# zaiisao/ConTEXTure-NeRF

Measured on AMD Instinct MI355X. Metric: UNet denoise steps/sec (CFG-batched SD2-depth UNet eval + PLMS update), higher is better.
Workload: dtype f16; 1 GPU; BASELINE configs[1]: 1 view @768^2 (latent 96^2), 50 PLMS steps (51 UNet evals), SD2-depth UNet fp16, CFG batch 2, guidance 10, random-init weights; mesh substitution napoleon.obj -> n/a for this stage (denoise loop only); latent=96, cfg_batch=2, ctx_len=77, views_per_rank=1, parallelism=view-shard x1

## Files before the change

contexture-nerf_amd/csrc/gemm.hip:

```cpp
#include "common.h"
#include "kernels.h"
#include <hip/hip_ext.h>
#include <stdlib.h>

__device__ __forceinline__ int xcd_remap(int bid, int nwg)
{
    int q = nwg >> 3, r = nwg & 7, x = bid & 7;
    return (x < r ? x * (q + 1) : r * (q + 1) + (x - r) * q) + (bid >> 3);
}

__device__ __forceinline__ float fast_erf(float x)
{
    float ax = __builtin_fabsf(x);
    float t = __builtin_amdgcn_rcpf(1.0f + 0.3275911f * ax);
    float p = t * (0.254829592f + t * (-0.284496736f + t * (1.421413741f + t * (-1.453152027f + t * 1.061405429f))));
    float e = 1.0f - p * __builtin_amdgcn_exp2f(-1.4426950408889634f * ax * ax);
    return __builtin_copysignf(e, x);
}
__device__ __forceinline__ float gelu_erf(float x) { return 0.5f * x * (1.0f + fast_erf(x * 0.70710678118654752f)); }

template <int MI, int NI>
__device__ __forceinline__ void gemm_epilogue(const GemmArgs &a, f32x16 (&acc)[MI][NI], int mw, int nw, int r, int h)
{
#pragma unroll
    for (int mi = 0; mi < MI; ++mi) {
        int m = mw + mi * 32 + r;
        if (m >= a.M) continue;
        int bidx = a.rowbias ? m / a.rows_per_batch : 0;
        if (a.epi == 1) {
            if constexpr (NI == 2) {
                int fbase = nw / 2;
#pragma unroll
                for (int g = 0; g < 4; ++g) {
                    int nn = nw + 8 * g + 4 * h;
                    if (nn >= a.N) continue;
                    f16x4 o;
#pragma unroll
                    for (int j = 0; j < 4; ++j) {
                        float xv = acc[mi][0][4 * g + j], gv = acc[mi][1][4 * g + j];
                        if (a.bias) { xv += (float)a.bias[nn + j]; gv += (float)a.bias[nn + 32 + j]; }
                        o[j] = (f16)(xv * gelu_erf(gv));
                    }
                    *(f16x4 *)(a.out + (size_t)m * a.ldc + fbase + 8 * g + 4 * h) = o;
                }
            }
        } else {
#pragma unroll
            for (int ni = 0; ni < NI; ++ni)
#pragma unroll
                for (int g = 0; g < 4; ++g) {
                    int nn = nw + ni * 32 + 8 * g + 4 * h;
                    if (nn >= a.N) continue;
                    float v[4];
#pragma unroll
                    for (int j = 0; j < 4; ++j) v[j] = acc[mi][ni][4 * g + j];
                    if (a.bias) {
                        f16x4 b = *(const f16x4 *)(a.bias + nn);
#pragma unroll
                        for (int j = 0; j < 4; ++j) v[j] += (float)b[j];
                    }
                    if (a.rowbias) {
                        f16x4 b = *(const f16x4 *)(a.rowbias + (size_t)bidx * a.ldrb + nn);
#pragma unroll
                        for (int j = 0; j < 4; ++j) v[j] += (float)b[j];
                    }
                    if (a.residual) {
                        if (a.res32) {
                            f32x4 b = *(const f32x4 *)((const float *)a.residual + (size_t)m * a.ldr + nn);
#pragma unroll
                            for (int j = 0; j < 4; ++j) v[j] += b[j];
                        } else {
                            f16x4 b = *(const f16x4 *)(a.residual + (size_t)m * a.ldr + nn);
#pragma unroll
                            for (int j = 0; j < 4; ++j) v[j] += (float)b[j];
                        }
                    }
                    if (a.out32) {
                        *(f32x4 *)((float *)a.out + (size_t)m * a.ldc + nn) = (f32x4){v[0], v[1], v[2], v[3]};
                    } else {
                        f16x4 o;
#pragma unroll
                        for (int j = 0; j < 4; ++j) o[j] = (f16)v[j];
                        *(f16x4 *)(a.out + (size_t)m * a.ldc + nn) = o;
                    }
                }
        }
    }
}

template <int MI, int NI>
__device__ __forceinline__ void gemm_epilogue_staged(const GemmArgs &a, f32x16 (&acc)[MI][NI], int mw, int nw, int r, int h,
                                                     float *stage, int lane)
{
    constexpr int RS = 32 * NI + 4;
    constexpr int LPR = 4 * NI;
    constexpr int RPP = 64 / LPR;
    const int prow = lane / LPR, c8 = (lane % LPR) * 8;
    const int n = nw + c8;
    f16x8 bs = {0, 0, 0, 0, 0, 0, 0, 0};
    if (a.bias && n < a.N) bs = *(const f16x8 *)(a.bias + n);
#pragma unroll
    for (int mi = 0; mi < MI; ++mi) {
#pragma unroll
        for (int ni = 0; ni < NI; ++ni)
#pragma unroll
            for (int g = 0; g < 4; ++g) {
                f32x4 v = {acc[mi][ni][4 * g], acc[mi][ni][4 * g + 1], acc[mi][ni][4 * g + 2], acc[mi][ni][4 * g + 3]};
                *(f32x4 *)(stage + r * RS + ni * 32 + 8 * g + 4 * h) = v;
            }
#pragma unroll
        for (int p = 0; p < 32 / RPP; ++p) {
            const int row = RPP * p + prow;
            const int m = mw + mi * 32 + row;
            f32x4 v0 = *(const f32x4 *)(stage + row * RS + c8), v1 = *(const f32x4 *)(stage + row * RS + c8 + 4);
            if (m < a.M && n < a.N) {
                float v[8] = {v0[0], v0[1], v0[2], v0[3], v1[0], v1[1], v1[2], v1[3]};
#pragma unroll
                for (int j = 0; j < 8; ++j) v[j] += (float)bs[j];
                if (a.rowbias) {
                    f16x8 b = *(const f16x8 *)(a.rowbias + (size_t)(m / a.rows_per_batch) * a.ldrb + n);
#pragma unroll
                    for (int j = 0; j < 8; ++j) v[j] += (float)b[j];
                }
                if (a.residual) {
                    if (a.res32) {
                        const float *rp = (const float *)a.residual + (size_t)m * a.ldr + n;
                        f32x4 b0 = *(const f32x4 *)rp, b1 = *(const f32x4 *)(rp + 4);
#pragma unroll
                        for (int j = 0; j < 4; ++j) { v[j] += b0[j]; v[4 + j] += b1[j]; }
                    } else {
                        f16x8 b = *(const f16x8 *)(a.residual + (size_t)m * a.ldr + n);
#pragma unroll
                        for (int j = 0; j < 8; ++j) v[j] += (float)b[j];
                    }
                }
                if (a.out32) {
                    float *op = (float *)a.out + (size_t)m * a.ldc + n;
                    *(f32x4 *)op = (f32x4){v[0], v[1], v[2], v[3]}; *(f32x4 *)(op + 4) = (f32x4){v[4], v[5], v[6], v[7]};
                } else {
                    f16x8 o;
#pragma unroll
                    for (int j = 0; j < 8; ++j) o[j] = (f16)v[j];
                    *(f16x8 *)(a.out + (size_t)m * a.ldc + n) = o;
                }
            }
        }
    }
}

__device__ __attribute__((aligned(16))) f16 g_zero_page[64];

typedef const __attribute__((address_space(1))) void *gptr_t;
typedef __attribute__((address_space(3))) void *lptr_t;

template <int WM, int WN, int MI, int NI, bool CONV, int NS, int PKT>
__global__ __launch_bounds__(64 * WM * WN) void k_gemm_pipe(GemmArgs a)
{
    constexpr int BM = 32 * MI * WM, BN = 32 * NI * WN, NW = WM * WN;
    constexpr int RP = 512 / PKT;
    constexpr int LPR = PKT / 8;
    constexpr int XI = BM / (RP * NW), WI = BN / (RP * NW);
    static_assert(XI >= 1 && WI >= 1, "tile too small for the wave count");
    constexpr int G = XI + WI;
    constexpr int STAGE = (BM + BN) * PKT;
    extern __shared__ __attribute__((aligned(16))) f16 smem[];

    const int tid = threadIdx.x, lane = tid & 63, wave = __builtin_amdgcn_readfirstlane(tid >> 6);
    const int r = lane & 31, h = lane >> 5;
    const int wm = wave / WN, wn = wave % WN;
    const int ntiles = a.ntm * a.ntn;
    const int lin = xcd_remap(blockIdx.x, ntiles * a.splitk);
    const int slice = lin / ntiles, bid = lin - slice * ntiles;
    const int tile_n = a.mfast ? bid / a.ntm : bid % a.ntn, tile_m = a.mfast ? bid % a.ntm : bid / a.ntn;
    const int m0 = tile_m * BM, n0 = tile_n * BN;
    const int lr = lane / LPR, pc = lane % LPR;

    const int nk_all = a.K / PKT;
    const int kbeg = (int)((long)nk_all * slice / a.splitk);
    const int nk = (int)((long)nk_all * (slice + 1) / a.splitk) - kbeg;

    const f16 *xp[XI], *wp[WI];
    int xst[XI], wst[WI];
    int xoff[XI], xoy[XI], xox[XI], xlc[XI];
    bool xok[XI];
#pragma unroll
    for (int i = 0; i < XI; ++i) {
        int row = RP * (wave + NW * i) + lr;
        int m = m0 + row;
        xlc[i] = (pc ^ (PKT == 32 ? ((row >> 2) & 3) : ((row >> 1) & 7))) * 8;
        xok[i] = m < a.M;
        if (CONV) {
            int hw = a.Ho * a.Wo;
            int b = m / hw, p = m - b * hw;
            int oy = p / a.Wo, ox = p - oy * a.Wo;
            xoy[i] = oy * a.stride; xox[i] = ox * a.stride;
            xoff[i] = b * a.H * a.W * a.Cin;
            xp[i] = g_zero_page; xst[i] = 0;
        } else {
            xoff[i] = 0; xoy[i] = 0; xox[i] = 0;
            xp[i] = xok[i] ? a.X + (size_t)m * a.K + kbeg * PKT + xlc[i] : g_zero_page;
            xst[i] = xok[i] ? PKT : 0;
        }
    }
#pragma unroll
    for (int i = 0; i < WI; ++i) {
        int row = RP * (wave + NW * i) + lr;
        bool ok = (n0 + row) < a.N;
        wp[i] = ok ? a.Wt + (size_t)(n0 + row) * a.K + kbeg * PKT + ((pc ^ (PKT == 32 ? ((row >> 2) & 3) : ((row >> 1) & 7))) * 8) : g_zero_page;
        wst[i] = ok ? PKT : 0;
    }
    const int k_lo = kbeg * PKT, k_hi = (kbeg + nk) * PKT;
    const int rot = a.krot == 1 ? (int)(((unsigned)tile_m * 13u + (unsigned)tile_n * 5u) % (unsigned)nk) : 0;
    int k_issue = k_lo + rot * PKT, issued = 0, tap_left = 0;
    if (!CONV) {
#pragma unroll
        for (int i = 0; i < XI; ++i) xp[i] += (xst[i] ? rot * PKT : 0);
    }
#pragma unroll
    for (int i = 0; i < WI; ++i) wp[i] += (wst[i] ? rot * PKT : 0);

    auto retap = [&]() {
        int tap = k_issue / a.Cin, c0 = k_issue - tap * a.Cin;
        int dy = tap / 3 - 1 + a.poff, dx = tap % 3 - 1 + a.poff;
        int Hv = a.H << a.ups, Wv = a.W << a.ups;
#pragma unroll
        for (int i = 0; i < XI; ++i) {
            int iy = xoy[i] + dy, ix = xox[i] + dx;
            bool ok = xok[i] && iy >= 0 && iy < Hv && ix >= 0 && ix < Wv && !(a.zins && ((iy | ix) & 1));
            xp[i] = ok ? a.X + xoff[i] + (((iy >> a.ups) * a.W + (ix >> a.ups)) * a.Cin) + c0 + xlc[i] : g_zero_page;
            xst[i] = ok ? PKT : 0;
        }
        tap_left = (a.Cin - c0) / PKT;
    };
    auto issue = [&](int buf) {
        if (k_issue == k_hi) {
            k_issue = k_lo;
            const int span = k_hi - k_lo;
            if (!CONV) {
#pragma unroll
                for (int i = 0; i < XI; ++i) xp[i] -= (xst[i] ? span : 0);
            }
#pragma unroll
            for (int i = 0; i < WI; ++i) wp[i] -= (wst[i] ? span : 0);
            tap_left = 0;
        }
        if (CONV) {
            if (tap_left == 0) retap();
            --tap_left;
        }
        f16 *Xs = smem + buf * STAGE;
        f16 *Ws = Xs + BM * PKT;
#pragma unroll
        for (int i = 0; i < XI; ++i) {
            __builtin_amdgcn_global_load_lds((gptr_t)xp[i], (lptr_t)(Xs + (wave + NW * i) * 512), 16, 0, 0);
            xp[i] += xst[i];
        }
#pragma unroll
        for (int i = 0; i < WI; ++i) {
            __builtin_amdgcn_global_load_lds((gptr_t)wp[i], (lptr_t)(Ws + (wave + NW * i) * 512), 16, 0, 0);
            wp[i] += wst[i];
        }
        k_issue += PKT;
        ++issued;
    };

    f32x16 acc[MI][NI];
#pragma unroll
    for (int i = 0; i < MI; ++i)
#pragma unroll
        for (int j = 0; j < NI; ++j)
#pragma unroll
            for (int q = 0; q < 16; ++q) acc[i][j][q] = 0.f;

#pragma unroll
    for (int p = 0; p < NS - 1; ++p)
        if (p < nk) issue(p);
    const int swz = PKT == 32 ? ((r >> 2) & 3) : ((r >> 1) & 7);
    const int xrow = (wm * 32 * MI + r) * PKT, wrow = BM * PKT + (wn * 32 * NI + r) * PKT;
    int kt = 0;
    for (; a.krot == 0 && kt + 2 * NS - 2 < nk; kt += NS) {
#pragma unroll
        for (int u = 0; u < NS; ++u) {
            asm volatile("s_waitcnt vmcnt(%0) lgkmcnt(0)" ::"n"((NS - 2) * G) : "memory");
            ctx_barrier();
            issue((u + NS - 1) % NS);
            const f16 *sb = smem + u * STAGE;
#pragma unroll
            for (int ks = 0; ks < PKT / 16; ++ks) {
                const int pch = ((2 * ks + h) ^ swz) * 8;
                f16x8 xf[MI], wf[NI];
#pragma unroll
                for (int i = 0; i < MI; ++i) xf[i] = *(const f16x8 *)(sb + xrow + i * 32 * PKT + pch);
#pragma unroll
                for (int j = 0; j < NI; ++j) wf[j] = *(const f16x8 *)(sb + wrow + j * 32 * PKT + pch);
#pragma unroll
                for (int i = 0; i < MI; ++i)
#pragma unroll
                    for (int j = 0; j < NI; ++j) acc[i][j] = __builtin_amdgcn_mfma_f32_32x32x16_f16(wf[j], xf[i], acc[i][j], 0, 0, 0);
            }
        }
    }
    for (; kt < nk; kt += NS) {
#pragma unroll
        for (int u = 0; u < NS; ++u) {
            if (kt + u < nk) {
                int newer = issued - 1 - (kt + u);
                if (NS >= 8 && newer >= 6) asm volatile("s_waitcnt vmcnt(%0)" ::"n"(6 * G) : "memory");
                else if (NS >= 7 && newer >= 5) asm volatile("s_waitcnt vmcnt(%0)" ::"n"(5 * G) : "memory");
                else if (NS >= 6 && newer >= 4) asm volatile("s_waitcnt vmcnt(%0)" ::"n"(4 * G) : "memory");
                else if (NS >= 5 && newer >= 3) asm volatile("s_waitcnt vmcnt(%0)" ::"n"(3 * G) : "memory");
                else if (NS >= 4 && newer >= 2) asm volatile("s_waitcnt vmcnt(%0)" ::"n"(2 * G) : "memory");
                else if (newer >= 1) asm volatile("s_waitcnt vmcnt(%0)" ::"n"(G) : "memory");
                else asm volatile("s_waitcnt vmcnt(0)" ::: "memory");
                asm volatile("s_waitcnt lgkmcnt(0)" ::: "memory");
                ctx_barrier();
                if (issued < nk) issue((u + NS - 1) % NS);
                const f16 *sb = smem + u * STAGE;
#pragma unroll
                for (int ks = 0; ks < PKT / 16; ++ks) {
                    const int pch = ((2 * ks + h) ^ swz) * 8;
                    f16x8 xf[MI], wf[NI];
#pragma unroll
                    for (int i = 0; i < MI; ++i) xf[i] = *(const f16x8 *)(sb + xrow + i * 32 * PKT + pch);
#pragma unroll
                    for (int j = 0; j < NI; ++j) wf[j] = *(const f16x8 *)(sb + wrow + j * 32 * PKT + pch);
#pragma unroll
                    for (int i = 0; i < MI; ++i)
#pragma unroll
                        for (int j = 0; j < NI; ++j) acc[i][j] = __builtin_amdgcn_mfma_f32_32x32x16_f16(wf[j], xf[i], acc[i][j], 0, 0, 0);
                }
            }
        }
    }
    if (a.splitk > 1) {
        float *pb = a.part + (size_t)slice * a.M * a.N;
#pragma unroll
        for (int mi = 0; mi < MI; ++mi) {
            int m = m0 + wm * 32 * MI + mi * 32 + r;
            if (m >= a.M) continue;
#pragma unroll
            for (int ni = 0; ni < NI; ++ni)
#pragma unroll
                for (int g = 0; g < 4; ++g) {
                    int nn = n0 + wn * 32 * NI + ni * 32 + 8 * g + 4 * h;
                    if (nn >= a.N) continue;
                    f32x4 v = {acc[mi][ni][4 * g], acc[mi][ni][4 * g + 1], acc[mi][ni][4 * g + 2], acc[mi][ni][4 * g + 3]};
                    *(f32x4 *)(pb + (size_t)m * a.N + nn) = v;
                }
        }
        return;
    }
    if (a.epi == 0 && a.stage_epi) {
        asm volatile("s_waitcnt vmcnt(0) lgkmcnt(0)" ::: "memory");
        ctx_barrier();
        gemm_epilogue_staged<MI, NI>(a, acc, m0 + wm * 32 * MI, n0 + wn * 32 * NI, r, h, (float *)smem + wave * (32 * (32 * NI + 4)), lane);
        return;
    }
    gemm_epilogue<MI, NI>(a, acc, m0 + wm * 32 * MI, n0 + wn * 32 * NI, r, h);
}

__global__ __launch_bounds__(256) void k_splitk_reduce(GemmArgs a)
{
    const int n4 = a.N / 4;
    const size_t total = (size_t)a.M * n4, MN = (size_t)a.M * a.N;
    for (size_t i = (size_t)blockIdx.x * 256 + threadIdx.x; i < total; i += (size_t)gridDim.x * 256) {
        int m = (int)(i / n4), nn = (int)(i % n4) * 4;
        f32x4 v = *(const f32x4 *)(a.part + (size_t)m * a.N + nn);
        for (int sidx = 1; sidx < a.splitk; ++sidx) {
            f32x4 p = *(const f32x4 *)(a.part + sidx * MN + (size_t)m * a.N + nn);
            v += p;
        }
        if (a.bias) { f16x4 b = *(const f16x4 *)(a.bias + nn); for (int j = 0; j < 4; ++j) v[j] += (float)b[j]; }
        if (a.rowbias) {
            f16x4 b = *(const f16x4 *)(a.rowbias + (size_t)(m / a.rows_per_batch) * a.ldrb + nn);
            for (int j = 0; j < 4; ++j) v[j] += (float)b[j];
        }
        if (a.residual) {
            if (a.res32) { f32x4 b = *(const f32x4 *)((const float *)a.residual + (size_t)m * a.ldr + nn); v += b; }
            else { f16x4 b = *(const f16x4 *)(a.residual + (size_t)m * a.ldr + nn); for (int j = 0; j < 4; ++j) v[j] += (float)b[j]; }
        }
        if (a.out32) { *(f32x4 *)((float *)a.out + (size_t)m * a.ldc + nn) = v; continue; }
        f16x4 o;
        for (int j = 0; j < 4; ++j) o[j] = (f16)v[j];
        *(f16x4 *)(a.out + (size_t)m * a.ldc + nn) = o;
    }
}

static int g_force_tile = -1, g_force_gemm8 = -1;
extern "C" void ctx_gemm_tune(int32_t tile, int32_t gemm8)
{
    g_force_tile = tile;
    g_force_gemm8 = gemm8;
}

template <int WM, int WN, int MI, int NI, bool CONV, int NS = 4, int PKT = 32>
static void launch_gemm(GemmArgs &a, hipStream_t s)
{
    constexpr int BM = 32 * MI * WM, BN = 32 * NI * WN;
    a.ntm = cdiv(a.M, BM);
    a.ntn = cdiv(a.N, BN);
    if (a.splitk < 1 || !a.part) a.splitk = 1;
    static int mfast = -2;
    if (mfast == -2) { const char *e = getenv("CTX_GEMM_MFAST"); mfast = e ? atoi(e) : -1; }
    const double wbytes = (double)a.N * a.K, xbytes = (double)a.M * (CONV ? a.Cin : a.K);
    a.mfast = mfast >= 0 ? mfast : (wbytes > xbytes ? 1 : 0);
    static int stg = -1;
    if (stg < 0) { const char *e = getenv("CTX_GEMM_STAGE_EPI"); stg = e ? atoi(e) : 1; }
    a.stage_epi = stg && (a.ldc % 8 == 0) && (!a.residual || a.ldr % 8 == 0) && (!a.rowbias || a.ldrb % 8 == 0) &&
                  (size_t)WM * WN * 32 * (32 * NI + 4) * sizeof(float) <= 160 * 1024;
    static int steady = -1;
    if (steady < 0) { const char *e = getenv("CTX_GEMM_STEADY"); steady = e ? atoi(e) : 1; }
    a.pk = PKT; a.krot = steady ? 0 : 2;
    constexpr int NT = 64 * WM * WN;
    constexpr size_t ring = (size_t)NS * (BM + BN) * PKT * sizeof(f16);
    constexpr size_t patch = (size_t)WM * WN * 32 * (32 * NI + 4) * sizeof(float);
    constexpr size_t lds = (ring > patch || patch > 160 * 1024) ? ring : patch;
    auto kern = k_gemm_pipe<WM, WN, MI, NI, CONV, NS, PKT>;
    static bool attr_done = false;
    if (!attr_done) {
        (void)hipFuncSetAttribute((const void *)kern, hipFuncAttributeMaxDynamicSharedMemorySize, (int)lds);
        attr_done = true;
    }
    if (ctx_prof_on()) {
        hipEvent_t e0, e1;
        ctx_prof_events(0, &e0, &e1);
        hipExtLaunchKernelGGL(kern, dim3(a.ntm * a.ntn * a.splitk), dim3(NT), lds, s, e0, e1, 0, a);
    } else
        hipLaunchKernelGGL(kern, dim3(a.ntm * a.ntn * a.splitk), dim3(NT), lds, s, a);
}

static void launch_reduce(GemmArgs &a, hipStream_t s)
{
    size_t total = (size_t)a.M * (a.N / 4);
    unsigned nb = (unsigned)((total + 255) / 256 < 2048 ? (total + 255) / 256 : 2048);
    if (ctx_prof_on()) {
        hipEvent_t e0, e1;
        ctx_prof_events(0, &e0, &e1);
        hipExtLaunchKernelGGL(k_splitk_reduce, dim3(nb), dim3(256), 0, s, e0, e1, 0, a);
    } else
        hipLaunchKernelGGL(k_splitk_reduce, dim3(nb), dim3(256), 0, s, a);
}

int ctx_gemm_pick_split(int M, int N, int K, int epi)
{
    static int en = -1;
    if (en < 0) { const char *e = getenv("CTX_SPLITK"); en = e ? atoi(e) : 1; }
    if (!en || epi != 0 || N % 4) return 1;
    bool wide = (N % 128 == 0);
    int tiles = wide ? cdiv(M, 128) * cdiv(N, 128) : cdiv(M, 256) * cdiv(N, 64);
    if (tiles >= 200) return 1;
    if (K < 2048 && tiles > 48) return 1;
    int S = 640 / tiles;
    int maxS = (K / 32) / 8;
    if (S > maxS) S = maxS;
    if (S > 32) S = 32;
    return S < 2 ? 1 : S;
}

#include "gemm_tuned.h"
void ctx_gemm_plan(GemmArgs &a, bool conv)
{
    a.tile = -1; a.use8 = -1;
    static int use_table = -1;
    if (use_table < 0) { const char *e = getenv("CTX_GEMM_TUNED"); use_table = e ? atoi(e) : 1; }
    if (use_table) {
        const int flags = conv ? ((a.stride == 2 ? 1 : 0) | (a.ups ? 2 : 0)) : 0;
        for (const TunedGemm &t : g_tuned)
            if (t.conv == (conv ? 1 : 0) && t.M == a.M && t.N == a.N && t.K == a.K && t.flags == flags && t.epi == a.epi) {
                a.tile = t.tile; a.use8 = t.use8; a.splitk = t.splitk;
                return;
            }
    }
    if (a.K % 64 == 0 && (!conv || a.Cin % 64 == 0)) {
        const double MN = (double)a.M * a.N;
        static const int heur144 = [] { const char *e = getenv("CTX_GEMM_HEUR144"); return e ? atoi(e) : 1; }();
        if (heur144 && a.epi == 0 && a.N % 8 == 0 && !a.zins && !a.res32 && !a.out32) {
            const int nt = cdiv(a.N, 160);
            const double fill = (double)a.N / (160.0 * nt);
            if (fill >= 0.9) {
                if (cdiv(a.M, 288) * nt >= 512) { a.tile = -1; a.use8 = 8; a.splitk = 1; return; }
                if (cdiv(a.M, 144) * nt >= 220) { a.tile = -1; a.use8 = 6; a.splitk = 1; return; }
            }
        }
        int tile, bm, bn;
        if (MN >= 5.0e6) { tile = a.epi == 1 ? 10 : (conv ? 12 : 11); bm = 256; bn = 128; }
        else if ((MN >= 2.5e6 && a.K >= 960) || (conv && MN >= 1.2e6 && a.K >= 5760)) { tile = 14; bm = 128; bn = 128; }
        else if (a.epi == 1) { tile = 16; bm = 64; bn = 128; }
        else { tile = 15; bm = 64; bn = 64; }
        const int tiles = cdiv(a.M, bm) * cdiv(a.N, bn);
        int S = 1;
        if (a.epi == 0 && a.N % 4 == 0) {
            S = 320 / tiles;
            const int maxS = a.K / 64 / 4;
            if (S > maxS) S = maxS;
            if (S > 12) S = 12;
            if (S < 1) S = 1;
        }
        a.tile = tile; a.splitk = S;
        a.use8 = (a.epi == 1 && MN >= 1.0e7) ? -1 : 0;
        return;
    }
    a.splitk = ctx_gemm_pick_split(a.M, a.N, a.K, a.epi);
}

int ctx_gemm_dispatch(GemmArgs &a, bool conv, hipStream_t s)
{
    const bool only_pipe = a.zins || a.res32 || a.out32;
    if (only_pipe) a.use8 = 0;
    const int want8 = only_pipe ? 0 : (g_force_gemm8 >= 0 ? g_force_gemm8 : a.use8);
    const int want_tile = g_force_tile >= 0 ? g_force_tile : (g_force_gemm8 >= 0 ? -1 : a.tile);
    if (want_tile < 0 && want8 >= 4 && want8 <= 8 && ctx_gemm144_try(a, conv, want8 - 4, s)) {
        if (a.splitk > 1) launch_reduce(a, s);
    } else if (want_tile < 0 && conv && (want8 == 2 || want8 == 3) && ctx_conv_halo_try(a, want8 == 2 ? 2 : 1, s)) {
        if (a.splitk > 1) launch_reduce(a, s);
    } else if (want_tile < 0 && want8 != 0 && want8 < 2 && ctx_gemm8_try(a, conv, want8 == 1, s)) {
        if (a.splitk > 1) launch_reduce(a, s);
    } else {
        static int big = -1;
        if (big < 0) { const char *e = getenv("CTX_GEMM_BIG"); big = e ? atoi(e) : 1; }
        const int S = a.splitk > 1 && a.part ? a.splitk : 1;
        auto wgs = [&](int bm, int bn) { return cdiv(a.M, bm) * cdiv(a.N, bn) * S; };
        const bool n128 = (a.N % 128 == 0);
        int pick;
        static int bigk = -1;
        if (bigk < 0) { const char *e = getenv("CTX_GEMM_BIGK"); bigk = e ? atoi(e) : 1024; }
        if (big && a.M >= 8192 && a.N >= 256 && a.K >= bigk) pick = 0;
        else if (n128 && wgs(128, 128) >= 384) pick = 1;
        else if (!n128 && wgs(256, 64) >= 384) pick = 2;
        else if (wgs(128, 64) >= 320) pick = 3;
        else if (S > 1) pick = n128 ? 1 : 2;
        else pick = 4;
        static int force = -2;
        if (force == -2) { const char *e = getenv("CTX_GEMM_TILE"); force = e ? atoi(e) : -1; }
        if (force >= 0) pick = force;
        if (want_tile >= 0) pick = want_tile;
        if (a.epi == 1 && (pick == 5 || pick == 6 || pick == 9 || pick == 11 || pick == 13 || pick == 15 || pick == 17 || pick == 19 || pick == 21 || pick == 23 || pick == 26 || pick == 27)) pick = 1;
        if (pick >= 10 && (a.K % 64 != 0 || (conv && a.Cin % 64 != 0))) pick = 1;
#define CTX_LAUNCH(WM_, WN_, MI_, NI_) do { if (conv) launch_gemm<WM_, WN_, MI_, NI_, true>(a, s); else launch_gemm<WM_, WN_, MI_, NI_, false>(a, s); } while (0)
        switch (pick) {
        case 0: CTX_LAUNCH(4, 2, 2, 2); break;
        case 1: CTX_LAUNCH(2, 2, 2, 2); break;
        case 2: CTX_LAUNCH(4, 1, 2, 2); break;
        case 3: CTX_LAUNCH(2, 1, 2, 2); break;
        case 4: CTX_LAUNCH(1, 1, 2, 2); break;
        case 5: CTX_LAUNCH(2, 2, 1, 1); break;
        case 6: CTX_LAUNCH(1, 2, 2, 1); break;
        case 7: CTX_LAUNCH(4, 2, 1, 2); break;
        case 8: CTX_LAUNCH(2, 2, 1, 2); break;
        case 9: CTX_LAUNCH(2, 2, 2, 1); break;
#define CTX_LAUNCH64(WM_, WN_, MI_, NI_) do { if (conv) launch_gemm<WM_, WN_, MI_, NI_, true, 3, 64>(a, s); else launch_gemm<WM_, WN_, MI_, NI_, false, 3, 64>(a, s); } while (0)
        case 10: CTX_LAUNCH64(8, 2, 1, 2); break;
        case 11: CTX_LAUNCH64(4, 4, 2, 1); break;
        case 12: CTX_LAUNCH64(4, 2, 2, 2); break;
        case 13: CTX_LAUNCH64(4, 4, 1, 1); break;
        case 14: CTX_LAUNCH64(4, 2, 1, 2); break;
        case 15: CTX_LAUNCH64(2, 2, 1, 1); break;
        case 16: CTX_LAUNCH64(2, 2, 1, 2); break;
        case 17: CTX_LAUNCH64(2, 2, 2, 1); break;
        case 18: CTX_LAUNCH64(2, 2, 2, 2); break;
#define CTX_LAUNCH64N2(WM_, WN_, MI_, NI_) do { if (conv) launch_gemm<WM_, WN_, MI_, NI_, true, 2, 64>(a, s); else launch_gemm<WM_, WN_, MI_, NI_, false, 2, 64>(a, s); } while (0)
        case 19: CTX_LAUNCH64N2(2, 2, 1, 1); break;
        case 20: CTX_LAUNCH64N2(4, 2, 1, 2); break;
        case 21: CTX_LAUNCH64N2(4, 4, 1, 1); break;
        case 22: CTX_LAUNCH64N2(2, 2, 2, 2); break;
#define CTX_LAUNCH64NS(NS_, WM_, WN_, MI_, NI_) do { if (conv) launch_gemm<WM_, WN_, MI_, NI_, true, NS_, 64>(a, s); else launch_gemm<WM_, WN_, MI_, NI_, false, NS_, 64>(a, s); } while (0)
        case 23: CTX_LAUNCH64NS(6, 2, 2, 1, 1); break;
        case 24: CTX_LAUNCH64NS(5, 2, 2, 1, 2); break;
        case 25: CTX_LAUNCH64NS(4, 4, 2, 1, 2); break;
        case 26: CTX_LAUNCH64NS(5, 2, 2, 2, 1); break;
        default: CTX_LAUNCH64N2(4, 2, 2, 5); break;
#undef CTX_LAUNCH64NS
#undef CTX_LAUNCH64N2
#undef CTX_LAUNCH64
        }
#undef CTX_LAUNCH
        if (a.splitk > 1) launch_reduce(a, s);
    }
    hipError_t e = hipGetLastError();
    if (e != hipSuccess) {
        ctx_set_error("gemm launch failed: %s", hipGetErrorString(e));
        return CTX_E_LAUNCH;
    }
    return CTX_OK;
}

extern "C" int32_t ctx_gemm_f16(const void *A, const void *Wt, const void *bias, const void *residual, int32_t M,
                                int32_t N, int32_t K, void *C, ctx_stream_t stream)
{
    CTX_REQUIRE(A && Wt && C, "gemm: null pointer");
    CTX_REQUIRE(M > 0 && N > 0 && K > 0 && K % 64 == 0 && N % 8 == 0, "gemm: need K%%64==0, N%%8==0 (M=%d N=%d K=%d)", M, N, K);
    CTX_REQUIRE((int64_t)M * K < (1ll << 31) && (int64_t)N * K < (1ll << 31), "gemm: operand too large for 32-bit offsets");
    GemmArgs a = {};
    a.X = (const f16 *)A; a.Wt = (const f16 *)Wt; a.bias = (const f16 *)bias; a.residual = (const f16 *)residual;
    a.out = (f16 *)C; a.M = M; a.N = N; a.K = K; a.ldc = N; a.ldr = N; a.rows_per_batch = 1; a.ldrb = N; a.epi = 0;
    a.tile = -1; a.use8 = -1;
    return ctx_gemm_dispatch(a, false, (hipStream_t)stream);
}

extern "C" int32_t ctx_conv3x3_f16(const void *x, const void *w, const void *bias, const void *rowbias,
                                   const void *residual, int32_t B, int32_t H, int32_t W, int32_t Cin, int32_t Cout,
                                   int32_t stride, int32_t upsample, void *y, ctx_stream_t stream)
{
    CTX_REQUIRE(x && w && y, "conv3x3: null pointer");
    CTX_REQUIRE(B > 0 && H > 0 && W > 0 && Cin % 64 == 0 && Cout % 8 == 0 && (stride == 1 || stride == 2) &&
                    (upsample == 0 || upsample == 1) && !(upsample && stride == 2),
                "conv3x3: need Cin%%64==0, Cout%%8==0, stride 1|2 (B=%d H=%d W=%d Cin=%d Cout=%d s=%d up=%d)", B, H, W, Cin, Cout, stride, upsample);
    GemmArgs a = {};
    int Hv = H << upsample, Wv = W << upsample;
    a.Ho = (Hv + 2 - 3) / stride + 1; a.Wo = (Wv + 2 - 3) / stride + 1;
    a.X = (const f16 *)x; a.Wt = (const f16 *)w; a.bias = (const f16 *)bias; a.rowbias = (const f16 *)rowbias;
    a.residual = (const f16 *)residual; a.out = (f16 *)y;
    a.M = B * a.Ho * a.Wo; a.N = Cout; a.K = 9 * Cin; a.ldc = Cout; a.ldr = Cout; a.rows_per_batch = a.Ho * a.Wo; a.ldrb = Cout; a.epi = 0;
    a.H = H; a.W = W; a.Cin = Cin; a.stride = stride; a.ups = upsample;
    a.tile = -1; a.use8 = -1;
    CTX_REQUIRE((int64_t)B * H * W * Cin < (1ll << 31) && (int64_t)Cout * a.K < (1ll << 31), "conv3x3: tensor too large for 32-bit offsets");
    return ctx_gemm_dispatch(a, true, (hipStream_t)stream);
}

#define GV_U 4
__global__ __launch_bounds__(256) void k_gemv_f16(const f16 *__restrict__ x, const f16 *__restrict__ w,
                                                  const f16 *__restrict__ bias, int Bm, int N, int K, int silu_in,
                                                  int silu_out, f16 *__restrict__ out)
{
    const int lane = threadIdx.x & 63;
    const int n0 = ((blockIdx.x * 256 + threadIdx.x) >> 6) * 2;
    if (n0 >= N) return;
    const int n1 = n0 + 1 < N ? n0 + 1 : n0;
    float acc[2][4] = {{0.f, 0.f, 0.f, 0.f}, {0.f, 0.f, 0.f, 0.f}};
    const f16x8 zero8 = {0, 0, 0, 0, 0, 0, 0, 0};
    for (int k0 = 0; k0 < K; k0 += 512 * GV_U) {
        f16x8 wv[2][GV_U];
#pragma unroll
        for (int u = 0; u < GV_U; ++u) {
            const int k = k0 + u * 512 + lane * 8;
            const int kc = k < K ? k : K - 8;
            wv[0][u] = *(const f16x8 *)(w + (size_t)n0 * K + kc);
            wv[1][u] = *(const f16x8 *)(w + (size_t)n1 * K + kc);
        }
#pragma unroll
        for (int u = 0; u < GV_U; ++u) {
            const int k = k0 + u * 512 + lane * 8;
            if (k >= K) { wv[0][u] = zero8; wv[1][u] = zero8; }
            const int kc = k < K ? k : K - 8;
            for (int b = 0; b < Bm; ++b) {
                f16x8 xv = *(const f16x8 *)(x + (size_t)b * K + kc);
#pragma unroll
                for (int j = 0; j < 8; ++j) {
                    float xf = (float)xv[j];
                    if (silu_in) xf = xf / (1.0f + __expf(-xf));
                    acc[0][b] += xf * (float)wv[0][u][j];
                    acc[1][b] += xf * (float)wv[1][u][j];
                }
            }
        }
    }
    for (int r = 0; r < 2; ++r) {
        const int n = n0 + r;
        for (int b = 0; b < Bm; ++b) {
            float v = wave_sum(acc[r][b]);
            if (lane == 0 && n < N) {
                if (bias) v += (float)bias[n];
                if (silu_out) v = v / (1.0f + __expf(-v));
                out[(size_t)b * N + n] = (f16)v;
            }
        }
    }
}

int ctx_gemv_f16(const f16 *x, const f16 *w, const f16 *bias, int Bm, int N, int K, int silu_in, int silu_out, f16 *out,
                 hipStream_t s)
{
    if (Bm < 1 || K % 8 != 0 || K < 8) {
        ctx_set_error("gemv: Bm=%d (>=1) K=%d (%%8)", Bm, K);
        return CTX_E_ARG;
    }
    for (int b0 = 0; b0 < Bm; b0 += 4) {
        const int nb = Bm - b0 < 4 ? Bm - b0 : 4;
        hipLaunchKernelGGL(k_gemv_f16, dim3(cdiv(N, 8)), dim3(256), 0, s, x + (size_t)b0 * K, w, bias, nb, N, K, silu_in, silu_out,
                           out + (size_t)b0 * N);
    }
    return CTX_OK;
}

extern "C" float ctx_bench_gemm(const void *A, const void *Wt, const void *bias, const void *residual, int32_t M, int32_t N,
                                int32_t K, void *C, int32_t conv_B, int32_t conv_H, int32_t conv_W, int32_t conv_Cin,
                                int32_t conv_flags, int32_t epi, void *part, int32_t splitk, int32_t iters, ctx_stream_t stream)
{
    hipStream_t s = (hipStream_t)stream;
    GemmArgs a = {};
    a.X = (const f16 *)A; a.Wt = (const f16 *)Wt; a.bias = (const f16 *)bias; a.residual = (const f16 *)residual; a.out = (f16 *)C;
    bool conv = conv_B > 0;
    if (conv) {
        a.stride = (conv_flags & 1) ? 2 : 1; a.ups = (conv_flags & 2) ? 1 : 0;
        int Hv = conv_H << a.ups, Wv = conv_W << a.ups;
        a.H = conv_H; a.W = conv_W; a.Cin = conv_Cin; a.Ho = (Hv - 1) / a.stride + 1; a.Wo = (Wv - 1) / a.stride + 1;
        a.M = conv_B * a.Ho * a.Wo; a.N = N; a.K = 9 * conv_Cin; a.rows_per_batch = a.Ho * a.Wo;
    } else {
        a.M = M; a.N = N; a.K = K; a.rows_per_batch = 1;
    }
    a.epi = epi;
    a.ldc = epi == 1 ? a.N / 2 : a.N; a.ldr = a.N; a.ldrb = a.N;
    a.tile = -1; a.use8 = -1;
    if (splitk < 0) {
        if (part) { ctx_gemm_plan(a, conv); splitk = a.splitk; } else splitk = 1;
    }
    hipEvent_t e0, e1;
    (void)hipEventCreate(&e0); (void)hipEventCreate(&e1);
    for (int i = 0; i < iters + 2; ++i) {
        if (i == 2) (void)hipEventRecord(e0, s);
        GemmArgs b = a;
        b.splitk = splitk; b.part = (float *)part;
        int rc = ctx_gemm_dispatch(b, conv, s);
        if (rc) return (float)rc;
    }
    (void)hipEventRecord(e1, s);
    (void)hipEventSynchronize(e1);
    float ms = 0.f;
    (void)hipEventElapsedTime(&ms, e0, e1);
    (void)hipEventDestroy(e0); (void)hipEventDestroy(e1);
    return ms / iters;
}
```

contexture-nerf_amd/csrc/gemm144.hip:

```cpp
#include "common.h"
#include "kernels.h"
#include <hip/hip_ext.h>
#include <stdlib.h>
#include <type_traits>

typedef const __attribute__((address_space(1))) void *g144_gptr_t;
typedef __attribute__((address_space(3))) void *g144_lptr_t;
__device__ __attribute__((aligned(128))) f16 g144_zero[64];

#define G144_BM 144
#define G144_BN 160
#define G144_STAGE ((G144_BM + G144_BN) * 64)

__device__ __forceinline__ int g144_xcd_remap(int bid, int nwg)
{
    int q = nwg >> 3, r = nwg & 7, x = bid & 7;
    return (x < r ? x * (q + 1) : r * (q + 1) + (x - r) * q) + (bid >> 3);
}

template <int WM, int WN, bool CONV, int NS, int VAR, bool UPS = false, int BMB = 9>
__global__ __launch_bounds__(64 * WM * WN) void k_gemm144(GemmArgs a)
{
    constexpr int NW = WM * WN, MI = BMB / WM, NI = 10 / WN;
    constexpr int BM = 16 * BMB, NPX = BM / 8;
    constexpr int NP = NPX + 20;
    constexpr int STAGE = (BM + G144_BN) * 64;
    static_assert(BMB % WM == 0 && (BMB == 9 || (BMB == 18 && VAR == 0)), "288-row tiles: lockstep schedule only");
    constexpr int SL = (NP + NW - 1) / NW;
    static_assert(9 % WM == 0 && 10 % WN == 0, "wave grid must divide 9 x 10 blocks");
    extern __shared__ __attribute__((aligned(16))) f16 smem[];
    const int tid = threadIdx.x, lane = tid & 63, wave = __builtin_amdgcn_readfirstlane(tid >> 6);
    const int wm = wave / WN, wn = wave % WN;
    const int r16 = lane & 15, kg = lane >> 4;

    const int ntiles = a.ntm * a.ntn;
    const int lin = g144_xcd_remap(blockIdx.x, ntiles * a.splitk);
    const int slice = lin / ntiles, bid = lin - slice * ntiles;
    const int tile_n = a.mfast ? bid / a.ntm : bid % a.ntn, tile_m = a.mfast ? bid % a.ntm : bid / a.ntn;
    const int m0 = tile_m * BM, n0 = tile_n * G144_BN;
    const int nk_all = a.K / 64;
    const int kbeg = (int)((long)nk_all * slice / a.splitk);
    const int nk = (int)((long)nk_all * (slice + 1) / a.splitk) - kbeg;

    const int prow = lane >> 3, pc = lane & 7;
    constexpr bool FAST = CONV && !UPS;
    const f16 *pp[SL], *xcen[SL];
    int pst[SL], xoff[SL], xoy[SL], xox[SL], xlc[SL], xval[SL];
    bool xok[SL];
    const f16 *const zp = g144_zero;
    const bool full = wave + NW * (SL - 1) < NP;
#pragma unroll
    for (int i = 0; i < SL; ++i) {
        const int p = wave + NW * i;
        const bool isx = p < NPX, live = p < NP;
        const int s = isx ? 8 * p + prow : 8 * (p - NPX) + prow;
        xlc[i] = (pc ^ ((s >> 1) & 7)) * 8;
        xoff[i] = 0; xoy[i] = 0; xox[i] = 0;
        if (isx) {
            const int m = m0 + s;
            xok[i] = m < a.M;
            if (CONV) {
                const int hw = a.Ho * a.Wo;
                const int mm = xok[i] ? m : 0;
                const int b = mm / hw, q = mm - b * hw;
                const int oy = q / a.Wo, ox = q - oy * a.Wo;
                xoy[i] = oy * a.stride; xox[i] = ox * a.stride;
                xoff[i] = b * a.H * a.W * a.Cin + xlc[i];
                pp[i] = zp; pst[i] = 0;
                if (FAST) {
                    xcen[i] = a.X + (size_t)xoff[i] + (size_t)(xoy[i] * a.W + xox[i]) * a.Cin;
                    int v = 0;
#pragma unroll
                    for (int t = 0; t < 9; ++t) {
                        const int iy = xoy[i] + t / 3 - 1 + a.poff, ix = xox[i] + t % 3 - 1 + a.poff;
                        if (xok[i] && iy >= 0 && iy < a.H && ix >= 0 && ix < a.W) v |= 1 << t;
                    }
                    xval[i] = v;
                }
            } else {
                pp[i] = xok[i] ? a.X + (size_t)m * a.K + (size_t)kbeg * 64 + xlc[i] : g144_zero;
                pst[i] = xok[i] ? 64 : 0;
            }
        } else {
            const bool ok = live && (n0 + s) < a.N;
            xok[i] = ok;
            pp[i] = ok ? a.Wt + (size_t)(n0 + s) * a.K + (size_t)kbeg * 64 + xlc[i] : g144_zero;
            pst[i] = ok ? 64 : 0;
        }
    }

    int k_issue = kbeg * 64, issued = 0, tap_left = 0;
    int cur_tap = CONV ? (kbeg * 64) / a.Cin : 0, cur_c0 = CONV ? kbeg * 64 - cur_tap * a.Cin : 0;
    auto retap = [&]() {
        if (FAST) {
            const int dy = cur_tap / 3 - 1 + a.poff, dx = cur_tap - (cur_tap / 3) * 3 - 1 + a.poff;
            const int soff = (dy * a.W + dx) * a.Cin + cur_c0;
#pragma unroll
            for (int i = 0; i < SL; ++i) {
                if (wave + NW * i >= NPX) continue;
                const bool v = (xval[i] >> cur_tap) & 1;
                pp[i] = v ? xcen[i] + soff : zp;
                pst[i] = v ? 64 : 0;
            }
            tap_left = (a.Cin - cur_c0) >> 6;
            return;
        }
        const int tap = k_issue / a.Cin, c0 = k_issue - tap * a.Cin;
        const int dy = tap / 3 - 1 + a.poff, dx = tap % 3 - 1 + a.poff;
        const int Hv = a.H << a.ups, Wv = a.W << a.ups;
#pragma unroll
        for (int i = 0; i < SL; ++i) {
            if (wave + NW * i >= NPX) continue;
            const int iy = xoy[i] + dy, ix = xox[i] + dx;
            const bool ok = xok[i] && iy >= 0 && iy < Hv && ix >= 0 && ix < Wv;
            pp[i] = ok ? a.X + xoff[i] + (((iy >> a.ups) * a.W + (ix >> a.ups)) * a.Cin) + c0 : zp;
            pst[i] = ok ? 64 : 0;
        }
        tap_left = (a.Cin - c0) / 64;
    };
    auto issue_begin = [&]() {
        if (CONV) {
            if (tap_left == 0) retap();
            --tap_left;
        }
    };
    auto issue_slot = [&](int buf, int i) {
        const int p = wave + NW * i;
        if (p < NP) {
            __builtin_amdgcn_global_load_lds((g144_gptr_t)pp[i], (g144_lptr_t)(smem + buf * STAGE + p * 512), 16, 0, 0);
            pp[i] += pst[i];
        }
    };
    auto issue_end = [&]() {
        k_issue += 64; ++issued;
        if (FAST) { cur_c0 += 64; if (cur_c0 == a.Cin) { cur_c0 = 0; ++cur_tap; } }
    };
    auto issue = [&](int buf) {
        issue_begin();
#pragma unroll
        for (int i = 0; i < SL; ++i) issue_slot(buf, i);
        issue_end();
    };

    f32x4 acc[MI][NI];
#pragma unroll
    for (int i = 0; i < MI; ++i)
#pragma unroll
        for (int j = 0; j < NI; ++j) acc[i][j] = (f32x4){0.f, 0.f, 0.f, 0.f};

    const int swz = (r16 >> 1) & 7;
    const int ck[2] = {(kg ^ swz) * 8, ((4 + kg) ^ swz) * 8};
    const int xrow = (wm * 16 * MI + r16) * 64, wrow = BM * 64 + (wn * 16 * NI + r16) * 64;

#pragma unroll
    for (int p = 0; p < NS - 1; ++p)
        if (p < nk) issue(p);
    auto wait_newer = [&](int newer) {
        if (newer >= 2) {
            if (full) asm volatile("s_waitcnt vmcnt(%0)" ::"n"(2 * SL) : "memory");
            else asm volatile("s_waitcnt vmcnt(%0)" ::"n"(2 * (SL - 1)) : "memory");
        } else if (newer >= 1) {
            if (full) asm volatile("s_waitcnt vmcnt(%0)" ::"n"(SL) : "memory");
            else asm volatile("s_waitcnt vmcnt(%0)" ::"n"(SL - 1) : "memory");
        } else
            asm volatile("s_waitcnt vmcnt(0)" ::: "memory");
    };
    int buf = 0;
    if constexpr (VAR == 0 && BMB == 18) {
        f16x8 xa[MI], wa[NI], wb[NI];
        auto mrow = [&](const f16x8 &xf, const f16x8 (&wf)[NI], int i) {
#pragma unroll
            for (int j = 0; j < NI; ++j) acc[i][j] = __builtin_amdgcn_mfma_f32_16x16x32_f16(wf[j], xf, acc[i][j], 0, 0, 0);
        };
        static_assert(BMB != 18 || SL <= MI, "one DMA piece per MFMA row");
        for (int kt = 0; kt < nk; ++kt) {
            wait_newer(issued - 1 - kt);
            asm volatile("s_waitcnt lgkmcnt(0)" ::: "memory");
            ctx_barrier();
            const bool go = issued < nk;
            const int pb = buf == 0 ? NS - 1 : buf - 1;
            const f16 *sb = smem + buf * STAGE;
#pragma unroll
            for (int i = 0; i < MI; ++i) xa[i] = *(const f16x8 *)(sb + xrow + i * 1024 + ck[0]);
#pragma unroll
            for (int j = 0; j < NI; ++j) wa[j] = *(const f16x8 *)(sb + wrow + j * 1024 + ck[0]);
            if (go) issue_begin();
#pragma unroll
            for (int i = 0; i < MI; ++i) {
                mrow(xa[i], wa, i);
                __builtin_amdgcn_sched_barrier(0);
                xa[i] = *(const f16x8 *)(sb + xrow + i * 1024 + ck[1]);
                if (i == 0) {
#pragma unroll
                    for (int j = 0; j < NI; ++j) wb[j] = *(const f16x8 *)(sb + wrow + j * 1024 + ck[1]);
                }
                if (go && i < SL) issue_slot(pb, i);
                __builtin_amdgcn_sched_barrier(0);
            }
            if (go) issue_end();
#pragma unroll
            for (int i = 0; i < MI; ++i) mrow(xa[i], wb, i);
            buf = buf == NS - 1 ? 0 : buf + 1;
        }
    } else if constexpr (VAR == 0) {
        for (int kt = 0; kt < nk; ++kt) {
            wait_newer(issued - 1 - kt);
            asm volatile("s_waitcnt lgkmcnt(0)" ::: "memory");
            ctx_barrier();
            if (issued < nk) issue(buf == 0 ? NS - 1 : buf - 1);
            const f16 *sb = smem + buf * STAGE;
#pragma unroll
            for (int ks = 0; ks < 2; ++ks) {
                f16x8 xf[MI], wf[NI];
#pragma unroll
                for (int i = 0; i < MI; ++i) xf[i] = *(const f16x8 *)(sb + xrow + i * 1024 + ck[ks]);
#pragma unroll
                for (int j = 0; j < NI; ++j) wf[j] = *(const f16x8 *)(sb + wrow + j * 1024 + ck[ks]);
#pragma unroll
                for (int i = 0; i < MI; ++i)
#pragma unroll
                    for (int j = 0; j < NI; ++j) acc[i][j] = __builtin_amdgcn_mfma_f32_16x16x32_f16(wf[j], xf[i], acc[i][j], 0, 0, 0);
            }
            buf = buf == NS - 1 ? 0 : buf + 1;
        }
    } else if constexpr (VAR == 2) {
        static_assert(VAR != 2 || NS == 4, "written for a ring of 4");
        f16x8 xa[MI], wa[NI], xb[MI], wb[NI];
        auto rd = [&](f16x8 (&xf)[MI], f16x8 (&wf)[NI], const f16 *sb, int ks) {
#pragma unroll
            for (int i = 0; i < MI; ++i) xf[i] = *(const f16x8 *)(sb + xrow + i * 1024 + ck[ks]);
#pragma unroll
            for (int j = 0; j < NI; ++j) wf[j] = *(const f16x8 *)(sb + wrow + j * 1024 + ck[ks]);
        };
        auto mrow = [&](const f16x8 &xf, const f16x8 (&wf)[NI], int i) {
#pragma unroll
            for (int j = 0; j < NI; ++j) acc[i][j] = __builtin_amdgcn_mfma_f32_16x16x32_f16(wf[j], xf, acc[i][j], 0, 0, 0);
        };
        static_assert(SL <= MI, "one DMA piece per MFMA row of a quarter");
        if (issued < nk) issue(issued & 3);
        auto pair = [&](int k0, auto steady) {
            constexpr bool ST = decltype(steady)::value;
            const int b0 = k0 & 3;
            const bool two = ST || k0 + 1 < nk;
            asm volatile("s_waitcnt vmcnt(0) lgkmcnt(0)" ::: "memory");
            ctx_barrier();
            rd(xa, wa, smem + b0 * STAGE, 0);
#pragma unroll
            for (int q = 0; q < 4; ++q) {
                if (q >= 2 && !two) break;
                const bool even = (q & 1) == 0;
                if (q + 1 < (two ? 4 : 2)) {
                    const f16 *sn = smem + (b0 + ((q + 1) >> 1)) * STAGE;
                    if (even) rd(xb, wb, sn, (q + 1) & 1); else rd(xa, wa, sn, (q + 1) & 1);
                }
                const bool dma = even && (ST || (issued < nk && issued <= k0 + 3));
                if (dma) issue_begin();
#pragma unroll
                for (int i = 0; i < MI; ++i) {
                    if (even) mrow(xa[i], wa, i); else mrow(xb[i], wb, i);
                    __builtin_amdgcn_sched_barrier(0);
                    if (dma && i < SL) issue_slot(issued & 3, i);
                    __builtin_amdgcn_sched_barrier(0);
                }
                if (dma) issue_end();
            }
        };
        using T1 = std::integral_constant<bool, true>;
        using T0 = std::integral_constant<bool, false>;
        int k0 = 0;
        if (k0 < nk) { pair(k0, T0{}); k0 += 2; }
        for (; k0 + 3 < nk; k0 += 2) pair(k0, T1{});
        for (; k0 < nk; k0 += 2) pair(k0, T0{});
    } else {
        static_assert(VAR == 0 || NS == 4, "written for a ring of 4");
        wait_newer(issued - 1);
        ctx_barrier();
        f16x8 xp_[MI], wp_[NI], xq[MI], wq[NI], xb[MI], wb[NI];
        auto rd = [&](f16x8 (&xf)[MI], f16x8 (&wf)[NI], const f16 *sb, int ks) {
#pragma unroll
            for (int i = 0; i < MI; ++i) xf[i] = *(const f16x8 *)(sb + xrow + i * 1024 + ck[ks]);
#pragma unroll
            for (int j = 0; j < NI; ++j) wf[j] = *(const f16x8 *)(sb + wrow + j * 1024 + ck[ks]);
        };
        auto mrow = [&](const f16x8 &xf, const f16x8 (&wf)[NI], int i) {
#pragma unroll
            for (int j = 0; j < NI; ++j) acc[i][j] = __builtin_amdgcn_mfma_f32_16x16x32_f16(wf[j], xf, acc[i][j], 0, 0, 0);
        };
        rd(xp_, wp_, smem, 0);
        auto stage = [&](f16x8 (&xc)[MI], f16x8 (&wc)[NI], f16x8 (&xn)[MI], f16x8 (&wn_)[NI], int kt, auto steady) {
            constexpr bool ST = decltype(steady)::value;
            if (ST) {
                if (full) asm volatile("s_waitcnt vmcnt(%0)" ::"n"(SL) : "memory");
                else asm volatile("s_waitcnt vmcnt(%0)" ::"n"(SL - 1) : "memory");
            } else
                wait_newer(issued - 1 - (kt + 1));
            asm volatile("s_waitcnt lgkmcnt(0)" ::: "memory");
            ctx_barrier();
            const bool go = ST || issued < nk;
            const int pb = buf == 0 ? NS - 1 : buf - 1;
            const int nb_ = buf == NS - 1 ? 0 : buf + 1;
            const f16 *sc = smem + buf * STAGE, *sn = smem + nb_ * STAGE;
            const bool more = ST || kt + 1 < nk;
            if (go) issue_begin();
#pragma unroll
            for (int i = 0; i < MI; ++i) {
                mrow(xc[i], wc, i);
                __builtin_amdgcn_sched_barrier(0);
                if (i == 0) rd(xb, wb, sc, 1);
                if (go && i < SL) issue_slot(pb, i);
                __builtin_amdgcn_sched_barrier(0);
            }
            if (go) {
#pragma unroll
                for (int i = MI; i < SL; ++i) issue_slot(pb, i);
                issue_end();
            }
#pragma unroll
            for (int i = 0; i < MI; ++i) {
                mrow(xb[i], wb, i);
                if (i == 0) {
                    __builtin_amdgcn_sched_barrier(0);
                    if (more) rd(xn, wn_, sn, 0);
                    __builtin_amdgcn_sched_barrier(0);
                }
            }
            buf = nb_;
        };
        using T1 = std::integral_constant<bool, true>;
        using T0 = std::integral_constant<bool, false>;
        int kt = 0;
        for (; kt + 4 < nk; kt += 2) {
            stage(xp_, wp_, xq, wq, kt, T1{});
            stage(xq, wq, xp_, wp_, kt + 1, T1{});
        }
        for (; kt + 1 < nk; kt += 2) {
            stage(xp_, wp_, xq, wq, kt, T0{});
            stage(xq, wq, xp_, wp_, kt + 1, T0{});
        }
        if (kt < nk) stage(xp_, wp_, xq, wq, kt, T0{});
    }

    const int mb = m0 + wm * 16 * MI, nb = n0 + wn * 16 * NI;
    if (a.splitk > 1) {
        float *pb = a.part + (size_t)slice * a.M * a.N;
#pragma unroll
        for (int i = 0; i < MI; ++i) {
            const int m = mb + 16 * i + r16;
            if (m >= a.M) continue;
#pragma unroll
            for (int j = 0; j < NI; ++j) {
                const int nn = nb + 16 * j + 4 * kg;
                if (nn < a.N) *(f32x4 *)(pb + (size_t)m * a.N + nn) = acc[i][j];
            }
        }
        return;
    }
    if (a.stage_epi) {
        constexpr int RS = G144_BN + 4;
        float *tile = (float *)smem;
        asm volatile("s_waitcnt vmcnt(0) lgkmcnt(0)" ::: "memory");
        ctx_barrier();
        constexpr int NT = 64 * NW, CPR = G144_BN / 8;
#pragma unroll
        for (int half = 0; half < BMB / 9; ++half) {
            if (half) __syncthreads();
#pragma unroll
            for (int i = 0; i < MI; ++i) {
                const int blk = wm * MI + i;
                if (blk / 9 != half) continue;
#pragma unroll
                for (int j = 0; j < NI; ++j)
                    *(f32x4 *)(tile + ((blk - 9 * half) * 16 + r16) * RS + wn * 16 * NI + 16 * j + 4 * kg) = acc[i][j];
            }
            __syncthreads();
            for (int ch = tid; ch < 144 * CPR; ch += NT) {
                const int row = ch / CPR, c8 = (ch - row * CPR) * 8;
                const int m = m0 + 144 * half + row, n = n0 + c8;
                if (m >= a.M || n >= a.N) continue;
                const f32x4 v0 = *(const f32x4 *)(tile + row * RS + c8), v1 = *(const f32x4 *)(tile + row * RS + c8 + 4);
                float v[8] = {v0[0], v0[1], v0[2], v0[3], v1[0], v1[1], v1[2], v1[3]};
                if (a.bias) {
                    const f16x8 bb = *(const f16x8 *)(a.bias + n);
#pragma unroll
                    for (int e = 0; e < 8; ++e) v[e] += (float)bb[e];
                }
                if (a.rowbias) {
                    const f16x8 bb = *(const f16x8 *)(a.rowbias + (size_t)(m / a.rows_per_batch) * a.ldrb + n);
#pragma unroll
                    for (int e = 0; e < 8; ++e) v[e] += (float)bb[e];
                }
                if (a.residual) {
                    const f16x8 bb = *(const f16x8 *)(a.residual + (size_t)m * a.ldr + n);
#pragma unroll
                    for (int e = 0; e < 8; ++e) v[e] += (float)bb[e];
                }
                f16x8 o;
#pragma unroll
                for (int e = 0; e < 8; ++e) o[e] = (f16)v[e];
                *(f16x8 *)(a.out + (size_t)m * a.ldc + n) = o;
            }
        }
        return;
    }
    f16x4 bs[NI];
#pragma unroll
    for (int j = 0; j < NI; ++j) {
        const int nn = nb + 16 * j + 4 * kg;
        bs[j] = (a.bias && nn < a.N) ? *(const f16x4 *)(a.bias + nn) : (f16x4){0, 0, 0, 0};
    }
#pragma unroll
    for (int i = 0; i < MI; ++i) {
        const int m = mb + 16 * i + r16;
        if (m >= a.M) continue;
        const int bidx = a.rowbias ? m / a.rows_per_batch : 0;
#pragma unroll
        for (int j = 0; j < NI; ++j) {
            const int nn = nb + 16 * j + 4 * kg;
            if (nn >= a.N) continue;
            f32x4 v = acc[i][j];
#pragma unroll
            for (int e = 0; e < 4; ++e) v[e] += (float)bs[j][e];
            if (a.rowbias) {
                f16x4 b = *(const f16x4 *)(a.rowbias + (size_t)bidx * a.ldrb + nn);
#pragma unroll
                for (int e = 0; e < 4; ++e) v[e] += (float)b[e];
            }
            if (a.residual) {
                f16x4 b = *(const f16x4 *)(a.residual + (size_t)m * a.ldr + nn);
#pragma unroll
                for (int e = 0; e < 4; ++e) v[e] += (float)b[e];
            }
            f16x4 o;
#pragma unroll
            for (int e = 0; e < 4; ++e) o[e] = (f16)v[e];
            *(f16x4 *)(a.out + (size_t)m * a.ldc + nn) = o;
        }
    }
}

int ctx_gemm144_try(GemmArgs &a, bool conv, int form, hipStream_t s)
{
    if (a.K % 64 != 0 || (conv && a.Cin % 64 != 0) || a.N % 4 != 0 || a.epi != 0 || a.res32 || a.out32 || a.zins) return 0;
    if (a.ldc % 4 != 0 || (a.residual && a.ldr % 4 != 0) || (a.rowbias && a.ldrb % 4 != 0)) return 0;
    const int bm = form == 4 ? 288 : G144_BM;
    a.ntm = cdiv(a.M, bm);
    a.ntn = cdiv(a.N, G144_BN);
    int S = (a.splitk > 1 && a.part) ? a.splitk : 1;
    if (S > a.K / 64) S = a.K / 64;
    a.splitk = S;
    const double wbytes = (double)a.N * a.K, xbytes = (double)a.M * (conv ? a.Cin : a.K);
    a.mfast = wbytes > xbytes ? 1 : 0;
    static int stg = -1;
    if (stg < 0) { const char *e = getenv("CTX_G144_STAGE"); stg = e ? atoi(e) : 1; }
    a.stage_epi = stg && form != 0 && a.N % 8 == 0 && a.ldc % 8 == 0 && (!a.residual || a.ldr % 8 == 0) && (!a.rowbias || a.ldrb % 8 == 0);
    static bool attr[20] = {};
    auto go = [&](auto kern, int which, int threads, int ns) {
        const size_t lds = (size_t)ns * (bm + G144_BN) * 64 * sizeof(f16);
        if (!attr[which]) {
            (void)hipFuncSetAttribute((const void *)kern, hipFuncAttributeMaxDynamicSharedMemorySize, (int)lds);
            attr[which] = true;
        }
        if (ctx_prof_on()) {
            hipEvent_t e0, e1;
            ctx_prof_events(0, &e0, &e1);
            hipExtLaunchKernelGGL(kern, dim3(a.ntm * a.ntn * S), dim3(threads), lds, s, e0, e1, 0, a);
        } else
            hipLaunchKernelGGL(kern, dim3(a.ntm * a.ntn * S), dim3(threads), lds, s, a);
    };
    const bool ups = conv && a.ups;
    switch (form) {
    case 4:
        if (!conv) go(k_gemm144<3, 5, false, 2, 0, false, 18>, 12, 960, 2);
        else if (ups) go(k_gemm144<3, 5, true, 2, 0, true, 18>, 13, 960, 2); else go(k_gemm144<3, 5, true, 2, 0, false, 18>, 14, 960, 2);
        break;
    case 1:
        if (!conv) go(k_gemm144<3, 5, false, 3, 0>, 2, 960, 3);
        else if (ups) go(k_gemm144<3, 5, true, 3, 0, true>, 8, 960, 3); else go(k_gemm144<3, 5, true, 3, 0>, 3, 960, 3);
        break;
    case 2:
        if (!conv) go(k_gemm144<3, 5, false, 4, 1>, 4, 960, 4);
        else if (ups) go(k_gemm144<3, 5, true, 4, 1, true>, 9, 960, 4); else go(k_gemm144<3, 5, true, 4, 1>, 5, 960, 4);
        break;
    case 3:
        if (!conv) go(k_gemm144<3, 5, false, 4, 2>, 6, 960, 4);
        else if (ups) go(k_gemm144<3, 5, true, 4, 2, true>, 10, 960, 4); else go(k_gemm144<3, 5, true, 4, 2>, 7, 960, 4);
        break;
    default:
        if (!conv) go(k_gemm144<3, 2, false, 3, 0>, 0, 384, 3);
        else if (ups) go(k_gemm144<3, 2, true, 3, 0, true>, 11, 384, 3); else go(k_gemm144<3, 2, true, 3, 0>, 1, 384, 3);
        break;
    }
    return 1;
}
```

contexture-nerf_amd/csrc/kernels.h:

```cpp
#pragma once
#include "common.h"

struct GemmArgs {
    const f16 *X;
    const f16 *Wt;
    const f16 *bias;
    const f16 *rowbias;
    const f16 *residual;
    f16 *out;
    int M, N, K;
    int ldc, ldr;
    int rows_per_batch;
    int ldrb;
    int epi;
    int H, W, Cin, Ho, Wo, stride, ups;
    int poff;
    int res32, out32;
    int zins;
    int ntm, ntn;
    int splitk;
    float *part;
    int pk;
    int krot;
    int tile, use8;
    int stage_epi;
    int mfast;
};

int ctx_gemm_dispatch(GemmArgs &a, bool conv, hipStream_t s);
int ctx_gemm8_try(GemmArgs &a, bool conv, bool force, hipStream_t s);
int ctx_conv_halo_try(GemmArgs &a, int ni, hipStream_t s);
int ctx_gemm144_try(GemmArgs &a, bool conv, int form, hipStream_t s);
int ctx_gemm_pick_split(int M, int N, int K, int epi);
void ctx_gemm_plan(GemmArgs &a, bool conv);
int ctx_gemv_f16(const f16 *x, const f16 *w, const f16 *bias, int Bm, int N, int K, int silu_in, int silu_out, f16 *out, hipStream_t s);
int ctx_concat_f16(const f16 *a, const f16 *b, int64_t M, int Ca, int Cb, f16 *y, hipStream_t s);
int ctx_transpose_v_f16(const f16 *v, int B, int S, int ld, int heads, int Sp, int perm, f16 *vt, hipStream_t s);
int ctx_f32_to_f16(const float *x, int64_t n, f16 *y, hipStream_t s);
int ctx_time_embed_f16(const float *t, int B, int dim, f16 *out, hipStream_t s);
int ctx_conv_in_f16(const float *x, const f16 *w, const f16 *bias, int B, int Cin, int H, int W, int Cout, f16 *y, hipStream_t s);
int ctx_conv_out_f16(const f16 *x, const f16 *w, const f16 *bias, int B, int H, int W, int C, int Cout, float *out, hipStream_t s);
int ctx_attention_core(const f16 *Q, const f16 *K, const f16 *V, int B, int Sq, int Skv, int heads, int q_stride,
                       int kv_stride, float scale, f16 *O, int o_stride, hipStream_t s);
extern "C" int64_t ctx_groupnorm_ws_bytes(int32_t B, int32_t groups);
int ctx_groupnorm_any(const void *x, int x32, const void *gamma, const void *beta, int B, int HW, int C, int groups, float eps, int silu,
                      void *y, void *stats_ws, hipStream_t stream);
int ctx_layernorm_any(const void *x, int x32, const void *gamma, const void *beta, int64_t rows, int C, float eps, void *y, hipStream_t stream);
int ctx_concat_f32(const float *a, const float *b, int64_t M, int Ca, int Cb, float *y, hipStream_t s);
int ctx_f16_to_f32(const f16 *x, int64_t n, float *y, hipStream_t s);

bool ctx_prof_on(void);
void ctx_prof_events(int klass, hipEvent_t *a, hipEvent_t *b);
```

contexture-nerf_amd/csrc/norm.hip:

```cpp
#include "common.h"
#include "kernels.h"
#include <math.h>

struct F8 { float v[8]; };
template <bool X32>
__device__ __forceinline__ F8 ld8(const void *base, size_t elem)
{
    F8 r;
    if (X32) {
        const f32x4 a = *(const f32x4 *)((const float *)base + elem), b = *(const f32x4 *)((const float *)base + elem + 4);
#pragma unroll
        for (int j = 0; j < 4; ++j) { r.v[j] = a[j]; r.v[4 + j] = b[j]; }
    } else {
        const f16x8 a = *(const f16x8 *)((const f16 *)base + elem);
#pragma unroll
        for (int j = 0; j < 8; ++j) r.v[j] = (float)a[j];
    }
    return r;
}

#define GN_MAX_GROUPS 64
#define GN_MAX_SPLITS 128
#define GN_MAX_C 4096
#define GN_U 4
#define GN_AU 6
#define GN_AU32 6
#define GN_FOLD 8

template <bool X32>
__global__ __launch_bounds__(1024) void k_gn_stats(const void *__restrict__ x, int HW, int C, int G, int NS, int PL,
                                                   float *__restrict__ part)
{
    extern __shared__ float s_part[];
    const int c8n = C / 8;
    const int b = blockIdx.y, sp = blockIdx.x;
    const int c8 = threadIdx.x % c8n, pl = threadIdx.x / c8n;
    const int per = (HW + NS - 1) / NS;
    const int p0 = sp * per, p1 = min(HW, p0 + per);
    float s[8], q[8];
#pragma unroll
    for (int j = 0; j < 8; ++j) { s[j] = 0.f; q[j] = 0.f; }
    const size_t base = ((size_t)b * HW) * C + c8 * 8;
    for (int p = p0 + pl; p < p1; p += PL * GN_U) {
        F8 v[GN_U];
#pragma unroll
        for (int u = 0; u < GN_U; ++u) v[u] = ld8<X32>(x, base + (size_t)min(p + u * PL, p1 - 1) * C);
#pragma unroll
        for (int u = 0; u < GN_U; ++u) {
            const bool live = p + u * PL < p1;
#pragma unroll
            for (int j = 0; j < 8; ++j) { float f = live ? v[u].v[j] : 0.f; s[j] += f; q[j] += f * f; }
        }
    }
#pragma unroll
    for (int j = 0; j < 8; ++j) {
        s_part[((size_t)pl * C + c8 * 8 + j) * 2 + 0] = s[j];
        s_part[((size_t)pl * C + c8 * 8 + j) * 2 + 1] = q[j];
    }
    __syncthreads();
    float *s_ch = s_part + (size_t)PL * C * 2;
    const int na = max(1, (int)blockDim.x / C);
    for (int it = threadIdx.x; it < C * na; it += blockDim.x) {
        const int a = it / C, c = it - a * C;
        float ss = 0.f, qq = 0.f;
#pragma unroll 4
        for (int l = a; l < PL; l += na) {
            ss += s_part[((size_t)l * C + c) * 2 + 0];
            qq += s_part[((size_t)l * C + c) * 2 + 1];
        }
        s_ch[((size_t)a * C + c) * 2 + 0] = ss;
        s_ch[((size_t)a * C + c) * 2 + 1] = qq;
    }
    __syncthreads();
    const int cg = C / G, cells = na * cg;
    const int octs = (int)blockDim.x >> 3;
    for (int g0 = 0; g0 < G; g0 += octs) {
        const int oc = (int)threadIdx.x >> 3, l = threadIdx.x & 7;
        const int g = oc < octs ? g0 + oc : G;
        float ss = 0.f, qq = 0.f;
        if (g < G)
            for (int k = l; k < cells; k += 8) {
                int a = k / cg, c = g * cg + (k - a * cg);
                ss += s_ch[((size_t)a * C + c) * 2 + 0];
                qq += s_ch[((size_t)a * C + c) * 2 + 1];
            }
#pragma unroll
        for (int o = 4; o > 0; o >>= 1) { ss += __shfl_xor(ss, o, 64); qq += __shfl_xor(qq, o, 64); }
        if (g < G && l == 0) {
            part[(((size_t)b * NS + sp) * G + g) * 2 + 0] = ss;
            part[(((size_t)b * NS + sp) * G + g) * 2 + 1] = qq;
        }
    }
}

template <bool X32> struct Raw8;
template <> struct Raw8<false> {
    f16x8 a;
    __device__ __forceinline__ float get(int j) const { return (float)a[j]; }
};
template <> struct Raw8<true> {
    f32x4 a, b;
    __device__ __forceinline__ float get(int j) const { return j < 4 ? a[j] : b[j - 4]; }
};
template <bool X32>
__device__ __forceinline__ Raw8<X32> ldraw(const void *base, size_t elem)
{
    Raw8<X32> r;
    if constexpr (X32) { r.a = *(const f32x4 *)((const float *)base + elem); r.b = *(const f32x4 *)((const float *)base + elem + 4); }
    else r.a = *(const f16x8 *)((const f16 *)base + elem);
    return r;
}

template <bool X32>
__global__ __launch_bounds__(512) void k_gn_apply(const void *__restrict__ x, const float *__restrict__ part,
                                                  const f16 *__restrict__ gamma, const f16 *__restrict__ beta, int HW, int C,
                                                  int G, int NS, int PL, float eps, int silu, f16 *__restrict__ y)
{
    constexpr int AU = X32 ? GN_AU32 : GN_AU;
    __shared__ float s_mean[GN_MAX_GROUPS], s_rstd[GN_MAX_GROUPS];
    const int b = blockIdx.y;
    const int c8n = C / 8;
    const int c8 = threadIdx.x % c8n, pl = threadIdx.x / c8n;
    const int p0 = blockIdx.x * (PL * AU);
    const size_t xb = (size_t)b * HW * C + c8 * 8;
    f16 *yb = y + (size_t)b * HW * C + c8 * 8;
    Raw8<X32> v[AU];
#pragma unroll
    for (int u = 0; u < AU; ++u) v[u] = ldraw<X32>(x, xb + (size_t)min(p0 + u * PL + pl, HW - 1) * C);
    const f16x8 ga = *(const f16x8 *)(gamma + c8 * 8), be = *(const f16x8 *)(beta + c8 * 8);
    if (threadIdx.x < 256) {
        const int lpg = min(256 / G, 64);
        const int gi = threadIdx.x / lpg, l = threadIdx.x % lpg;
        const int g = min(gi, G - 1);
        float s = 0.f, q = 0.f;
        for (int k0 = 0; k0 < NS; k0 += GN_FOLD * lpg) {
            float2 pv[GN_FOLD];
#pragma unroll
            for (int k = 0; k < GN_FOLD; ++k)
                pv[k] = *(const float2 *)(part + (((size_t)b * NS + min(k0 + k * lpg + l, NS - 1)) * G + g) * 2);
#pragma unroll
            for (int k = 0; k < GN_FOLD; ++k)
                if (k0 + k * lpg + l < NS) { s += pv[k].x; q += pv[k].y; }
        }
        for (int o = lpg >> 1; o > 0; o >>= 1) { s += __shfl_xor(s, o, 64); q += __shfl_xor(q, o, 64); }
        if (l == 0 && gi < G) {
            float n = (float)HW * (float)(C / G);
            float mean = s / n;
            float var = fmaxf(q / n - mean * mean, 0.f);
            s_mean[g] = mean;
            s_rstd[g] = rsqrtf(var + eps);
        }
    }
    __syncthreads();
    const int cg = C / G;
    float sa[8], sh[8];
#pragma unroll
    for (int j = 0; j < 8; ++j) {
        const int gg = (c8 * 8 + j) / cg;
        sa[j] = s_rstd[gg] * (float)ga[j];
        sh[j] = (float)be[j] - s_mean[gg] * sa[j];
    }
#pragma unroll
    for (int u = 0; u < AU; ++u) {
        const int p = p0 + u * PL + pl;
        if (p < HW) {
            f16x8 o;
#pragma unroll
            for (int j = 0; j < 8; ++j) {
                float t = v[u].get(j) * sa[j] + sh[j];
                if (silu) t = t * __builtin_amdgcn_rcpf(1.0f + __builtin_amdgcn_exp2f(-1.4426950408889634f * t));
                o[j] = (f16)t;
            }
            *(f16x8 *)(yb + (size_t)p * C) = o;
        }
    }
}

#define GN_FT 512
#define GN_FU 12
template <bool X32>
__global__ __launch_bounds__(GN_FT) void k_gn_fused(const void *__restrict__ x, const f16 *__restrict__ gamma,
                                                    const f16 *__restrict__ beta, int HW, int C, int G, int PLF, float eps, int silu,
                                                    f16 *__restrict__ y)
{
    __shared__ float s_red[2][GN_FT / 64];
    const int g = blockIdx.x, b = blockIdx.y;
    const int cg = C / G, cpg = cg / 8;
    const int c = threadIdx.x % cpg, pl = threadIdx.x / cpg;
    const bool act = pl < PLF;
    const size_t xb = (size_t)b * HW * C + g * cg + c * 8;
    f16 *yb = y + (size_t)b * HW * C + g * cg + c * 8;
    const f16x8 ga = *(const f16x8 *)(gamma + g * cg + c * 8), be = *(const f16x8 *)(beta + g * cg + c * 8);
    F8 v[GN_FU];
#pragma unroll
    for (int u = 0; u < GN_FU; ++u) v[u] = ld8<X32>(x, xb + (size_t)min(pl + PLF * u, HW - 1) * C);
    float s = 0.f, q = 0.f;
#pragma unroll
    for (int u = 0; u < GN_FU; ++u)
        if (act && pl + PLF * u < HW) {
#pragma unroll
            for (int j = 0; j < 8; ++j) { float f = v[u].v[j]; s += f; q += f * f; }
        }
    s = wave_sum_dpp(s); q = wave_sum_dpp(q);
    const int wave = threadIdx.x >> 6;
    if ((threadIdx.x & 63) == 0) { s_red[0][wave] = s; s_red[1][wave] = q; }
    __syncthreads();
    float ss = 0.f, qq = 0.f;
    const int nw = ((int)blockDim.x + 63) >> 6;
    for (int w = 0; w < nw; ++w) { ss += s_red[0][w]; qq += s_red[1][w]; }
    const float n = (float)HW * (float)cg;
    const float mean = ss / n;
    const float rstd = rsqrtf(fmaxf(qq / n - mean * mean, 0.f) + eps);
    float sa[8], sh[8];
#pragma unroll
    for (int j = 0; j < 8; ++j) { sa[j] = rstd * (float)ga[j]; sh[j] = (float)be[j] - mean * sa[j]; }
#pragma unroll
    for (int u = 0; u < GN_FU; ++u) {
        const int p = pl + PLF * u;
        if (act && p < HW) {
            f16x8 o;
#pragma unroll
            for (int j = 0; j < 8; ++j) {
                float t = v[u].v[j] * sa[j] + sh[j];
                if (silu) t = t * __builtin_amdgcn_rcpf(1.0f + __builtin_amdgcn_exp2f(-1.4426950408889634f * t));
                o[j] = (f16)t;
            }
            *(f16x8 *)(yb + (size_t)p * C) = o;
        }
    }
}

extern "C" int64_t ctx_groupnorm_ws_bytes(int32_t B, int32_t groups)
{
    return ((int64_t)B * GN_MAX_SPLITS * groups * 2 + (int64_t)B * 2 * GN_MAX_C) * 4;
}

extern "C" int32_t ctx_groupnorm_f16(const void *x, const void *gamma, const void *beta, int32_t B, int32_t HW, int32_t C,
                                     int32_t groups, float eps, int32_t silu, void *y, void *stats_ws, ctx_stream_t stream)
{
    return ctx_groupnorm_any(x, 0, gamma, beta, B, HW, C, groups, eps, silu, y, stats_ws, (hipStream_t)stream);
}

int ctx_groupnorm_any(const void *x, int x32, const void *gamma, const void *beta, int B, int HW, int C, int groups, float eps, int silu,
                      void *y, void *stats_ws, hipStream_t stream)
{
    CTX_REQUIRE(x && gamma && beta && y && stats_ws, "groupnorm: null pointer");
    CTX_REQUIRE(B > 0 && HW > 0 && C % 8 == 0 && C % groups == 0 && groups <= GN_MAX_GROUPS && C <= GN_MAX_C &&
                    256 % groups == 0 && (256 / groups & (256 / groups - 1)) == 0,
                "groupnorm: unsupported B=%d HW=%d C=%d groups=%d", B, HW, C, groups);
    hipStream_t s = stream;
    {
        static int fuse = -1;
        if (fuse < 0) { const char *e = getenv("CTX_GN_FUSED"); fuse = e ? atoi(e) : 1; }
        const int cg = C / groups;
        const int cpg = cg / 8;
        const int plf = cg % 8 == 0 ? GN_FT / cpg : 0;
        if (fuse && cg % 8 == 0 && cpg <= GN_FT && (HW + plf - 1) / plf <= GN_FU) {
            const int thr = (cpg * plf + 63) / 64 * 64;
            if (x32) hipLaunchKernelGGL(k_gn_fused<true>, dim3(groups, B), dim3(thr), 0, s, x, (const f16 *)gamma, (const f16 *)beta, HW, C, groups, plf, eps, silu, (f16 *)y);
            else hipLaunchKernelGGL(k_gn_fused<false>, dim3(groups, B), dim3(thr), 0, s, x, (const f16 *)gamma, (const f16 *)beta, HW, C, groups, plf, eps, silu, (f16 *)y);
            CTX_CHECK_LAUNCH("groupnorm");
            return CTX_OK;
        }
    }
    int c8n = C / 8;
    int PL = 1024 / c8n;
    if (PL < 1) PL = 1;
    if (PL > HW) PL = HW;
    int threads = c8n * PL;
    int NS = min(GN_MAX_SPLITS, max(1, HW / PL));
    {
        static const int ns_env = [] { const char *e = getenv("CTX_GN_NS"); return e ? atoi(e) : 0; }();
        const int64_t sample_bytes = (int64_t)HW * C * (x32 ? 4 : 2);
        const int by_size = (int)min((int64_t)GN_MAX_SPLITS, sample_bytes / (384 * 1024));
        const int want = ns_env > 0 ? ns_env : max(16, max(by_size, (64 + B - 1) / B));
        NS = min(NS, want);
    }
    float *part = (float *)stats_ws;
    const int na = threads / C > 1 ? threads / C : 1;
    size_t lds = (size_t)(PL + na) * C * 2 * sizeof(float);
    static bool attr = false;
    if (!attr) {
        (void)hipFuncSetAttribute((const void *)k_gn_stats<false>, hipFuncAttributeMaxDynamicSharedMemorySize, 80 * 1024);
        (void)hipFuncSetAttribute((const void *)k_gn_stats<true>, hipFuncAttributeMaxDynamicSharedMemorySize, 80 * 1024);
        attr = true;
    }
    if (x32) hipLaunchKernelGGL(k_gn_stats<true>, dim3(NS, B), dim3(threads), lds, s, x, HW, C, groups, NS, PL, part);
    else hipLaunchKernelGGL(k_gn_stats<false>, dim3(NS, B), dim3(threads), lds, s, x, HW, C, groups, NS, PL, part);
    size_t total = (size_t)HW * c8n;
    {
        const int au = x32 ? GN_AU32 : GN_AU;
        const int apl = (256 + c8n - 1) / c8n;
        const int athreads = c8n * apl;
        const int nb = (HW + apl * au - 1) / (apl * au);
        if (x32) hipLaunchKernelGGL(k_gn_apply<true>, dim3(nb, B), dim3(athreads), 0, s, x, part, (const f16 *)gamma, (const f16 *)beta, HW, C,
                                    groups, NS, apl, eps, silu, (f16 *)y);
        else hipLaunchKernelGGL(k_gn_apply<false>, dim3(nb, B), dim3(athreads), 0, s, x, part, (const f16 *)gamma, (const f16 *)beta, HW, C,
                                groups, NS, apl, eps, silu, (f16 *)y);
    }
    CTX_CHECK_LAUNCH("groupnorm");
    return CTX_OK;
}

template <int KC, int R, bool X32>
__global__ __launch_bounds__(256) void k_layernorm(const void *__restrict__ x, const f16 *__restrict__ gamma,
                                                   const f16 *__restrict__ beta, int64_t rows, int C, float eps,
                                                   f16 *__restrict__ y)
{
    const int lane = threadIdx.x & 63;
    const int c8n = C / 8;
    const int64_t wave = ((int64_t)blockIdx.x * 256 + threadIdx.x) >> 6;
    const int64_t row0 = wave * R;
    if (row0 >= rows) return;
    F8 v[R][KC];
#pragma unroll
    for (int rr = 0; rr < R; ++rr)
#pragma unroll
        for (int k = 0; k < KC; ++k) {
            int c8 = lane + 64 * k;
            const int64_t rw = row0 + rr < rows ? row0 + rr : rows - 1;
            v[rr][k] = ld8<X32>(x, (size_t)(rw * C + min(c8, c8n - 1) * 8));
            if (c8 >= c8n) {
#pragma unroll
                for (int j = 0; j < 8; ++j) v[rr][k].v[j] = 0.f;
            }
        }
    f16x8 ga[KC], be[KC];
#pragma unroll
    for (int k = 0; k < KC; ++k) {
        int c8 = lane + 64 * k;
        ga[k] = *(const f16x8 *)(gamma + min(c8, c8n - 1) * 8);
        be[k] = *(const f16x8 *)(beta + min(c8, c8n - 1) * 8);
    }
#pragma unroll
    for (int rr = 0; rr < R; ++rr) {
        if (row0 + rr >= rows) break;
        float s = 0.f;
#pragma unroll
        for (int k = 0; k < KC; ++k)
#pragma unroll
            for (int j = 0; j < 8; ++j) s += v[rr][k].v[j];
        float mean = wave_sum_dpp(s) / (float)C;
        float q = 0.f;
#pragma unroll
        for (int k = 0; k < KC; ++k) {
            int c8 = lane + 64 * k;
            if (c8 < c8n) {
#pragma unroll
                for (int j = 0; j < 8; ++j) { float d = v[rr][k].v[j] - mean; q += d * d; }
            }
        }
        float rstd = rsqrtf(wave_sum_dpp(q) / (float)C + eps);
        f16 *yr = y + (row0 + rr) * C;
#pragma unroll
        for (int k = 0; k < KC; ++k) {
            int c8 = lane + 64 * k;
            if (c8 < c8n) {
                f16x8 o;
#pragma unroll
                for (int j = 0; j < 8; ++j) o[j] = (f16)((v[rr][k].v[j] - mean) * rstd * (float)ga[k][j] + (float)be[k][j]);
                *(f16x8 *)(yr + c8 * 8) = o;
            }
        }
    }
}

__device__ __forceinline__ float sum8_dpp(float v)
{
    v += __builtin_bit_cast(float, __builtin_amdgcn_update_dpp(0, __builtin_bit_cast(int, v), 0xB1, 0xf, 0xf, true));
    v += __builtin_bit_cast(float, __builtin_amdgcn_update_dpp(0, __builtin_bit_cast(int, v), 0x4E, 0xf, 0xf, true));
    v += __builtin_bit_cast(float, __builtin_amdgcn_update_dpp(0, __builtin_bit_cast(int, v), 0x141, 0xf, 0xf, true));
    return v;
}
template <int KC>
__global__ __launch_bounds__(256) void k_layernorm_g8(const f16 *__restrict__ x, const f16 *__restrict__ gamma, const f16 *__restrict__ beta,
                                                      int64_t rows, float eps, f16 *__restrict__ y)
{
    constexpr int C = 64 * KC;
    const int lane = threadIdx.x & 63, s = lane & 7, rw = lane >> 3;
    const int64_t wave = ((int64_t)blockIdx.x * 256 + threadIdx.x) >> 6;
    const int64_t row = wave * 8 + rw;
    const bool live = row < rows;
    const f16 *xr = x + (live ? row : rows - 1) * C + s * 8;
    f16x8 v[KC];
#pragma unroll
    for (int k = 0; k < KC; ++k) v[k] = *(const f16x8 *)(xr + k * 64);
    f16x8 ga[KC], be[KC];
#pragma unroll
    for (int k = 0; k < KC; ++k) {
        ga[k] = *(const f16x8 *)(gamma + k * 64 + s * 8);
        be[k] = *(const f16x8 *)(beta + k * 64 + s * 8);
    }
    float sum = 0.f;
#pragma unroll
    for (int k = 0; k < KC; ++k)
#pragma unroll
        for (int j = 0; j < 8; ++j) sum += (float)v[k][j];
    const float mean = sum8_dpp(sum) / (float)C;
    float q = 0.f;
#pragma unroll
    for (int k = 0; k < KC; ++k)
#pragma unroll
        for (int j = 0; j < 8; ++j) { const float d = (float)v[k][j] - mean; q += d * d; }
    const float rstd = rsqrtf(sum8_dpp(q) / (float)C + eps);
    if (!live) return;
    f16 *yr = y + row * C + s * 8;
#pragma unroll
    for (int k = 0; k < KC; ++k) {
        f16x8 o;
#pragma unroll
        for (int j = 0; j < 8; ++j) o[j] = (f16)(((float)v[k][j] - mean) * rstd * (float)ga[k][j] + (float)be[k][j]);
        *(f16x8 *)(yr + k * 64) = o;
    }
}

extern "C" int32_t ctx_layernorm_f16(const void *x, const void *gamma, const void *beta, int64_t rows, int32_t C, float eps,
                                     void *y, ctx_stream_t stream)
{
    return ctx_layernorm_any(x, 0, gamma, beta, rows, C, eps, y, (hipStream_t)stream);
}

int ctx_layernorm_any(const void *x, int x32, const void *gamma, const void *beta, int64_t rows, int C, float eps, void *y, hipStream_t stream)
{
    CTX_REQUIRE(x && gamma && beta && y && rows > 0 && C % 8 == 0 && C <= 2048, "layernorm: unsupported rows=%lld C=%d", (long long)rows, C);
    {
        static const int g8 = [] { const char *e = getenv("CTX_LN_G8"); return e ? atoi(e) : 1; }();
        if (g8 && !x32 && C % 64 == 0 && C <= 640 && rows >= 64) {
            const unsigned nb = (unsigned)cdiv64(cdiv64(rows, 8), 4);
#define LN_G8(KC_) case KC_: hipLaunchKernelGGL(k_layernorm_g8<KC_>, dim3(nb), dim3(256), 0, stream, (const f16 *)x, (const f16 *)gamma, (const f16 *)beta, rows, eps, (f16 *)y); break
            switch (C / 64) {
                LN_G8(1); LN_G8(2); LN_G8(3); LN_G8(4); LN_G8(5); LN_G8(6); LN_G8(7); LN_G8(8); LN_G8(9); LN_G8(10);
            }
#undef LN_G8
            CTX_CHECK_LAUNCH("layernorm");
            return CTX_OK;
        }
    }
    const int kc = (C / 8 + 63) / 64;
#define LN_GO(KC_, R_) do { int64_t nb = cdiv64(cdiv64(rows, R_), 4); \
        if (x32) hipLaunchKernelGGL((k_layernorm<KC_, R_, true>), dim3((unsigned)nb), dim3(256), 0, stream, x, \
                           (const f16 *)gamma, (const f16 *)beta, rows, C, eps, (f16 *)y); \
        else hipLaunchKernelGGL((k_layernorm<KC_, R_, false>), dim3((unsigned)nb), dim3(256), 0, stream, x, \
                           (const f16 *)gamma, (const f16 *)beta, rows, C, eps, (f16 *)y); } while (0)
    const bool many = rows >= 8192;
    if (kc == 1) { if (many) LN_GO(1, 4); else LN_GO(1, 1); }
    else if (kc == 2) { if (many) LN_GO(2, 2); else LN_GO(2, 1); }
    else if (kc == 3) LN_GO(3, 1);
    else LN_GO(4, 1);
#undef LN_GO
    CTX_CHECK_LAUNCH("layernorm");
    return CTX_OK;
}

__global__ __launch_bounds__(256) void k_geglu(const f16 *__restrict__ h, int64_t M, int C4, f16 *__restrict__ y)
{
    const int c8n = C4 / 8;
    const int64_t total = M * c8n;
    for (int64_t i = (int64_t)blockIdx.x * 256 + threadIdx.x; i < total; i += (int64_t)gridDim.x * 256) {
        int64_t m = i / c8n;
        int c8 = (int)(i % c8n);
        f16x8 a = *(const f16x8 *)(h + m * 2 * C4 + c8 * 8);
        f16x8 g = *(const f16x8 *)(h + m * 2 * C4 + C4 + c8 * 8);
        f16x8 o;
#pragma unroll
        for (int j = 0; j < 8; ++j) {
            float gf = (float)g[j];
            o[j] = (f16)((float)a[j] * (0.5f * gf * (1.0f + erff(gf * 0.70710678118654752f))));
        }
        *(f16x8 *)(y + m * C4 + c8 * 8) = o;
    }
}

extern "C" int32_t ctx_geglu_f16(const void *h, int64_t M, int32_t C4, void *y, ctx_stream_t stream)
{
    CTX_REQUIRE(h && y && M > 0 && C4 % 8 == 0, "geglu: bad args");
    int64_t nb = cdiv64(M * (C4 / 8), 256);
    if (nb > 4096) nb = 4096;
    hipLaunchKernelGGL(k_geglu, dim3((unsigned)nb), dim3(256), 0, (hipStream_t)stream, (const f16 *)h, M, C4, (f16 *)y);
    CTX_CHECK_LAUNCH("geglu");
    return CTX_OK;
}

__global__ __launch_bounds__(256) void k_concat(const f16 *__restrict__ a, const f16 *__restrict__ b, int64_t M, int Ca,
                                                int Cb, f16 *__restrict__ y)
{
    const int n8 = (Ca + Cb) / 8, a8 = Ca / 8;
    const int64_t total = M * n8;
    for (int64_t i = (int64_t)blockIdx.x * 256 + threadIdx.x; i < total; i += (int64_t)gridDim.x * 256) {
        int64_t m = i / n8;
        int c8 = (int)(i % n8);
        f16x8 v = c8 < a8 ? *(const f16x8 *)(a + m * Ca + c8 * 8) : *(const f16x8 *)(b + m * Cb + (c8 - a8) * 8);
        *(f16x8 *)(y + i * 8) = v;
    }
}

int ctx_concat_f32(const float *a, const float *b, int64_t M, int Ca, int Cb, float *y, hipStream_t s)
{
    return ctx_concat_f16((const f16 *)a, (const f16 *)b, M, 2 * Ca, 2 * Cb, (f16 *)y, s);
}

int ctx_concat_f16(const f16 *a, const f16 *b, int64_t M, int Ca, int Cb, f16 *y, hipStream_t s)
{
    int64_t nb = cdiv64(M * ((Ca + Cb) / 8), 256);
    if (nb > 4096) nb = 4096;
    hipLaunchKernelGGL(k_concat, dim3((unsigned)nb), dim3(256), 0, s, a, b, M, Ca, Cb, y);
    return CTX_OK;
}

__global__ __launch_bounds__(256) void k_transpose_v(const f16 *__restrict__ v, int S, int ld, int heads, int Sp, int perm,
                                                     f16 *__restrict__ vt)
{
    __shared__ f16 tile[64][66];
    const int b = blockIdx.z, hd = blockIdx.y, s0 = blockIdx.x * 64;
    for (int i = 0; i < 2; ++i) {
        int key = (threadIdx.x >> 3) + 32 * i, c = threadIdx.x & 7;
        f16x8 val = {0, 0, 0, 0, 0, 0, 0, 0};
        if (s0 + key < S) val = *(const f16x8 *)(v + ((size_t)b * S + s0 + key) * ld + hd * 64 + c * 8);
#pragma unroll
        for (int j = 0; j < 8; ++j) tile[key][c * 8 + j] = val[j];
    }
    __syncthreads();
    for (int i = 0; i < 2; ++i) {
        int d = (threadIdx.x >> 3) + 32 * i, c = threadIdx.x & 7;
        f16x8 o;
#pragma unroll
        for (int j = 0; j < 8; ++j) o[j] = perm ? tile[16 * (c >> 1) + 8 * (j >> 2) + 4 * (c & 1) + (j & 3)][d] : tile[c * 8 + j][d];
        if (s0 + c * 8 < Sp) *(f16x8 *)(vt + (((size_t)b * heads + hd) * 64 + d) * Sp + s0 + c * 8) = o;
    }
}

int ctx_transpose_v_f16(const f16 *v, int B, int S, int ld, int heads, int Sp, int perm, f16 *vt, hipStream_t s)
{
    hipLaunchKernelGGL(k_transpose_v, dim3(cdiv(Sp, 64), heads, B), dim3(256), 0, s, v, S, ld, heads, Sp, perm, vt);
    return CTX_OK;
}

__global__ __launch_bounds__(256) void k_f32_to_f16(const float *__restrict__ x, int64_t n, f16 *__restrict__ y)
{
    for (int64_t i = (int64_t)blockIdx.x * 256 + threadIdx.x; i < n; i += (int64_t)gridDim.x * 256) y[i] = (f16)x[i];
}
__global__ __launch_bounds__(256) void k_f16_to_f32(const f16 *__restrict__ x, int64_t n8, float *__restrict__ y)
{
    for (int64_t i = (int64_t)blockIdx.x * 256 + threadIdx.x; i < n8; i += (int64_t)gridDim.x * 256) {
        const f16x8 v = *(const f16x8 *)(x + i * 8);
        f32x4 a = {(float)v[0], (float)v[1], (float)v[2], (float)v[3]}, b = {(float)v[4], (float)v[5], (float)v[6], (float)v[7]};
        *(f32x4 *)(y + i * 8) = a; *(f32x4 *)(y + i * 8 + 4) = b;
    }
}
int ctx_f16_to_f32(const f16 *x, int64_t n, float *y, hipStream_t s)
{
    int64_t nb = cdiv64(n / 8, 256);
    if (nb > 4096) nb = 4096;
    hipLaunchKernelGGL(k_f16_to_f32, dim3((unsigned)nb), dim3(256), 0, s, x, n / 8, y);
    return CTX_OK;
}
int ctx_f32_to_f16(const float *x, int64_t n, f16 *y, hipStream_t s)
{
    int64_t nb = cdiv64(n, 256);
    if (nb > 2048) nb = 2048;
    hipLaunchKernelGGL(k_f32_to_f16, dim3((unsigned)nb), dim3(256), 0, s, x, n, y);
    return CTX_OK;
}

__global__ void k_time_embed(const float *__restrict__ t, int B, int dim, f16 *__restrict__ out)
{
    int i = blockIdx.x * blockDim.x + threadIdx.x;
    int half = dim / 2;
    if (i >= half) return;
    float fr = expf(-9.210340371976184f * (float)i / (float)half);
    float a = t[0] * fr;
    float c = cosf(a), sn = sinf(a);
    for (int b = 0; b < B; ++b) {
        out[(size_t)b * dim + i] = (f16)c;
        out[(size_t)b * dim + half + i] = (f16)sn;
    }
}
int ctx_time_embed_f16(const float *t, int B, int dim, f16 *out, hipStream_t s)
{
    hipLaunchKernelGGL(k_time_embed, dim3(cdiv(dim / 2, 64)), dim3(64), 0, s, t, B, dim, out);
    return CTX_OK;
}

#define CI_SPLIT 16
template <int CP, int CX>
__global__ __launch_bounds__(256) void k_conv_in(const float *__restrict__ x, const f16 *__restrict__ w,
                                                 const f16 *__restrict__ bias, int B, int Cin, int H, int W, int Cout,
                                                 f16 *__restrict__ y)
{
    extern __shared__ __attribute__((aligned(16))) float s_w[];
    constexpr int WR = 9 * CP, WX = 9 * CX;
    const int o8n = Cout / 8;
    const int o8_per = (o8n + CI_SPLIT - 1) / CI_SPLIT;
    const int o8_0 = blockIdx.y * o8_per, o8_1 = min(o8n, o8_0 + o8_per);
    const int no = (o8_1 - o8_0) * 8;
    for (int i = threadIdx.x; i < no * WX; i += 256) {
        const int o = i / WX, r = i - o * WX, t = r / CX, c = r - t * CX;
        s_w[i] = (float)w[(size_t)(o8_0 * 8 + o) * WR + t * CP + c];
    }
    __syncthreads();
    const int64_t npix = (int64_t)B * H * W;
    const int64_t pix0 = (int64_t)blockIdx.x * 256;
    const int64_t pix = pix0 + threadIdx.x;
    const bool live = pix < npix;
    const int64_t pq = live ? pix : npix - 1;
    int b = (int)(pq / (H * W)), p = (int)(pq % (H * W));
    int oy = p / W, ox = p % W;
    float in[9][CX];
#pragma unroll
    for (int t = 0; t < 9; ++t) {
        int iy = oy + t / 3 - 1, ix = ox + t % 3 - 1;
        bool ok = iy >= 0 && iy < H && ix >= 0 && ix < W;
#pragma unroll
        for (int c = 0; c < CX; ++c)
            in[t][c] = (ok && c < Cin) ? (float)(f16)x[(((size_t)b * Cin + c) * H + iy) * W + ix] : 0.f;
    }
    f16 *patch = (f16 *)(s_w + no * WX);
    for (int g0 = o8_0; g0 < o8_1; g0 += 8) {
        const int ng = min(8, o8_1 - g0);
        for (int gi = 0; gi < ng; ++gi) {
            const int o8 = g0 + gi;
            f16x8 o;
#pragma unroll
            for (int j = 0; j < 8; ++j) {
                const float *wr = s_w + ((o8 - o8_0) * 8 + j) * WX;
                float acc = (float)bias[o8 * 8 + j];
#pragma unroll
                for (int t = 0; t < 9; ++t)
#pragma unroll
                    for (int c = 0; c < CX; ++c) acc += in[t][c] * wr[t * CX + c];
                o[j] = (f16)acc;
            }
            *(f16x8 *)(patch + threadIdx.x * 72 + gi * 8) = o;
        }
        __syncthreads();
        for (int ch = threadIdx.x; ch < 256 * ng; ch += 256) {
            const int px = ch / ng, gi = ch - px * ng;
            if (pix0 + px < npix) *(f16x8 *)(y + (pix0 + px) * Cout + (g0 + gi) * 8) = *(const f16x8 *)(patch + px * 72 + gi * 8);
        }
        __syncthreads();
    }
}
int ctx_conv_in_f16(const float *x, const f16 *w, const f16 *bias, int B, int Cin, int H, int W, int Cout, f16 *y, hipStream_t s)
{
    int64_t npix = (int64_t)B * H * W;
    int o8_per = (Cout / 8 + CI_SPLIT - 1) / CI_SPLIT;
    const dim3 grid((unsigned)cdiv64(npix, 256), CI_SPLIT);
#define CI_GO(CP_, CX_) hipLaunchKernelGGL((k_conv_in<CP_, CX_>), grid, dim3(256), (size_t)o8_per * 8 * 9 * CX_ * sizeof(float) + 256 * 72 * sizeof(f16), s, x, w, bias, B, Cin, H, W, Cout, y)
    if (Cin <= 3) CI_GO(8, 3);
    else if (Cin == 4) CI_GO(8, 4);
    else if (Cin == 5) CI_GO(8, 5);
    else if (Cin <= 8) CI_GO(8, 8);
    else if (Cin == 9) CI_GO(16, 9);
    else CI_GO(16, 16);
#undef CI_GO
    return CTX_OK;
}

template <int NU, bool WF32>
__global__ __launch_bounds__(256) void k_conv_out(const f16 *__restrict__ x, const f16 *__restrict__ w,
                                                  const f16 *__restrict__ bias, int B, int H, int W, int C, int Cout,
                                                  float *__restrict__ out)
{
    extern __shared__ __attribute__((aligned(16))) char s_cw_raw[];
    f16 *s_cw = (f16 *)s_cw_raw;
    float *s_cf = (float *)s_cw_raw;
    const int nwt = Cout * 9 * C;
    if (WF32) {
        for (int i = threadIdx.x * 8; i < nwt; i += 256 * 8) {
            const f16x8 v = *(const f16x8 *)(w + i);
#pragma unroll
            for (int j = 0; j < 8; ++j) s_cf[i + j] = (float)v[j];
        }
    } else {
        for (int i = threadIdx.x * 8; i < nwt; i += 256 * 8) *(f16x8 *)(s_cw + i) = *(const f16x8 *)(w + i);
    }
    __syncthreads();
    const int lane = threadIdx.x & 63;
    const int c8n = C / 8, nitems = 9 * c8n;
    const int64_t npix = (int64_t)B * H * W;
    const f16x8 zero8 = {0, 0, 0, 0, 0, 0, 0, 0};
    int itap[NU], ic[NU];
#pragma unroll
    for (int u = 0; u < NU; ++u) {
        const int i = min(lane + 64 * u, nitems - 1);
        itap[u] = i / c8n; ic[u] = (i - itap[u] * c8n) * 8;
    }
    const int64_t pstep = ((int64_t)gridDim.x * 256) >> 6;
    f16x8 xn[NU];
    auto fetch = [&](int64_t pp_) {
        const int64_t q = pp_ < npix ? pp_ : npix - 1;
        const int b = (int)(q / (H * W)), p = (int)(q % (H * W));
        const int oy = p / W, ox = p % W;
#pragma unroll
        for (int u = 0; u < NU; ++u) {
            const int iy = oy + itap[u] / 3 - 1, ix = ox + itap[u] % 3 - 1;
            const int cy = min(max(iy, 0), H - 1), cx = min(max(ix, 0), W - 1);
            xn[u] = *(const f16x8 *)(x + (((size_t)b * H + cy) * W + cx) * C + ic[u]);
            if (lane + 64 * u >= nitems || iy != cy || ix != cx) xn[u] = zero8;
        }
    };
    int64_t pix = ((int64_t)blockIdx.x * 256 + threadIdx.x) >> 6;
    if (pix < npix) fetch(pix);
    for (; pix < npix; pix += pstep) {
        const int b = (int)(pix / (H * W)), p = (int)(pix % (H * W));
        const int oy = p / W, ox = p % W;
        f16x8 xv[NU];
#pragma unroll
        for (int u = 0; u < NU; ++u) xv[u] = xn[u];
        if (pix + pstep < npix) fetch(pix + pstep);
        float acc[4] = {0.f, 0.f, 0.f, 0.f};
#pragma unroll
        for (int u = 0; u < NU; ++u) {
            float xf[8];
#pragma unroll
            for (int j = 0; j < 8; ++j) xf[j] = (float)xv[u][j];
#pragma unroll
            for (int o = 0; o < 4; ++o) {
                if (o < Cout) {
                    if (WF32) {
                        const float *wr = s_cf + itap[u] * C + ic[u] + o * 9 * C;
                        const f32x4 w0 = *(const f32x4 *)wr, w1 = *(const f32x4 *)(wr + 4);
#pragma unroll
                        for (int j = 0; j < 4; ++j) { acc[o] += xf[j] * w0[j]; }
#pragma unroll
                        for (int j = 0; j < 4; ++j) { acc[o] += xf[4 + j] * w1[j]; }
                    } else {
                        const f16x8 wv = *(const f16x8 *)(s_cw + itap[u] * C + ic[u] + o * 9 * C);
#pragma unroll
                        for (int j = 0; j < 8; ++j) acc[o] += xf[j] * (float)wv[j];
                    }
                }
            }
        }
#pragma unroll
        for (int o = 0; o < 4; ++o) {
            if (o < Cout) {
                float v = wave_sum_dpp(acc[o]);
                if (lane == 0) out[(((size_t)b * Cout + o) * H + oy) * W + ox] = v + (float)bias[o];
            }
        }
    }
}
int ctx_conv_out_f16(const f16 *x, const f16 *w, const f16 *bias, int B, int H, int W, int C, int Cout, float *out, hipStream_t s)
{
    int64_t nb = cdiv64((int64_t)B * H * W, 4);
    if (nb > 2048) nb = 2048;
    const int nitems = 9 * (C / 8);
    const size_t lds16 = (size_t)Cout * 9 * C * sizeof(f16);
    if (Cout > 4 || C % 8 != 0 || nitems > 64 * 12 || lds16 > 64 * 1024) {
        ctx_set_error("conv_out: unsupported C=%d Cout=%d", C, Cout);
        return CTX_E_ARG;
    }
    const bool f32w = 2 * lds16 <= 64 * 1024;
    const size_t lds = f32w ? 2 * lds16 : lds16;
#define CO_GO(NU_) do { if (f32w) hipLaunchKernelGGL((k_conv_out<NU_, true>), dim3((unsigned)nb), dim3(256), lds, s, x, w, bias, B, H, W, C, Cout, out); \
                        else hipLaunchKernelGGL((k_conv_out<NU_, false>), dim3((unsigned)nb), dim3(256), lds, s, x, w, bias, B, H, W, C, Cout, out); } while (0)
    if (nitems <= 64 * 3) CO_GO(3);
    else if (nitems <= 64 * 6) CO_GO(6);
    else CO_GO(12);
#undef CO_GO
    return CTX_OK;
}

__global__ __launch_bounds__(256) void k_cfg_plms(const float *__restrict__ eps_pair, int64_t n, float guidance,
                                                  float *__restrict__ ets, int head, float c0, float c1, float c2,
                                                  float c3, float sample_coeff, float eps_coeff, int mode,
                                                  float *__restrict__ cur, float *__restrict__ x)
{
    for (int64_t i = (int64_t)blockIdx.x * 256 + threadIdx.x; i < n; i += (int64_t)gridDim.x * 256) {
        float eu = eps_pair[i], et = eps_pair[n + i];
        float e = eu + guidance * (et - eu);
        float xs;
        float comb;
        if (mode == 1) {
            comb = (e + ets[(size_t)head * n + i]) / 2.0f;
            xs = cur[i];
        } else {
            ets[(size_t)head * n + i] = e;
            float e1 = ets[(size_t)((head + 3) & 3) * n + i];
            float e2 = ets[(size_t)((head + 2) & 3) * n + i];
            float e3 = ets[(size_t)((head + 1) & 3) * n + i];
            comb = c0 * e;
            if (c1 != 0.f) comb += c1 * e1;
            if (c2 != 0.f) comb += c2 * e2;
            if (c3 != 0.f) comb += c3 * e3;
            xs = x[i];
            if (mode == 2) cur[i] = xs;
        }
        x[i] = sample_coeff * xs - eps_coeff * comb;
    }
}

extern "C" int32_t ctx_cfg_plms_step(const float *eps_pair, int64_t n, float guidance, float *ets, int32_t head,
                                     const float *coef4, float sample_coeff, float eps_coeff, int32_t mode,
                                     float *cur_sample_ws, float *x, ctx_stream_t stream)
{
    CTX_REQUIRE(eps_pair && ets && coef4 && x && n > 0 && head >= 0 && head < 4, "cfg_plms_step: bad args");
    CTX_REQUIRE(mode == 0 || cur_sample_ws, "cfg_plms_step: mode %d needs cur_sample_ws", mode);
    int64_t nb = cdiv64(n, 256);
    if (nb > 2048) nb = 2048;
    hipLaunchKernelGGL(k_cfg_plms, dim3((unsigned)nb), dim3(256), 0, (hipStream_t)stream, eps_pair, n, guidance, ets, head,
                       coef4[0], coef4[1], coef4[2], coef4[3], sample_coeff, eps_coeff, mode, cur_sample_ws, x);
    CTX_CHECK_LAUNCH("cfg_plms_step");
    return CTX_OK;
}
```

contexture-nerf_amd/csrc/unet.hip:

```cpp
#include "common.h"
#include "kernels.h"
#include <string>
#include <vector>
#include <string.h>

enum PackKind { PK_COPY = 0, PK_CONV3 = 1, PK_CONVIN = 2, PK_GEGLU_W = 3, PK_GEGLU_B = 4 };

struct Param {
    std::string name;
    int ndim;
    int64_t shape[4];
    int kind;
    size_t dst;
    int a, b;
};

struct ResP {
    int cin, cout;
    size_t n1g, n1b, c1w, c1b, n2g, n2b, c2w, c2b, scw, scb;
    int temb_row;
};
struct TrP {
    int C, heads;
    size_t ng, nb, piw, pib, l1g, l1b, qkv, o1w, o1b, l2g, l2b, q2, kv2, o2w, o2b, l3g, l3b, f1w, f1b, f2w, f2b, pow_, pob;
    int kv_row;
};
struct LevelP {
    std::vector<ResP> res;
    std::vector<TrP> tr;
    bool has_attn = false, has_sampler = false;
    size_t sw = 0, sb = 0;
    int sc = 0;
};

struct ctx_unet {
    ctx_unet_config_t cfg;
    std::vector<Param> params;
    size_t wtop = 0;
    size_t ciw, cib, t1w, t1b, t2w, t2b, tpw, tpb, cng, cnb, cow, cob;
    int temb_dim = 0, temb_rows = 0;
    size_t kvw = 0;
    int kv_rows_total = 0, kv_rows = 0;
    std::vector<LevelP> down, up;
    LevelP mid;
    f16 *W = nullptr;
    char *ws = nullptr;
    size_t ws_cap = 0;
    size_t top = 0, peak = 0;
    bool dry = false;
    hipStream_t s = nullptr;
    int rc = 0;
    int64_t launches[3] = {0, 0, 0};
    double flops[3] = {0, 0, 0};
    struct RefSlot { size_t off; int tokens, C, rows; };
    int ref_mode = 0;
    f16 *ref_bank = nullptr;
    size_t ref_cursor = 0;
    int ref_k = 0, ref_row0 = 0;
    std::vector<RefSlot> ref_slots;
    bool is_controlnet = false;
    int cond_channels = 3;
    struct CondConv { size_t w, b; int cin, cout, stride; };
    std::vector<CondConv> cond_convs;
    std::vector<size_t> zc_w, zc_b;
    std::vector<int> zc_c;
    size_t zm_w = 0, zm_b = 0;
    const float *cn_cond = nullptr;
    f16 *cn_cache = nullptr;
    bool cn_cache_valid = false;
    f16 *cn_out = nullptr;
    const f16 *add_res = nullptr;
    float add_scale = 1.0f;
    bool res32 = false;
    void *allocS(size_t n) { return alloc(n * (res32 ? 4 : 2)); }
    struct Tap { size_t off; int rows, C; };
    f16 *tap_buf = nullptr;
    size_t tap_cap = 0, tap_cursor = 0;
    std::vector<Tap> taps;
    void tap(const void *x, int rows, int C)
    {
        if (!tap_buf || res32) return;
        const size_t n = (size_t)rows * C;
        Tap t = {tap_cursor, rows, C};
        taps.push_back(t);
        if (!dry && rc == 0 && tap_cursor + n <= tap_cap) (void)hipMemcpyAsync(tap_buf + tap_cursor, x, n * 2, hipMemcpyDeviceToDevice, s);
        tap_cursor += n;
    }

    size_t walloc(size_t n) { size_t o = wtop; wtop += (n + 127) / 128 * 128; return o; }
    size_t add(const std::string &name, std::vector<int64_t> shp, int kind, size_t dst, int a = 0, int b = 0)
    {
        Param p; p.name = name; p.ndim = (int)shp.size(); p.kind = kind; p.dst = dst; p.a = a; p.b = b;
        for (int i = 0; i < 4; ++i) p.shape[i] = i < p.ndim ? shp[i] : 1;
        params.push_back(p);
        return dst;
    }
    size_t vec(const std::string &name, int n) { return add(name, {n}, PK_COPY, walloc(n)); }
    size_t lin(const std::string &name, int out, int in) { return add(name, {out, in}, PK_COPY, walloc((size_t)out * in)); }

    void *alloc(size_t bytes)
    {
        size_t o = (top + 255) / 256 * 256;
        top = o + bytes;
        if (top > peak) peak = top;
        if (!dry && top > ws_cap) { rc = CTX_E_STATE; ctx_set_error("unet: workspace too small (%zu > %zu)", top, ws_cap); return ws; }
        return dry ? nullptr : (void *)(ws + o);
    }
    f16 *allocH(size_t n) { return (f16 *)alloc(n * 2); }
};

static void add_resnet(ctx_unet *u, const std::string &p, int cin, int cout, ResP &r)
{
    r.cin = cin; r.cout = cout;
    r.n1g = u->vec(p + ".norm1.weight", cin); r.n1b = u->vec(p + ".norm1.bias", cin);
    r.c1w = u->add(p + ".conv1.weight", {cout, cin, 3, 3}, PK_CONV3, u->walloc((size_t)cout * cin * 9), cout, cin);
    r.c1b = u->vec(p + ".conv1.bias", cout);
    r.temb_row = u->temb_rows;
    u->add(p + ".time_emb_proj.weight", {cout, u->temb_dim}, PK_COPY, u->tpw + (size_t)u->temb_rows * u->temb_dim);
    u->add(p + ".time_emb_proj.bias", {cout}, PK_COPY, u->tpb + u->temb_rows);
    u->temb_rows += cout;
    r.n2g = u->vec(p + ".norm2.weight", cout); r.n2b = u->vec(p + ".norm2.bias", cout);
    r.c2w = u->add(p + ".conv2.weight", {cout, cout, 3, 3}, PK_CONV3, u->walloc((size_t)cout * cout * 9), cout, cout);
    r.c2b = u->vec(p + ".conv2.bias", cout);
    if (cin != cout) {
        r.scw = u->add(p + ".conv_shortcut.weight", {cout, cin, 1, 1}, PK_COPY, u->walloc((size_t)cout * cin));
        r.scb = u->vec(p + ".conv_shortcut.bias", cout);
    } else r.scw = r.scb = 0;
}

static void add_transformer(ctx_unet *u, const std::string &p, int C, int heads, TrP &t)
{
    int cd = u->cfg.cross_attention_dim;
    t.C = C; t.heads = heads;
    t.ng = u->vec(p + ".norm.weight", C); t.nb = u->vec(p + ".norm.bias", C);
    t.piw = u->lin(p + ".proj_in.weight", C, C); t.pib = u->vec(p + ".proj_in.bias", C);
    std::string b = p + ".transformer_blocks.0";
    t.l1g = u->vec(b + ".norm1.weight", C); t.l1b = u->vec(b + ".norm1.bias", C);
    t.qkv = u->walloc((size_t)3 * C * C);
    u->add(b + ".attn1.to_q.weight", {C, C}, PK_COPY, t.qkv);
    u->add(b + ".attn1.to_k.weight", {C, C}, PK_COPY, t.qkv + (size_t)C * C);
    u->add(b + ".attn1.to_v.weight", {C, C}, PK_COPY, t.qkv + (size_t)2 * C * C);
    t.o1w = u->lin(b + ".attn1.to_out.0.weight", C, C); t.o1b = u->vec(b + ".attn1.to_out.0.bias", C);
    t.l2g = u->vec(b + ".norm2.weight", C); t.l2b = u->vec(b + ".norm2.bias", C);
    t.q2 = u->lin(b + ".attn2.to_q.weight", C, C);
    t.kv_row = u->kv_rows;
    t.kv2 = u->kvw + (size_t)u->kv_rows * cd;
    u->kv_rows += 2 * C;
    u->add(b + ".attn2.to_k.weight", {C, cd}, PK_COPY, t.kv2);
    u->add(b + ".attn2.to_v.weight", {C, cd}, PK_COPY, t.kv2 + (size_t)C * cd);
    t.o2w = u->lin(b + ".attn2.to_out.0.weight", C, C); t.o2b = u->vec(b + ".attn2.to_out.0.bias", C);
    t.l3g = u->vec(b + ".norm3.weight", C); t.l3b = u->vec(b + ".norm3.bias", C);
    t.f1w = u->add(b + ".ff.net.0.proj.weight", {8 * C, C}, PK_GEGLU_W, u->walloc((size_t)8 * C * C), 4 * C, C);
    t.f1b = u->add(b + ".ff.net.0.proj.bias", {8 * C}, PK_GEGLU_B, u->walloc((size_t)8 * C), 4 * C, 0);
    t.f2w = u->lin(b + ".ff.net.2.weight", C, 4 * C); t.f2b = u->vec(b + ".ff.net.2.bias", C);
    t.pow_ = u->lin(p + ".proj_out.weight", C, C); t.pob = u->vec(p + ".proj_out.bias", C);
}

static ctx_unet_t *unet_create_impl(const ctx_unet_config_t *cfg, bool controlnet, int cond_channels)
{
    if (!cfg || cfg->n_levels < 1 || cfg->n_levels > 4 || cfg->in_channels > 16 || cfg->out_channels > 4 ||
        cfg->groups > 64 || cfg->layers_per_block < 1 || cfg->layers_per_block > 4 || cfg->cross_attention_dim % 64) {
        ctx_set_error("unet_create: unsupported config");
        return nullptr;
    }
    for (int i = 0; i < cfg->n_levels; ++i)
        if (cfg->block_out_channels[i] % 64 || cfg->block_out_channels[i] % cfg->groups || cfg->heads[i] * 64 != cfg->block_out_channels[i]) {
            ctx_set_error("unet_create: level %d: channels %d must be a multiple of 64 and of groups, with head_dim 64 (heads=%d)",
                          i, cfg->block_out_channels[i], cfg->heads[i]);
            return nullptr;
        }
    ctx_unet *u = new ctx_unet();
    u->cfg = *cfg;
    const int n = cfg->n_levels, lpb = cfg->layers_per_block;
    const int *ch = cfg->block_out_channels;
    u->temb_dim = ch[0] * 4;
    int rows = 0;
    u->is_controlnet = controlnet; u->cond_channels = cond_channels;
    for (int i = 0; i < n; ++i) rows += lpb * ch[i];
    rows += 2 * ch[n - 1];
    if (!controlnet)
        for (int i = 0; i < n; ++i) rows += (lpb + 1) * ch[n - 1 - i];
    u->tpw = u->walloc((size_t)rows * u->temb_dim);
    u->tpb = u->walloc(rows);
    {
        int kvr = 2 * ch[n - 1];
        for (int i = 0; i < n; ++i) {
            if (cfg->down_attn[i]) kvr += lpb * 2 * ch[i];
            if (cfg->up_attn[i] && !controlnet) kvr += (lpb + 1) * 2 * ch[n - 1 - i];
        }
        u->kv_rows_total = kvr;
        u->kvw = u->walloc((size_t)kvr * cfg->cross_attention_dim);
    }

    u->ciw = u->add("conv_in.weight", {ch[0], cfg->in_channels, 3, 3}, PK_CONVIN, u->walloc((size_t)ch[0] * 9 * (cfg->in_channels > 8 ? 16 : 8)), ch[0],
                    cfg->in_channels);
    u->cib = u->vec("conv_in.bias", ch[0]);
    u->t1w = u->lin("time_embedding.linear_1.weight", u->temb_dim, ch[0]); u->t1b = u->vec("time_embedding.linear_1.bias", u->temb_dim);
    u->t2w = u->lin("time_embedding.linear_2.weight", u->temb_dim, u->temb_dim); u->t2b = u->vec("time_embedding.linear_2.bias", u->temb_dim);
    u->down.resize(n);
    int out = ch[0];
    for (int i = 0; i < n; ++i) {
        LevelP &L = u->down[i];
        int cin = out; out = ch[i];
        std::string p = "down_blocks." + std::to_string(i);
        L.res.resize(lpb);
        for (int j = 0; j < lpb; ++j) add_resnet(u, p + ".resnets." + std::to_string(j), j == 0 ? cin : out, out, L.res[j]);
        L.has_attn = cfg->down_attn[i] != 0;
        if (L.has_attn) {
            L.tr.resize(lpb);
            for (int j = 0; j < lpb; ++j) add_transformer(u, p + ".attentions." + std::to_string(j), out, cfg->heads[i], L.tr[j]);
        }
        if (i != n - 1) {
            L.has_sampler = true; L.sc = out;
            L.sw = u->add(p + ".downsamplers.0.conv.weight", {out, out, 3, 3}, PK_CONV3, u->walloc((size_t)out * out * 9), out, out);
            L.sb = u->vec(p + ".downsamplers.0.conv.bias", out);
        }
    }
    {
        LevelP &L = u->mid;
        L.res.resize(2); L.tr.resize(1); L.has_attn = true;
        add_resnet(u, "mid_block.resnets.0", ch[n - 1], ch[n - 1], L.res[0]);
        add_transformer(u, "mid_block.attentions.0", ch[n - 1], cfg->heads[n - 1], L.tr[0]);
        add_resnet(u, "mid_block.resnets.1", ch[n - 1], ch[n - 1], L.res[1]);
    }
    if (!controlnet) {
        u->up.resize(n);
        out = ch[n - 1];
        for (int i = 0; i < n; ++i) {
            LevelP &L = u->up[i];
            int prev = out; out = ch[n - 1 - i];
            int inp = ch[n - 1 - (i + 1 < n ? i + 1 : n - 1)];
            std::string p = "up_blocks." + std::to_string(i);
            L.res.resize(lpb + 1);
            for (int j = 0; j <= lpb; ++j) {
                int skip = j == lpb ? inp : out;
                int rin = j == 0 ? prev : out;
                add_resnet(u, p + ".resnets." + std::to_string(j), rin + skip, out, L.res[j]);
            }
            L.has_attn = cfg->up_attn[i] != 0;
            if (L.has_attn) {
                L.tr.resize(lpb + 1);
                for (int j = 0; j <= lpb; ++j) add_transformer(u, p + ".attentions." + std::to_string(j), out, cfg->heads[n - 1 - i], L.tr[j]);
            }
            if (i != n - 1) {
                L.has_sampler = true; L.sc = out;
                L.sw = u->add(p + ".upsamplers.0.conv.weight", {out, out, 3, 3}, PK_CONV3, u->walloc((size_t)out * out * 9), out, out);
                L.sb = u->vec(p + ".upsamplers.0.conv.bias", out);
            }
        }
        u->cng = u->vec("conv_norm_out.weight", ch[0]); u->cnb = u->vec("conv_norm_out.bias", ch[0]);
        u->cow = u->add("conv_out.weight", {cfg->out_channels, ch[0], 3, 3}, PK_CONV3, u->walloc((size_t)cfg->out_channels * ch[0] * 9), cfg->out_channels, ch[0]);
        u->cob = u->vec("conv_out.bias", cfg->out_channels);
    } else {
        const int cc[4] = {16, 32, 96, 256};
        const std::string e = "controlnet_cond_embedding";
        auto addc = [&](const std::string &name, int cin, int cout, int stride) {
            ctx_unet::CondConv c; c.cin = cin; c.cout = cout; c.stride = stride;
            c.w = u->add(name + ".weight", {cout, cin, 3, 3}, PK_CONV3, u->walloc((size_t)cout * cin * 9), cout, cin);
            c.b = u->vec(name + ".bias", cout);
            u->cond_convs.push_back(c);
        };
        addc(e + ".conv_in", cond_channels, cc[0], 1);
        for (int i = 0; i < 3; ++i) {
            addc(e + ".blocks." + std::to_string(2 * i), cc[i], cc[i], 1);
            addc(e + ".blocks." + std::to_string(2 * i + 1), cc[i], cc[i + 1], 2);
        }
        addc(e + ".conv_out", cc[3], ch[0], 1);
        std::vector<int> skc; skc.push_back(ch[0]);
        for (int i = 0; i < n; ++i) {
            for (int j = 0; j < lpb; ++j) skc.push_back(ch[i]);
            if (i != n - 1) skc.push_back(ch[i]);
        }
        for (size_t k = 0; k < skc.size(); ++k) {
            std::string p = "controlnet_down_blocks." + std::to_string(k);
            u->zc_w.push_back(u->add(p + ".weight", {skc[k], skc[k], 1, 1}, PK_COPY, u->walloc((size_t)skc[k] * skc[k])));
            u->zc_b.push_back(u->vec(p + ".bias", skc[k]));
            u->zc_c.push_back(skc[k]);
        }
        u->zm_w = u->add("controlnet_mid_block.weight", {ch[n - 1], ch[n - 1], 1, 1}, PK_COPY, u->walloc((size_t)ch[n - 1] * ch[n - 1]));
        u->zm_b = u->vec("controlnet_mid_block.bias", ch[n - 1]);
    }
    if (u->kv_rows != u->kv_rows_total) {
        ctx_set_error("unet_create: internal cross-attention K/V row count mismatch %d != %d", u->kv_rows, u->kv_rows_total);
        delete u;
        return nullptr;
    }
    if (u->temb_rows != rows) {
        ctx_set_error("unet_create: internal temb row count mismatch %d != %d", u->temb_rows, rows);
        delete u;
        return nullptr;
    }
    return u;
}

extern "C" ctx_unet_t *ctx_unet_create(const ctx_unet_config_t *cfg) { return unet_create_impl(cfg, false, 0); }
extern "C" ctx_unet_t *ctx_controlnet_create(const ctx_unet_config_t *cfg, int32_t cond_channels)
{
    if (cond_channels < 1 || cond_channels > 8) { ctx_set_error("controlnet_create: cond_channels=%d outside [1,8]", cond_channels); return nullptr; }
    return unet_create_impl(cfg, true, cond_channels);
}
extern "C" void ctx_unet_destroy(ctx_unet_t *u) { delete u; }
extern "C" int32_t ctx_unet_param_count(const ctx_unet_t *u) { return u ? (int32_t)u->params.size() : 0; }
extern "C" const char *ctx_unet_param_name(const ctx_unet_t *u, int32_t i)
{
    return (u && i >= 0 && i < (int)u->params.size()) ? u->params[i].name.c_str() : "";
}
extern "C" int32_t ctx_unet_param_shape(const ctx_unet_t *u, int32_t i, int64_t shape4[4])
{
    if (!u || i < 0 || i >= (int)u->params.size()) return 0;
    for (int k = 0; k < 4; ++k) shape4[k] = u->params[i].shape[k];
    return u->params[i].ndim;
}
extern "C" int64_t ctx_unet_weight_bytes(const ctx_unet_t *u) { return u ? (int64_t)u->wtop * 2 + 256 : 0; }

extern "C" int32_t ctx_unet_bind(ctx_unet_t *u, void *weights, void *workspace, int64_t workspace_bytes)
{
    CTX_REQUIRE(u && weights && workspace && workspace_bytes > 0, "unet_bind: bad args");
    CTX_REQUIRE(((uintptr_t)weights & 255) == 0 && ((uintptr_t)workspace & 255) == 0, "unet_bind: blobs must be 256-byte aligned");
    u->W = (f16 *)weights; u->ws = (char *)workspace; u->ws_cap = (size_t)workspace_bytes;
    return CTX_OK;
}

__global__ void k_pack_copy(const float *__restrict__ s, int64_t n, f16 *__restrict__ d)
{
    for (int64_t i = (int64_t)blockIdx.x * 256 + threadIdx.x; i < n; i += (int64_t)gridDim.x * 256) d[i] = (f16)s[i];
}
__global__ void k_pack_conv3(const float *__restrict__ s, int Cout, int Cin, int Cinp, f16 *__restrict__ d)
{
    int64_t n = (int64_t)Cout * 9 * Cinp;
    for (int64_t i = (int64_t)blockIdx.x * 256 + threadIdx.x; i < n; i += (int64_t)gridDim.x * 256) {
        int c = (int)(i % Cinp);
        int tap = (int)((i / Cinp) % 9);
        int o = (int)(i / ((int64_t)Cinp * 9));
        d[i] = c < Cin ? (f16)s[((int64_t)o * Cin + c) * 9 + tap] : (f16)0.f;
    }
}
__global__ void k_pack_geglu(const float *__restrict__ s, int C4, int K, f16 *__restrict__ d)
{
    int64_t n = (int64_t)2 * C4 * (K > 0 ? K : 1);
    int kk = K > 0 ? K : 1;
    for (int64_t i = (int64_t)blockIdx.x * 256 + threadIdx.x; i < n; i += (int64_t)gridDim.x * 256) {
        int k = (int)(i % kk);
        int p = (int)(i / kk);
        int blk = p / 64, w = p % 64;
        int src = w < 32 ? blk * 32 + w : C4 + blk * 32 + (w - 32);
        d[i] = (f16)s[(int64_t)src * kk + k];
    }
}

extern "C" int32_t ctx_unet_set_param(ctx_unet_t *u, int32_t i, const float *src, ctx_stream_t stream)
{
    CTX_REQUIRE(u && u->W && src && i >= 0 && i < (int)u->params.size(), "unet_set_param: bad args / not bound");
    const Param &p = u->params[i];
    hipStream_t s = (hipStream_t)stream;
    int64_t n = 1;
    for (int k = 0; k < p.ndim; ++k) n *= p.shape[k];
    f16 *d = u->W + p.dst;
    int64_t nbk = cdiv64(n, 256);
    unsigned nb = (unsigned)(nbk > 4096 ? 4096 : nbk);
    switch (p.kind) {
    case PK_COPY: hipLaunchKernelGGL(k_pack_copy, dim3(nb), dim3(256), 0, s, src, n, d); break;
    case PK_CONV3: hipLaunchKernelGGL(k_pack_conv3, dim3(nb), dim3(256), 0, s, src, p.a, p.b, p.b, d); break;
    case PK_CONVIN: hipLaunchKernelGGL(k_pack_conv3, dim3(nb), dim3(256), 0, s, src, p.a, p.b, p.b > 8 ? 16 : 8, d); break;
    case PK_GEGLU_W: hipLaunchKernelGGL(k_pack_geglu, dim3(nb), dim3(256), 0, s, src, p.a, p.b, d); break;
    case PK_GEGLU_B: hipLaunchKernelGGL(k_pack_geglu, dim3(nb), dim3(256), 0, s, src, p.a, 0, d); break;
    }
    CTX_CHECK_LAUNCH("unet_set_param");
    return CTX_OK;
}

__global__ __launch_bounds__(256) void k_conv_small(const float *__restrict__ x32, const f16 *__restrict__ x16, const f16 *__restrict__ w,
                                                    const f16 *__restrict__ bias, int B, int H, int W, int Cin, int Cout, int stride,
                                                    int silu, f16 *__restrict__ y)
{
    const int Ho = (H - 1) / stride + 1, Wo = (W - 1) / stride + 1, o8n = Cout / 8;
    const int64_t total = (int64_t)B * Ho * Wo * o8n;
    for (int64_t i = (int64_t)blockIdx.x * 256 + threadIdx.x; i < total; i += (int64_t)gridDim.x * 256) {
        const int o8 = (int)(i % o8n);
        const int64_t pix = i / o8n;
        const int b = (int)(pix / ((int64_t)Ho * Wo)), p = (int)(pix % ((int64_t)Ho * Wo));
        const int oy = p / Wo, ox = p % Wo;
        float acc[8];
#pragma unroll
        for (int j = 0; j < 8; ++j) acc[j] = (float)bias[o8 * 8 + j];
        for (int t = 0; t < 9; ++t) {
            const int iy = oy * stride + t / 3 - 1, ix = ox * stride + t % 3 - 1;
            if (iy < 0 || iy >= H || ix < 0 || ix >= W) continue;
            if (x16 && (Cin & 7) == 0) {
                const f16 *xp = x16 + (((int64_t)b * H + iy) * W + ix) * Cin;
                const f16 *wp = w + ((int64_t)(o8 * 8) * 9 + t) * Cin;
                for (int c = 0; c < Cin; c += 8) {
                    const f16x8 xv = *(const f16x8 *)(xp + c);
                    float xf[8];
#pragma unroll
                    for (int q = 0; q < 8; ++q) xf[q] = (float)xv[q];
#pragma unroll
                    for (int j = 0; j < 8; ++j) {
                        const f16x8 wv = *(const f16x8 *)(wp + (int64_t)j * 9 * Cin + c);
#pragma unroll
                        for (int q = 0; q < 8; ++q) acc[j] += xf[q] * (float)wv[q];
                    }
                }
                continue;
            }
            for (int c = 0; c < Cin; ++c) {
                const float v = x32 ? (float)(f16)x32[(((int64_t)b * Cin + c) * H + iy) * W + ix]
                                    : (float)x16[(((int64_t)b * H + iy) * W + ix) * Cin + c];
#pragma unroll
                for (int j = 0; j < 8; ++j) acc[j] += v * (float)w[(((int64_t)(o8 * 8 + j)) * 9 + t) * Cin + c];
            }
        }
        f16x8 o;
#pragma unroll
        for (int j = 0; j < 8; ++j) {
            float v = acc[j];
            if (silu) v = v / (1.0f + __expf(-v));
            o[j] = (f16)v;
        }
        *(f16x8 *)(y + pix * Cout + o8 * 8) = o;
    }
}

__global__ __launch_bounds__(256) void k_add_scaled_f16(f16 *__restrict__ dst, const f16 *__restrict__ src, float scale, int64_t n8)
{
    for (int64_t i = (int64_t)blockIdx.x * 256 + threadIdx.x; i < n8; i += (int64_t)gridDim.x * 256) {
        f16x8 a = *(const f16x8 *)(dst + i * 8), b = *(const f16x8 *)(src + i * 8);
#pragma unroll
        for (int j = 0; j < 8; ++j) a[j] = (f16)((float)a[j] + scale * (float)b[j]);
        *(f16x8 *)(dst + i * 8) = a;
    }
}

static void note(ctx_unet *u, int klass, double fl, int n = 1) { u->launches[klass] += n; u->flops[klass] += fl; }
#define RUN(expr) do { if (!u->dry && u->rc == 0) { int r__ = (expr); if (r__ != 0) u->rc = r__; } } while (0)

static void op_gemm(ctx_unet *u, const f16 *X, size_t w, size_t bias, bool has_bias, const void *res, int M, int N, int K, void *out,
                    int epi = 0, bool res_s = false, bool out_s = false)
{
    GemmArgs a = {};
    a.X = X; a.Wt = u->W + w; a.bias = has_bias ? u->W + bias : nullptr; a.residual = (const f16 *)res; a.out = (f16 *)out;
    a.M = M; a.N = N; a.K = K; a.ldc = epi == 1 ? N / 2 : N; a.ldr = N; a.rows_per_batch = 1; a.ldrb = N; a.epi = epi;
    a.res32 = (u->res32 && res_s && res) ? 1 : 0; a.out32 = (u->res32 && out_s) ? 1 : 0;
    note(u, 0, 2.0 * M * N * K);
    size_t mark = u->top;
    ctx_gemm_plan(a, false);
    if (a.splitk > 1) a.part = (float *)u->alloc((size_t)a.splitk * M * N * 4);
    RUN(ctx_gemm_dispatch(a, false, u->s));
    u->top = mark;
}
static void op_conv(ctx_unet *u, const f16 *x, size_t w, size_t bias, const f16 *rowbias, int ldrb, const void *res, int B, int H,
                    int W, int Cin, int Cout, int stride, int ups, void *out, bool res_s = false, bool out_s = false)
{
    GemmArgs a = {};
    int Hv = H << ups, Wv = W << ups;
    a.Ho = (Hv - 1) / stride + 1; a.Wo = (Wv - 1) / stride + 1;
    a.X = x; a.Wt = u->W + w; a.bias = u->W + bias; a.rowbias = rowbias; a.residual = (const f16 *)res; a.out = (f16 *)out;
    a.M = B * a.Ho * a.Wo; a.N = Cout; a.K = 9 * Cin; a.ldc = Cout; a.ldr = Cout; a.rows_per_batch = a.Ho * a.Wo; a.ldrb = ldrb;
    a.H = H; a.W = W; a.Cin = Cin; a.stride = stride; a.ups = ups;
    a.res32 = (u->res32 && res_s && res) ? 1 : 0; a.out32 = (u->res32 && out_s) ? 1 : 0;
    note(u, 0, 2.0 * a.M * a.N * a.K);
    size_t mark = u->top;
    ctx_gemm_plan(a, true);
    if (a.splitk > 1) a.part = (float *)u->alloc((size_t)a.splitk * a.M * a.N * 4);
    RUN(ctx_gemm_dispatch(a, true, u->s));
    u->top = mark;
}
static void op_gn(ctx_unet *u, const void *x, size_t g, size_t b, int B, int HW, int C, float eps, int silu, f16 *y, void *stats, bool x_s = true)
{
    note(u, 2, 0, 2);
    RUN(ctx_groupnorm_any(x, (u->res32 && x_s) ? 1 : 0, u->W + g, u->W + b, B, HW, C, u->cfg.groups, eps, silu, y, stats, u->s));
}
static void op_ln(ctx_unet *u, const void *x, size_t g, size_t b, int64_t rows, int C, f16 *y)
{
    note(u, 2, 0);
    RUN(ctx_layernorm_any(x, u->res32 ? 1 : 0, u->W + g, u->W + b, rows, C, 1e-5f, y, u->s));
}
static const f16 *op_as16(ctx_unet *u, const void *x, size_t n)
{
    if (!u->res32) return (const f16 *)x;
    f16 *c = u->allocH(n);
    note(u, 2, 0);
    RUN(ctx_f32_to_f16((const float *)x, (int64_t)n, c, u->s));
    return c;
}
static void op_attn(ctx_unet *u, const f16 *Q, const f16 *K, const f16 *V, int B, int Sq, int Skv, int heads, int qs, int kvs, f16 *O)
{
    note(u, 1, 4.0 * B * heads * (double)Sq * Skv * 64);
    RUN(ctx_attention_core(Q, K, V, B, Sq, Skv, heads, qs, kvs, 0.125f, O, heads * 64, u->s));
}

struct FwdCtx {
    int B, L;
    const f16 *tproj;
    const f16 *ctx16;
    const f16 *kv_all;
    void *gn_stats;
};

static void *run_resnet(ctx_unet *u, const FwdCtx &f, const ResP &r, const void *x, int H, int W, void *out)
{
    const int B = f.B, HW = H * W, M = B * HW;
    size_t mark = u->top;
    f16 *t1 = u->allocH((size_t)M * r.cin);
    op_gn(u, x, r.n1g, r.n1b, B, HW, r.cin, u->cfg.norm_eps, 1, t1, f.gn_stats);
    f16 *h = u->allocH((size_t)M * r.cout);
    op_conv(u, t1, r.c1w, r.c1b, f.tproj ? f.tproj + r.temb_row : nullptr, u->temb_rows, nullptr, B, H, W, r.cin, r.cout, 1, 0, h);
    f16 *t2 = u->allocH((size_t)M * r.cout);
    op_gn(u, h, r.n2g, r.n2b, B, HW, r.cout, u->cfg.norm_eps, 1, t2, f.gn_stats, false);
    const void *sc = x;
    if (r.cin != r.cout) {
        void *s2 = u->allocS((size_t)M * r.cout);
        op_gemm(u, op_as16(u, x, (size_t)M * r.cin), r.scw, r.scb, true, nullptr, M, r.cout, r.cin, s2, 0, false, true);
        sc = s2;
    }
    op_conv(u, t2, r.c2w, r.c2b, nullptr, 0, sc, B, H, W, r.cout, r.cout, 1, 0, out, true, true);
    u->top = mark;
    return out;
}

static void *run_transformer(ctx_unet *u, const FwdCtx &f, const TrP &t, const void *x, int H, int W, void *out)
{
    const int B = f.B, S = H * W, M = B * S, C = t.C, cd = u->cfg.cross_attention_dim;
    size_t mark = u->top;
    f16 *g = u->allocH((size_t)M * C);
    op_gn(u, x, t.ng, t.nb, B, S, C, 1e-6f, 0, g, f.gn_stats);
    void *h0 = u->allocS((size_t)M * C);
    op_gemm(u, g, t.piw, t.pib, true, nullptr, M, C, C, h0, 0, false, true);
    f16 *l = g;
    op_ln(u, h0, t.l1g, t.l1b, M, C, l);
    f16 *a = nullptr;
    if (u->ref_mode == 2) {
        if (u->ref_k >= (int)u->ref_slots.size() || u->ref_slots[u->ref_k].C != C ||
            u->ref_slots[u->ref_k].rows != B - u->ref_row0) {
            u->rc = CTX_E_STATE;
            ctx_set_error("unet: the reference bank does not match this pass (run the 'w' pass on the condition latent first; layer %d)", u->ref_k);
            u->top = mark;
            return out;
        }
        const ctx_unet::RefSlot sl = u->ref_slots[u->ref_k++];
        f16 *q = u->allocH((size_t)M * C);
        op_gemm(u, l, t.qkv, 0, false, nullptr, M, C, C, q);
        a = u->allocH((size_t)M * C);
        f16 *kv = u->allocH((size_t)(S + sl.tokens) * 2 * C);
        for (int b = 0; b < B; ++b) {
            const int Sr = b >= u->ref_row0 ? sl.tokens : 0;
            op_gemm(u, l ? l + (size_t)b * S * C : nullptr, t.qkv + (size_t)C * C, 0, false, nullptr, S, 2 * C, C, kv);
            if (Sr)
                op_gemm(u, u->ref_bank ? u->ref_bank + sl.off + (size_t)(b - u->ref_row0) * sl.tokens * C : nullptr,
                        t.qkv + (size_t)C * C, 0, false, nullptr, Sr, 2 * C, C, kv ? kv + (size_t)S * 2 * C : nullptr);
            op_attn(u, q ? q + (size_t)b * S * C : nullptr, kv, kv ? kv + C : nullptr, 1, S, S + Sr, t.heads, C, 2 * C,
                    a ? a + (size_t)b * S * C : nullptr);
        }
    } else {
        if (u->ref_mode == 1) {
            ctx_unet::RefSlot sl; sl.off = u->ref_cursor; sl.tokens = S; sl.C = C; sl.rows = B;
            u->ref_slots.push_back(sl);
            u->ref_cursor += (size_t)M * C;
            if (!u->dry && u->rc == 0 && u->ref_bank)
                (void)hipMemcpyAsync(u->ref_bank + sl.off, l, (size_t)M * C * 2, hipMemcpyDeviceToDevice, u->s);
        }
        f16 *qkv = u->allocH((size_t)M * 3 * C);
        op_gemm(u, l, t.qkv, 0, false, nullptr, M, 3 * C, C, qkv);
        a = u->allocH((size_t)M * C);
        op_attn(u, qkv, qkv + C, qkv + 2 * C, B, S, S, t.heads, 3 * C, 3 * C, a);
    }
    void *h1 = u->allocS((size_t)M * C);
    op_gemm(u, a, t.o1w, t.o1b, true, h0, M, C, C, h1, 0, true, true);
    op_ln(u, h1, t.l2g, t.l2b, M, C, l);
    f16 *q = a;
    op_gemm(u, l, t.q2, 0, false, nullptr, M, C, C, q);
    const f16 *kv = f.kv_all + t.kv_row;
    f16 *a2 = u->allocH((size_t)M * C);
    op_attn(u, q, kv, kv + C, B, S, f.L, t.heads, C, u->kv_rows_total, a2);
    void *h2 = h0;
    op_gemm(u, a2, t.o2w, t.o2b, true, h1, M, C, C, h2, 0, true, true);
    op_ln(u, h2, t.l3g, t.l3b, M, C, l);
    f16 *ff = u->allocH((size_t)M * 4 * C);
    op_gemm(u, l, t.f1w, t.f1b, true, nullptr, M, 8 * C, C, ff, 1);
    void *h3 = h1;
    op_gemm(u, ff, t.f2w, t.f2b, true, h2, M, C, 4 * C, h3, 0, true, true);
    op_gemm(u, op_as16(u, h3, (size_t)M * C), t.pow_, t.pob, true, x, M, C, C, out, 0, true, true);
    u->top = mark;
    return out;
}

static int unet_run(ctx_unet *u, const float *sample, const float *timestep, const float *ctx, int B, int H, int W, int L, float *out)
{
    const ctx_unet_config_t &c = u->cfg;
    const int n = c.n_levels, lpb = c.layers_per_block;
    const int *ch = c.block_out_channels;
    u->top = 0; u->peak = 0; u->rc = 0;
    u->ref_k = 0; u->ref_cursor = 0;
    u->taps.clear(); u->tap_cursor = 0;
    if (u->ref_mode == 1) u->ref_slots.clear();
    for (int k = 0; k < 3; ++k) { u->launches[k] = 0; u->flops[k] = 0; }
    FwdCtx f; f.B = B; f.L = L;
    f.gn_stats = u->alloc((size_t)ctx_groupnorm_ws_bytes(B, c.groups));
    f16 *te0 = u->allocH((size_t)B * ch[0]);
    note(u, 2, 0); RUN(ctx_time_embed_f16(timestep, B, ch[0], te0, u->s));
    f16 *te1 = u->allocH((size_t)B * u->temb_dim);
    note(u, 2, 2.0 * B * ch[0] * u->temb_dim); RUN(ctx_gemv_f16(te0, u->W + u->t1w, u->W + u->t1b, B, u->temb_dim, ch[0], 0, 1, te1, u->s));
    f16 *te2 = u->allocH((size_t)B * u->temb_dim);
    note(u, 2, 2.0 * B * u->temb_dim * u->temb_dim); RUN(ctx_gemv_f16(te1, u->W + u->t2w, u->W + u->t2b, B, u->temb_dim, u->temb_dim, 0, 1, te2, u->s));
    f16 *tproj = u->allocH((size_t)B * u->temb_rows);
    note(u, 2, 2.0 * B * u->temb_rows * u->temb_dim); RUN(ctx_gemv_f16(te2, u->W + u->tpw, u->W + u->tpb, B, u->temb_rows, u->temb_dim, 0, 0, tproj, u->s));
    f.tproj = tproj;
    f16 *ctx16 = u->allocH((size_t)B * L * c.cross_attention_dim);
    note(u, 2, 0); RUN(ctx_f32_to_f16(ctx, (int64_t)B * L * c.cross_attention_dim, ctx16, u->s));
    f.ctx16 = ctx16;
    f16 *kv_all = u->allocH((size_t)B * L * u->kv_rows_total);
    op_gemm(u, ctx16, u->kvw, 0, false, nullptr, B * L, u->kv_rows_total, c.cross_attention_dim, kv_all);
    f.kv_all = kv_all;

    int h = H, w = W;
    if (u->res32 && (u->is_controlnet || u->add_res || u->ref_mode)) {
        ctx_set_error("unet: the fp32 residual-stream mode covers the plain UNet forward only");
        return CTX_E_STATE;
    }
    void *x = u->allocS((size_t)B * h * w * ch[0]);
    {
        size_t m0 = u->top;
        f16 *x16 = u->res32 ? u->allocH((size_t)B * h * w * ch[0]) : (f16 *)x;
        note(u, 2, 2.0 * B * h * w * ch[0] * c.in_channels * 9); RUN(ctx_conv_in_f16(sample, u->W + u->ciw, u->W + u->cib, B, c.in_channels, h, w, ch[0], x16, u->s));
        if (u->res32) { note(u, 2, 0); RUN(ctx_f16_to_f32(x16, (int64_t)B * h * w * ch[0], (float *)x, u->s)); u->top = m0; }
    }

    auto add_scaled = [&](f16 *dst, const f16 *src, float scale, size_t n) {
        note(u, 2, 0);
        if (!u->dry && u->rc == 0)
            hipLaunchKernelGGL(k_add_scaled_f16, dim3((unsigned)std::min<int64_t>(cdiv64((int64_t)n / 8, 256), 4096)), dim3(256), 0, u->s, dst, src,
                               scale, (int64_t)n / 8);
    };
    if (u->is_controlnet) {
        size_t mark = u->top;
        int eh = 8 * H, ew = 8 * W;
        const f16 *cur16 = nullptr;
        const size_t nconv = u->cond_convs.size();
        for (size_t k = 0; k + 1 < nconv; ++k) {
            const ctx_unet::CondConv &cc = u->cond_convs[k];
            int oh = (eh - 1) / cc.stride + 1, ow = (ew - 1) / cc.stride + 1;
            const bool last = k + 2 == nconv;
            f16 *o = (last && u->cn_cache) ? u->cn_cache : u->allocH((size_t)B * oh * ow * cc.cout);
            if (!u->cn_cache_valid) {
                note(u, 2, 2.0 * B * oh * ow * cc.cout * cc.cin * 9);
                if (!u->dry && u->rc == 0) {
                    int64_t items = (int64_t)B * oh * ow * (cc.cout / 8);
                    hipLaunchKernelGGL(k_conv_small, dim3((unsigned)std::min<int64_t>(cdiv64(items, 256), 65535)), dim3(256), 0, u->s,
                                       k == 0 ? u->cn_cond : nullptr, cur16, u->W + cc.w, u->W + cc.b, B, eh, ew, cc.cin, cc.cout, cc.stride, 1, o);
                }
            }
            cur16 = o; eh = oh; ew = ow;
        }
        if (eh != h || ew != w) { ctx_set_error("controlnet: conditioning embedding grid %dx%d != latent grid %dx%d", eh, ew, h, w); return CTX_E_ARG; }
        const ctx_unet::CondConv &co = u->cond_convs.back();
        f16 *emb = u->allocH((size_t)B * h * w * ch[0]);
        op_conv(u, cur16, co.w, co.b, nullptr, 0, x, B, h, w, co.cin, ch[0], 1, 0, emb);
        if (!u->dry && u->rc == 0) (void)hipMemcpyAsync(x, emb, (size_t)B * h * w * ch[0] * 2, hipMemcpyDeviceToDevice, u->s);
        u->top = mark;
    }
    struct Skip { void *p; int C, h, w; };
    std::vector<Skip> skips;
    skips.push_back({x, ch[0], h, w});
    u->tap(x, B * h * w, ch[0]);
    int cur = ch[0];
    for (int i = 0; i < n; ++i) {
        LevelP &Lv = u->down[i];
        for (int j = 0; j < lpb; ++j) {
            int cout = Lv.res[j].cout;
            void *o = u->allocS((size_t)B * h * w * cout);
            if (Lv.has_attn) {
                size_t mark = u->top;
                void *t = u->allocS((size_t)B * h * w * cout);
                run_resnet(u, f, Lv.res[j], x, h, w, t);
                u->tap(t, B * h * w, cout);
                run_transformer(u, f, Lv.tr[j], t, h, w, o);
                u->top = mark;
            } else run_resnet(u, f, Lv.res[j], x, h, w, o);
            u->tap(o, B * h * w, cout);
            x = o; cur = cout;
            skips.push_back({x, cur, h, w});
        }
        if (Lv.has_sampler) {
            int ho = (h - 1) / 2 + 1, wo = (w - 1) / 2 + 1;
            void *o = u->allocS((size_t)B * ho * wo * cur);
            size_t m0 = u->top;
            op_conv(u, op_as16(u, x, (size_t)B * h * w * cur), Lv.sw, Lv.sb, nullptr, 0, nullptr, B, h, w, cur, cur, 2, 0, o, false, true);
            u->top = m0;
            x = o; h = ho; w = wo;
            u->tap(x, B * h * w, cur);
            skips.push_back({x, cur, h, w});
        }
    }
    size_t res_off = 0;
    if (u->is_controlnet) {
        if (skips.size() != u->zc_w.size()) { ctx_set_error("controlnet: %zu skip tensors but %zu zero convolutions", skips.size(), u->zc_w.size()); return CTX_E_STATE; }
        for (size_t k = 0; k < skips.size(); ++k) {
            const Skip &sk = skips[k];
            const size_t nel = (size_t)B * sk.h * sk.w * sk.C;
            op_gemm(u, (const f16 *)sk.p, u->zc_w[k], u->zc_b[k], true, nullptr, B * sk.h * sk.w, sk.C, sk.C, u->cn_out ? u->cn_out + res_off : nullptr);
            res_off += nel;
        }
    } else if (u->add_res) {
        for (size_t k = 0; k < skips.size(); ++k) {
            Skip &sk = skips[k];
            const size_t nel = (size_t)B * sk.h * sk.w * sk.C;
            if (sk.p == x) {
                f16 *cp = u->allocH(nel);
                if (!u->dry && u->rc == 0) (void)hipMemcpyAsync(cp, sk.p, nel * 2, hipMemcpyDeviceToDevice, u->s);
                sk.p = cp;
            }
            add_scaled((f16 *)sk.p, u->add_res + res_off, u->add_scale, nel);
            res_off += nel;
        }
    }
    {
        void *o1 = u->allocS((size_t)B * h * w * cur);
        run_resnet(u, f, u->mid.res[0], x, h, w, o1);
        u->tap(o1, B * h * w, cur);
        void *o2 = u->allocS((size_t)B * h * w * cur);
        run_transformer(u, f, u->mid.tr[0], o1, h, w, o2);
        u->tap(o2, B * h * w, cur);
        void *o3 = u->allocS((size_t)B * h * w * cur);
        run_resnet(u, f, u->mid.res[1], o2, h, w, o3);
        u->tap(o3, B * h * w, cur);
        x = o3;
    }
    if (u->is_controlnet) {
        op_gemm(u, (const f16 *)x, u->zm_w, u->zm_b, true, nullptr, B * h * w, cur, cur, u->cn_out ? u->cn_out + res_off : nullptr);
        res_off += (size_t)B * h * w * cur;
        u->ref_cursor = res_off;
        if (!u->dry && u->rc == 0) {
            hipError_t e = hipGetLastError();
            if (e != hipSuccess) { ctx_set_error("controlnet_forward: launch failed: %s", hipGetErrorString(e)); return CTX_E_LAUNCH; }
        }
        return u->rc;
    }
    if (u->add_res) add_scaled((f16 *)x, u->add_res + res_off, u->add_scale, (size_t)B * h * w * cur);
    for (int i = 0; i < n; ++i) {
        LevelP &Lv = u->up[i];
        for (int j = 0; j <= lpb; ++j) {
            Skip sk = skips.back(); skips.pop_back();
            if (sk.h != h || sk.w != w) { ctx_set_error("unet: skip size mismatch (H, W must be multiples of %d)", 1 << (n - 1)); return CTX_E_ARG; }
            int cin = cur + sk.C, cout = Lv.res[j].cout;
            void *o = u->allocS((size_t)B * h * w * cout);
            size_t mark = u->top;
            void *cat = u->allocS((size_t)B * h * w * cin);
            note(u, 2, 0);
            if (u->res32) RUN(ctx_concat_f32((const float *)x, (const float *)sk.p, (int64_t)B * h * w, cur, sk.C, (float *)cat, u->s));
            else RUN(ctx_concat_f16((const f16 *)x, (const f16 *)sk.p, (int64_t)B * h * w, cur, sk.C, (f16 *)cat, u->s));
            if (Lv.has_attn) {
                void *t = u->allocS((size_t)B * h * w * cout);
                run_resnet(u, f, Lv.res[j], cat, h, w, t);
                u->tap(t, B * h * w, cout);
                run_transformer(u, f, Lv.tr[j], t, h, w, o);
            } else run_resnet(u, f, Lv.res[j], cat, h, w, o);
            u->tap(o, B * h * w, cout);
            u->top = mark;
            x = o; cur = cout;
        }
        if (Lv.has_sampler) {
            void *o = u->allocS((size_t)B * (2 * h) * (2 * w) * cur);
            size_t m0 = u->top;
            op_conv(u, op_as16(u, x, (size_t)B * h * w * cur), Lv.sw, Lv.sb, nullptr, 0, nullptr, B, h, w, cur, cur, 1, 1, o, false, true);
            u->top = m0;
            x = o; h *= 2; w *= 2;
            u->tap(x, B * h * w, cur);
        }
    }
    f16 *y = u->allocH((size_t)B * h * w * cur);
    op_gn(u, x, u->cng, u->cnb, B, h * w, cur, c.norm_eps, 1, y, f.gn_stats);
    note(u, 2, 2.0 * B * h * w * cur * c.out_channels * 9);
    RUN(ctx_conv_out_f16(y, u->W + u->cow, u->W + u->cob, B, h, w, cur, c.out_channels, out, u->s));
    if (!u->dry && u->rc == 0) {
        hipError_t e = hipGetLastError();
        if (e != hipSuccess) { ctx_set_error("unet_forward: launch failed: %s", hipGetErrorString(e)); return CTX_E_LAUNCH; }
    }
    return u->rc;
}

static int check_dims(const ctx_unet *u, int B, int H, int W, int L)
{
    int div = 1 << (u->cfg.n_levels - 1);
    if (B < 1 || B > 16 || H < div || W < div || H % div || W % div || L < 1) {
        ctx_set_error("unet: need 1<=B<=16, H,W multiples of %d, ctx_len>=1 (B=%d H=%d W=%d L=%d)", div, B, H, W, L);
        return CTX_E_ARG;
    }
    return 0;
}

extern "C" int64_t ctx_unet_workspace_bytes(const ctx_unet_t *cu, int32_t B, int32_t H, int32_t W, int32_t ctx_len)
{
    ctx_unet *u = const_cast<ctx_unet *>(cu);
    if (!u || check_dims(u, B, H, W, ctx_len)) return -1;
    bool was = u->dry;
    u->dry = true;
    unet_run(u, nullptr, nullptr, nullptr, B, H, W, ctx_len, nullptr);
    u->dry = was;
    return (int64_t)u->peak + 4096;
}

extern "C" int32_t ctx_unet_forward(ctx_unet_t *u, const float *sample, const float *timestep, const float *ctx, int32_t B,
                                    int32_t H, int32_t W, int32_t ctx_len, float *out, ctx_stream_t stream)
{
    CTX_REQUIRE(u && sample && timestep && ctx && out, "unet_forward: null pointer");
    CTX_REQUIRE(u->W && u->ws, "unet_forward: ctx_unet_bind() first");
    if (check_dims(u, B, H, W, ctx_len)) return CTX_E_ARG;
    u->s = (hipStream_t)stream;
    u->dry = false;
    return unet_run(u, sample, timestep, ctx, B, H, W, ctx_len, out);
}

extern "C" int64_t ctx_controlnet_residual_bytes(const ctx_unet_t *cu, int32_t B, int32_t H, int32_t W)
{
    ctx_unet *u = const_cast<ctx_unet *>(cu);
    if (!u || !u->is_controlnet || check_dims(u, B, H, W, 1)) return -1;
    bool was = u->dry;
    u->dry = true;
    int rc = unet_run(u, nullptr, nullptr, nullptr, B, H, W, 1, nullptr);
    u->dry = was;
    return rc ? -1 : (int64_t)u->ref_cursor * 2 + 256;
}

extern "C" int64_t ctx_controlnet_cond_cache_bytes(const ctx_unet_t *u, int32_t B, int32_t H, int32_t W)
{
    if (!u || !u->is_controlnet || B < 1 || H < 1 || W < 1 || u->cond_convs.size() < 2) return -1;
    return (int64_t)B * H * W * u->cond_convs[u->cond_convs.size() - 2].cout * 2 + 256;
}

extern "C" int32_t ctx_controlnet_forward(ctx_unet_t *u, const float *sample, const float *timestep, const float *ctx, const float *cond,
                                          void *cond_cache, int32_t cache_valid, int32_t B, int32_t H, int32_t W, int32_t ctx_len,
                                          void *residuals, ctx_stream_t stream)
{
    CTX_REQUIRE(u && sample && timestep && ctx && cond && residuals, "controlnet_forward: null pointer");
    CTX_REQUIRE(!cache_valid || cond_cache, "controlnet_forward: cache_valid without a cond_cache buffer");
    CTX_REQUIRE(u->is_controlnet, "controlnet_forward: the handle is a UNet (create it with ctx_controlnet_create)");
    CTX_REQUIRE(u->W && u->ws, "controlnet_forward: ctx_unet_bind() first");
    if (check_dims(u, B, H, W, ctx_len)) return CTX_E_ARG;
    u->s = (hipStream_t)stream; u->dry = false;
    u->cn_cond = cond; u->cn_out = (f16 *)residuals; u->cn_cache = (f16 *)cond_cache; u->cn_cache_valid = cache_valid != 0;
    int rc = unet_run(u, sample, timestep, ctx, B, H, W, ctx_len, nullptr);
    u->cn_cond = nullptr; u->cn_out = nullptr; u->cn_cache = nullptr; u->cn_cache_valid = false;
    return rc;
}

extern "C" int32_t ctx_unet_set_residuals(ctx_unet_t *u, const void *residuals, float scale)
{
    CTX_REQUIRE(u && !u->is_controlnet, "unet_set_residuals: need a UNet handle");
    u->add_res = (const f16 *)residuals; u->add_scale = scale;
    return CTX_OK;
}

extern "C" int64_t ctx_unet_ref_bank_bytes(const ctx_unet_t *cu, int32_t B, int32_t H, int32_t W)
{
    ctx_unet *u = const_cast<ctx_unet *>(cu);
    if (!u || check_dims(u, B, H, W, 1)) return -1;
    std::vector<ctx_unet::RefSlot> keep = u->ref_slots;
    bool was = u->dry; int mode = u->ref_mode;
    u->dry = true; u->ref_mode = 1;
    unet_run(u, nullptr, nullptr, nullptr, B, H, W, 1, nullptr);
    int64_t n = (int64_t)u->ref_cursor * 2 + 256;
    u->dry = was; u->ref_mode = mode; u->ref_slots = keep;
    return n;
}

extern "C" int64_t ctx_unet_workspace_bytes_ref(const ctx_unet_t *cu, int32_t B, int32_t H, int32_t W, int32_t ctx_len, int32_t mode,
                                                int32_t ref_row0)
{
    ctx_unet *u = const_cast<ctx_unet *>(cu);
    if (!u || check_dims(u, B, H, W, ctx_len) || mode < 1 || mode > 2 || ref_row0 < 0 || ref_row0 >= B) return -1;
    std::vector<ctx_unet::RefSlot> keep = u->ref_slots;
    bool was = u->dry; int m0 = u->ref_mode, r0 = u->ref_row0;
    u->dry = true; u->ref_mode = mode; u->ref_row0 = ref_row0;
    int rc = unet_run(u, nullptr, nullptr, nullptr, B, H, W, ctx_len, nullptr);
    int64_t n = rc ? -1 : (int64_t)u->peak + 4096;
    u->dry = was; u->ref_mode = m0; u->ref_row0 = r0;
    if (mode == 1) u->ref_slots = keep;
    return n;
}

extern "C" int32_t ctx_unet_forward_ref(ctx_unet_t *u, const float *sample, const float *timestep, const float *ctx, int32_t B,
                                        int32_t H, int32_t W, int32_t ctx_len, int32_t mode, void *bank, int32_t ref_row0, float *out,
                                        ctx_stream_t stream)
{
    CTX_REQUIRE(u && sample && timestep && ctx && out && bank, "unet_forward_ref: null pointer");
    CTX_REQUIRE(u->W && u->ws, "unet_forward_ref: ctx_unet_bind() first");
    CTX_REQUIRE(mode == 1 || mode == 2, "unet_forward_ref: mode %d (1 = 'w' park the attn1 inputs, 2 = 'r' attend to them)", mode);
    CTX_REQUIRE(ref_row0 >= 0 && ref_row0 < B, "unet_forward_ref: ref_row0=%d outside [0, B)", ref_row0);
    if (check_dims(u, B, H, W, ctx_len)) return CTX_E_ARG;
    u->s = (hipStream_t)stream;
    u->dry = false;
    u->ref_mode = mode; u->ref_bank = (f16 *)bank; u->ref_row0 = mode == 2 ? ref_row0 : 0;
    int rc = unet_run(u, sample, timestep, ctx, B, H, W, ctx_len, out);
    u->ref_mode = 0; u->ref_bank = nullptr; u->ref_row0 = 0;
    return rc;
}

extern "C" int32_t ctx_unet_set_residual_fp32(ctx_unet_t *u, int32_t on)
{
    CTX_REQUIRE(u, "unet_set_residual_fp32: null handle");
    u->res32 = on != 0;
    return CTX_OK;
}

extern "C" int32_t ctx_unet_set_taps(ctx_unet_t *u, void *buf, int64_t capacity)
{
    CTX_REQUIRE(u && capacity >= 0, "unet_set_taps: bad args");
    u->tap_buf = (f16 *)buf; u->tap_cap = buf ? (size_t)capacity : 0;
    return CTX_OK;
}
extern "C" int32_t ctx_unet_tap_count(const ctx_unet_t *u) { return u ? (int32_t)u->taps.size() : -1; }
extern "C" int32_t ctx_unet_tap_info(const ctx_unet_t *u, int32_t i, int64_t *offset, int32_t *rows, int32_t *channels)
{
    CTX_REQUIRE(u && offset && rows && channels && i >= 0 && i < (int32_t)u->taps.size(), "unet_tap_info: bad args");
    *offset = (int64_t)u->taps[i].off; *rows = u->taps[i].rows; *channels = u->taps[i].C;
    return CTX_OK;
}

extern "C" int32_t ctx_unet_stats(const ctx_unet_t *u, int32_t klass, int64_t *launches, double *flops)
{
    CTX_REQUIRE(u && klass >= 0 && klass < 3 && launches && flops, "unet_stats: bad args");
    *launches = u->launches[klass];
    *flops = u->flops[klass];
    return CTX_OK;
}
```

Baseline: 120.7 steps/s.

## Fuse GroupNorm statistics into producer GEMM, split-K reduce and concat epilogues

Producer kernels (the gemm144 staged epilogue, the split-K reduce and the skip concat) now accumulate per-group sum and sum-of-squares partial records from their f16 outputs. The following GroupNorm reads these records and runs only its apply pass, skipping the separate statistics pass over the activation. This is meant to remove one full read of large activations per GroupNorm on the two-pass path. It adds record buffers, extra LDS work and barriers in the epilogues, and a per-layer chain of records threaded through the UNet; taking statistics from rounded f16 outputs can shift numerics slightly.

```diff
diff --git a/contexture-nerf_amd/csrc/gemm.hip b/contexture-nerf_amd/csrc/gemm.hip
--- a/contexture-nerf_amd/csrc/gemm.hip
+++ b/contexture-nerf_amd/csrc/gemm.hip
@@ -384,6 +384,45 @@
         for (int j = 0; j < 4; ++j) o[j] = (f16)v[j];
         *(f16x4 *)(a.out + (size_t)m * a.ldc + nn) = o;
     }
+}
+
+__global__ __launch_bounds__(1024) void k_splitk_reduce_rec(GemmArgs a, int PL)
+{
+    extern __shared__ float s_rp[];
+    const int n4 = a.N / 4;
+    const int b = blockIdx.y, sl = blockIdx.x, nsl = gridDim.x;
+    const int col = threadIdx.x % n4, pl = threadIdx.x / n4;
+    const int nn = col * 4;
+    const int rb = (a.gn_rows + nsl - 1) / nsl;
+    const int r0 = b * a.gn_rows + sl * rb, r1 = b * a.gn_rows + min(a.gn_rows, (sl + 1) * rb);
+    const size_t MN = (size_t)a.M * a.N;
+    float gs[4] = {0.f, 0.f, 0.f, 0.f}, gq[4] = {0.f, 0.f, 0.f, 0.f};
+    f16x4 bs = {0, 0, 0, 0};
+    if (a.bias) bs = *(const f16x4 *)(a.bias + nn);
+#pragma unroll 4
+    for (int m = r0 + pl; m < r1; m += PL) {
+        f32x4 v = *(const f32x4 *)(a.part + (size_t)m * a.N + nn);
+        for (int sidx = 1; sidx < a.splitk; ++sidx) {
+            f32x4 p = *(const f32x4 *)(a.part + sidx * MN + (size_t)m * a.N + nn);
+            v += p;
+        }
+        if (a.bias) { for (int j = 0; j < 4; ++j) v[j] += (float)bs[j]; }
+        if (a.rowbias) {
+            f16x4 rb4 = *(const f16x4 *)(a.rowbias + (size_t)(m / a.rows_per_batch) * a.ldrb + nn);
+            for (int j = 0; j < 4; ++j) v[j] += (float)rb4[j];
+        }
+        if (a.residual) { f16x4 r4 = *(const f16x4 *)(a.residual + (size_t)m * a.ldr + nn); for (int j = 0; j < 4; ++j) v[j] += (float)r4[j]; }
+        f16x4 o;
+        for (int j = 0; j < 4; ++j) o[j] = (f16)v[j];
+        *(f16x4 *)(a.out + (size_t)m * a.ldc + nn) = o;
+#pragma unroll
+        for (int j = 0; j < 4; ++j) { const float f = (float)o[j]; gs[j] += f; gq[j] += f * f; }
+    }
+#pragma unroll
+    for (int j = 0; j < 4; ++j) { s_rp[(pl * a.N + nn + j) * 2] = gs[j]; s_rp[(pl * a.N + nn + j) * 2 + 1] = gq[j]; }
+    __syncthreads();
+    gn_fold_records(s_rp, s_rp + (size_t)PL * a.N * 2, PL, a.N, a.gn_c0, a.gn_cg, a.gn_groups,
+                    a.gn_rec + ((size_t)b * nsl + sl) * a.gn_groups * 2, threadIdx.x, blockDim.x);
 }
 
 static int g_force_tile = -1, g_force_gemm8 = -1;
@@ -431,6 +470,23 @@
 
 static void launch_reduce(GemmArgs &a, hipStream_t s)
 {
+    a.gn_ns = 0;
+    const int n4 = a.N / 4;
+    if (a.gn_rec && !a.out32 && !a.res32 && a.N % 4 == 0 && n4 <= 1024 && a.gn_rows > 0 && a.M % a.gn_rows == 0) {
+        const int PL = max(1, 1024 / n4);
+        const int nsl = min(GN_REC_MAX_NS, max(1, cdiv(a.gn_rows, PL * 4)));
+        const int nt = n4 * PL, na = max(1, nt / (2 * a.N));
+        const size_t lds = (size_t)(PL + na) * a.N * 2 * sizeof(float);
+        a.gn_ns = nsl;
+        const dim3 grid(nsl, a.M / a.gn_rows);
+        if (ctx_prof_on()) {
+            hipEvent_t e0, e1;
+            ctx_prof_events(0, &e0, &e1);
+            hipExtLaunchKernelGGL(k_splitk_reduce_rec, grid, dim3(nt), lds, s, e0, e1, 0, a, PL);
+        } else
+            hipLaunchKernelGGL(k_splitk_reduce_rec, grid, dim3(nt), lds, s, a, PL);
+        return;
+    }
     size_t total = (size_t)a.M * (a.N / 4);
     unsigned nb = (unsigned)((total + 255) / 256 < 2048 ? (total + 255) / 256 : 2048);
     if (ctx_prof_on()) {
@@ -505,6 +561,7 @@
 
 int ctx_gemm_dispatch(GemmArgs &a, bool conv, hipStream_t s)
 {
+    a.gn_ns = 0;
     const bool only_pipe = a.zins || a.res32 || a.out32;
     if (only_pipe) a.use8 = 0;
     const int want8 = only_pipe ? 0 : (g_force_gemm8 >= 0 ? g_force_gemm8 : a.use8);
diff --git a/contexture-nerf_amd/csrc/gemm144.hip b/contexture-nerf_amd/csrc/gemm144.hip
--- a/contexture-nerf_amd/csrc/gemm144.hip
+++ b/contexture-nerf_amd/csrc/gemm144.hip
@@ -361,6 +361,11 @@
         asm volatile("s_waitcnt vmcnt(0) lgkmcnt(0)" ::: "memory");
         ctx_barrier();
         constexpr int NT = 64 * NW, CPR = G144_BN / 8;
+        constexpr bool REC = NT % CPR == 0;
+        const bool rec = REC && a.gn_rec;
+        float gs[8], gq[8];
+#pragma unroll
+        for (int e = 0; e < 8; ++e) { gs[e] = 0.f; gq[e] = 0.f; }
 #pragma unroll
         for (int half = 0; half < BMB / 9; ++half) {
             if (half) __syncthreads();
@@ -398,7 +403,24 @@
 #pragma unroll
                 for (int e = 0; e < 8; ++e) o[e] = (f16)v[e];
                 *(f16x8 *)(a.out + (size_t)m * a.ldc + n) = o;
-            }
+                if (rec) {
+#pragma unroll
+                    for (int e = 0; e < 8; ++e) { const float f = (float)o[e]; gs[e] += f; gq[e] += f * f; }
+                }
+            }
+        }
+        if (rec) {
+            constexpr int PL = NT / CPR;
+            float *sp = tile;
+            __syncthreads();
+            const int pl = tid / CPR, c8 = (tid - pl * CPR) * 8;
+#pragma unroll
+            for (int e = 0; e < 8; ++e) { sp[(pl * G144_BN + c8 + e) * 2] = gs[e]; sp[(pl * G144_BN + c8 + e) * 2 + 1] = gq[e]; }
+            __syncthreads();
+            const int b = m0 / a.gn_rows;
+            const int slot = ((m0 - b * a.gn_rows) / BM) * a.ntn + tile_n;
+            gn_fold_records(sp, sp + PL * G144_BN * 2, PL, G144_BN, a.gn_c0 + n0, a.gn_cg, a.gn_groups,
+                            a.gn_rec + ((size_t)b * a.gn_ns + slot) * a.gn_groups * 2, tid, NT);
         }
         return;
     }
@@ -453,6 +475,12 @@
     static int stg = -1;
     if (stg < 0) { const char *e = getenv("CTX_G144_STAGE"); stg = e ? atoi(e) : 1; }
     a.stage_epi = stg && form != 0 && a.N % 8 == 0 && a.ldc % 8 == 0 && (!a.residual || a.ldr % 8 == 0) && (!a.rowbias || a.ldrb % 8 == 0);
+    a.gn_ns = 0;
+    if (a.gn_rec && S == 1 && a.stage_epi && a.gn_rows > 0 && a.gn_rows % bm == 0 && a.M % a.gn_rows == 0 &&
+        (a.gn_rows / bm) * a.ntn <= GN_REC_MAX_NS)
+        a.gn_ns = (a.gn_rows / bm) * a.ntn;
+    float *const rec_keep = a.gn_rec;
+    if (S == 1 && !a.gn_ns) a.gn_rec = nullptr;
     static bool attr[20] = {};
     auto go = [&](auto kern, int which, int threads, int ns) {
         const size_t lds = (size_t)ns * (bm + G144_BN) * 64 * sizeof(f16);
@@ -490,5 +518,6 @@
         else if (ups) go(k_gemm144<3, 2, true, 3, 0, true>, 11, 384, 3); else go(k_gemm144<3, 2, true, 3, 0>, 1, 384, 3);
         break;
     }
+    a.gn_rec = rec_keep;
     return 1;
 }
diff --git a/contexture-nerf_amd/csrc/kernels.h b/contexture-nerf_amd/csrc/kernels.h
--- a/contexture-nerf_amd/csrc/kernels.h
+++ b/contexture-nerf_amd/csrc/kernels.h
@@ -25,7 +25,32 @@
     int tile, use8;
     int stage_epi;
     int mfast;
+    float *gn_rec;
+    int gn_groups, gn_cg, gn_c0, gn_rows, gn_ns;
 };
+
+#define GN_REC_MAX_NS 256
+__device__ __forceinline__ void gn_fold_records(const float *s_part, float *s_tmp, int PL, int NC, int c0, int cg, int G, float *rec,
+                                                int tid, int nt)
+{
+    const int na = max(1, nt / (2 * NC));
+    for (int i = tid; i < 2 * NC * na; i += nt) {
+        const int a = i / (2 * NC), cw = i - a * 2 * NC;
+        float s = 0.f;
+        for (int l = a; l < PL; l += na) s += s_part[l * 2 * NC + cw];
+        s_tmp[i] = s;
+    }
+    __syncthreads();
+    for (int i = tid; i < 2 * G; i += nt) {
+        const int g = i >> 1, w = i & 1;
+        const int lo = max(g * cg, c0) - c0, hi = min(g * cg + cg, c0 + NC) - c0;
+        float s = 0.f;
+        for (int c = lo; c < hi; ++c)
+            for (int a = 0; a < na; ++a) s += s_tmp[(a * NC + c) * 2 + w];
+        rec[i] = s;
+    }
+    __syncthreads();
+}
 
 int ctx_gemm_dispatch(GemmArgs &a, bool conv, hipStream_t s);
 int ctx_gemm8_try(GemmArgs &a, bool conv, bool force, hipStream_t s);
@@ -45,6 +70,10 @@
 extern "C" int64_t ctx_groupnorm_ws_bytes(int32_t B, int32_t groups);
 int ctx_groupnorm_any(const void *x, int x32, const void *gamma, const void *beta, int B, int HW, int C, int groups, float eps, int silu,
                       void *y, void *stats_ws, hipStream_t stream);
+int ctx_groupnorm_two_pass(int HW, int C, int groups);
+int ctx_groupnorm_apply_rec(const f16 *x, const float *rec, int ns, const void *gamma, const void *beta, int B, int HW, int C, int groups,
+                            float eps, int silu, void *y, hipStream_t stream);
+int ctx_concat_rec_f16(const f16 *a, const f16 *b, int B, int HW, int Ca, int Cb, int groups, f16 *y, float *rec, hipStream_t s);
 int ctx_layernorm_any(const void *x, int x32, const void *gamma, const void *beta, int64_t rows, int C, float eps, void *y, hipStream_t stream);
 int ctx_concat_f32(const float *a, const float *b, int64_t M, int Ca, int Cb, float *y, hipStream_t s);
 int ctx_f16_to_f32(const f16 *x, int64_t n, float *y, hipStream_t s);
diff --git a/contexture-nerf_amd/csrc/norm.hip b/contexture-nerf_amd/csrc/norm.hip
--- a/contexture-nerf_amd/csrc/norm.hip
+++ b/contexture-nerf_amd/csrc/norm.hip
@@ -1,6 +1,7 @@
 #include "common.h"
 #include "kernels.h"
 #include <math.h>
+#include <algorithm>
 
 struct F8 { float v[8]; };
 template <bool X32>
@@ -230,6 +231,32 @@
     }
 }
 
+int ctx_groupnorm_two_pass(int HW, int C, int groups)
+{
+    static int fuse = -1;
+    if (fuse < 0) { const char *e = getenv("CTX_GN_FUSED"); fuse = e ? atoi(e) : 1; }
+    const int cg = C / groups, cpg = cg / 8;
+    if (!fuse || cg % 8 != 0 || cpg > GN_FT) return 1;
+    const int plf = GN_FT / cpg;
+    return (HW + plf - 1) / plf <= GN_FU ? 0 : 1;
+}
+
+int ctx_groupnorm_apply_rec(const f16 *x, const float *rec, int ns, const void *gamma, const void *beta, int B, int HW, int C, int groups,
+                            float eps, int silu, void *y, hipStream_t stream)
+{
+    CTX_REQUIRE(x && rec && gamma && beta && y && ns > 0, "groupnorm_apply_rec: null pointer or no records");
+    CTX_REQUIRE(B > 0 && HW > 0 && C % 8 == 0 && C % groups == 0 && groups <= GN_MAX_GROUPS && C <= GN_MAX_C &&
+                    256 % groups == 0 && (256 / groups & (256 / groups - 1)) == 0,
+                "groupnorm_apply_rec: unsupported B=%d HW=%d C=%d groups=%d", B, HW, C, groups);
+    const int c8n = C / 8;
+    const int apl = (256 + c8n - 1) / c8n;
+    const int nb = (HW + apl * GN_AU - 1) / (apl * GN_AU);
+    hipLaunchKernelGGL(k_gn_apply<false>, dim3(nb, B), dim3(c8n * apl), 0, stream, x, rec, (const f16 *)gamma, (const f16 *)beta, HW, C,
+                       groups, ns, apl, eps, silu, (f16 *)y);
+    CTX_CHECK_LAUNCH("groupnorm_apply_rec");
+    return CTX_OK;
+}
+
 extern "C" int64_t ctx_groupnorm_ws_bytes(int32_t B, int32_t groups)
 {
     return ((int64_t)B * GN_MAX_SPLITS * groups * 2 + (int64_t)B * 2 * GN_MAX_C) * 4;
@@ -250,12 +277,10 @@
                 "groupnorm: unsupported B=%d HW=%d C=%d groups=%d", B, HW, C, groups);
     hipStream_t s = stream;
     {
-        static int fuse = -1;
-        if (fuse < 0) { const char *e = getenv("CTX_GN_FUSED"); fuse = e ? atoi(e) : 1; }
         const int cg = C / groups;
         const int cpg = cg / 8;
         const int plf = cg % 8 == 0 ? GN_FT / cpg : 0;
-        if (fuse && cg % 8 == 0 && cpg <= GN_FT && (HW + plf - 1) / plf <= GN_FU) {
+        if (!ctx_groupnorm_two_pass(HW, C, groups)) {
             const int thr = (cpg * plf + 63) / 64 * 64;
             if (x32) hipLaunchKernelGGL(k_gn_fused<true>, dim3(groups, B), dim3(thr), 0, s, x, (const f16 *)gamma, (const f16 *)beta, HW, C, groups, plf, eps, silu, (f16 *)y);
             else hipLaunchKernelGGL(k_gn_fused<false>, dim3(groups, B), dim3(thr), 0, s, x, (const f16 *)gamma, (const f16 *)beta, HW, C, groups, plf, eps, silu, (f16 *)y);
@@ -492,6 +517,57 @@
         f16x8 v = c8 < a8 ? *(const f16x8 *)(a + m * Ca + c8 * 8) : *(const f16x8 *)(b + m * Cb + (c8 - a8) * 8);
         *(f16x8 *)(y + i * 8) = v;
     }
+}
+
+__global__ __launch_bounds__(1024) void k_concat_rec(const f16 *__restrict__ a, const f16 *__restrict__ b, int HW, int Ca, int Cb, int PL,
+                                                     int G, f16 *__restrict__ y, float *__restrict__ rec)
+{
+    extern __shared__ float s_cp[];
+    const int C = Ca + Cb, c8n = C / 8, a8 = Ca / 8;
+    const int bs = blockIdx.y, sl = blockIdx.x, nsl = gridDim.x;
+    const int c8 = threadIdx.x % c8n, pl = threadIdx.x / c8n;
+    const int per = (HW + nsl - 1) / nsl;
+    const int p0 = sl * per, p1 = min(HW, p0 + per);
+    const bool left = c8 < a8;
+    const f16 *src = left ? a + (size_t)bs * HW * Ca + c8 * 8 : b + (size_t)bs * HW * Cb + (c8 - a8) * 8;
+    const int ld = left ? Ca : Cb;
+    f16 *dst = y + (size_t)bs * HW * C + c8 * 8;
+    float s[8], q[8];
+#pragma unroll
+    for (int j = 0; j < 8; ++j) { s[j] = 0.f; q[j] = 0.f; }
+    for (int p = p0 + pl; p < p1; p += PL * GN_U) {
+        f16x8 v[GN_U];
+#pragma unroll
+        for (int u = 0; u < GN_U; ++u) v[u] = *(const f16x8 *)(src + (size_t)min(p + u * PL, p1 - 1) * ld);
+#pragma unroll
+        for (int u = 0; u < GN_U; ++u) {
+            if (p + u * PL < p1) {
+                *(f16x8 *)(dst + (size_t)(p + u * PL) * C) = v[u];
+#pragma unroll
+                for (int j = 0; j < 8; ++j) { const float f = (float)v[u][j]; s[j] += f; q[j] += f * f; }
+            }
+        }
+    }
+#pragma unroll
+    for (int j = 0; j < 8; ++j) { s_cp[(pl * C + c8 * 8 + j) * 2] = s[j]; s_cp[(pl * C + c8 * 8 + j) * 2 + 1] = q[j]; }
+    __syncthreads();
+    gn_fold_records(s_cp, s_cp + (size_t)PL * C * 2, PL, C, 0, C / G, G, rec + ((size_t)bs * nsl + sl) * G * 2, threadIdx.x, blockDim.x);
+}
+
+int ctx_concat_rec_f16(const f16 *a, const f16 *b, int B, int HW, int Ca, int Cb, int groups, f16 *y, float *rec, hipStream_t s)
+{
+    const int C = Ca + Cb, c8n = C / 8;
+    if (Ca % 8 || Cb % 8 || c8n > 1024 || C % groups) return 0;
+    const int PL = max(1, min(HW, 1024 / c8n));
+    const int nt = c8n * PL, na = max(1, nt / (2 * C));
+    const int by_size = (int)std::min<int64_t>(GN_MAX_SPLITS, (int64_t)HW * C * 2 / (384 * 1024));
+    const int nsl = min(GN_REC_MAX_NS, max(1, min(HW / PL, max(16, max(by_size, (64 + B - 1) / B)))));
+    const size_t lds = (size_t)(PL + na) * C * 2 * sizeof(float);
+    static bool attr = false;
+    if (!attr) { (void)hipFuncSetAttribute((const void *)k_concat_rec, hipFuncAttributeMaxDynamicSharedMemorySize, 80 * 1024); attr = true; }
+    if (lds > 80 * 1024) return 0;
+    hipLaunchKernelGGL(k_concat_rec, dim3(nsl, B), dim3(nt), lds, s, a, b, HW, Ca, Cb, PL, groups, y, rec);
+    return nsl;
 }
 
 int ctx_concat_f32(const float *a, const float *b, int64_t M, int Ca, int Cb, float *y, hipStream_t s)
diff --git a/contexture-nerf_amd/csrc/unet.hip b/contexture-nerf_amd/csrc/unet.hip
--- a/contexture-nerf_amd/csrc/unet.hip
+++ b/contexture-nerf_amd/csrc/unet.hip
@@ -72,6 +72,7 @@
     const f16 *add_res = nullptr;
     float add_scale = 1.0f;
     bool res32 = false;
+    int gn_epi = 1;
     void *allocS(size_t n) { return alloc(n * (res32 ? 4 : 2)); }
     struct Tap { size_t off; int rows, C; };
     f16 *tap_buf = nullptr;
@@ -434,8 +435,23 @@
 static void note(ctx_unet *u, int klass, double fl, int n = 1) { u->launches[klass] += n; u->flops[klass] += fl; }
 #define RUN(expr) do { if (!u->dry && u->rc == 0) { int r__ = (expr); if (r__ != 0) u->rc = r__; } } while (0)
 
+struct GnRec { float *buf; int ns, rows; };
+static size_t gn_rec_bytes(int B, int groups) { return (size_t)B * GN_REC_MAX_NS * groups * 2 * sizeof(float); }
+static GnRec *gn_want(ctx_unet *u, GnRec *r, int HW, int C)
+{
+    if (!r) return nullptr;
+    r->ns = 0; r->rows = HW;
+    if (!r->buf || !u->gn_epi || u->res32 || !ctx_groupnorm_two_pass(HW, C, u->cfg.groups)) return nullptr;
+    return r;
+}
+static void gn_request(ctx_unet *u, GemmArgs &a, const GnRec *rq)
+{
+    if (!rq) return;
+    a.gn_rec = rq->buf; a.gn_groups = u->cfg.groups; a.gn_cg = a.N / u->cfg.groups; a.gn_c0 = 0; a.gn_rows = rq->rows;
+}
+
 static void op_gemm(ctx_unet *u, const f16 *X, size_t w, size_t bias, bool has_bias, const void *res, int M, int N, int K, void *out,
-                    int epi = 0, bool res_s = false, bool out_s = false)
+                    int epi = 0, bool res_s = false, bool out_s = false, GnRec *rq = nullptr)
 {
     GemmArgs a = {};
     a.X = X; a.Wt = u->W + w; a.bias = has_bias ? u->W + bias : nullptr; a.residual = (const f16 *)res; a.out = (f16 *)out;
@@ -445,11 +461,13 @@
     size_t mark = u->top;
     ctx_gemm_plan(a, false);
     if (a.splitk > 1) a.part = (float *)u->alloc((size_t)a.splitk * M * N * 4);
+    gn_request(u, a, rq);
     RUN(ctx_gemm_dispatch(a, false, u->s));
+    if (rq && !u->dry && u->rc == 0) rq->ns = a.gn_ns;
     u->top = mark;
 }
 static void op_conv(ctx_unet *u, const f16 *x, size_t w, size_t bias, const f16 *rowbias, int ldrb, const void *res, int B, int H,
-                    int W, int Cin, int Cout, int stride, int ups, void *out, bool res_s = false, bool out_s = false)
+                    int W, int Cin, int Cout, int stride, int ups, void *out, bool res_s = false, bool out_s = false, GnRec *rq = nullptr)
 {
     GemmArgs a = {};
     int Hv = H << ups, Wv = W << ups;
@@ -462,12 +480,20 @@
     size_t mark = u->top;
     ctx_gemm_plan(a, true);
     if (a.splitk > 1) a.part = (float *)u->alloc((size_t)a.splitk * a.M * a.N * 4);
+    gn_request(u, a, rq);
     RUN(ctx_gemm_dispatch(a, true, u->s));
+    if (rq && !u->dry && u->rc == 0) rq->ns = a.gn_ns;
     u->top = mark;
 }
-static void op_gn(ctx_unet *u, const void *x, size_t g, size_t b, int B, int HW, int C, float eps, int silu, f16 *y, void *stats, bool x_s = true)
-{
-    note(u, 2, 0, 2);
+static void op_gn(ctx_unet *u, const void *x, size_t g, size_t b, int B, int HW, int C, float eps, int silu, f16 *y, void *stats, bool x_s = true,
+                  const GnRec *rec = nullptr)
+{
+    if (rec && rec->ns > 0 && !(u->res32 && x_s)) {
+        note(u, 2, 0);
+        RUN(ctx_groupnorm_apply_rec((const f16 *)x, rec->buf, rec->ns, u->W + g, u->W + b, B, HW, C, u->cfg.groups, eps, silu, y, u->s));
+        return;
+    }
+    note(u, 2, 0, ctx_groupnorm_two_pass(HW, C, u->cfg.groups) ? 2 : 1);
     RUN(ctx_groupnorm_any(x, (u->res32 && x_s) ? 1 : 0, u->W + g, u->W + b, B, HW, C, u->cfg.groups, eps, silu, y, stats, u->s));
 }
 static void op_ln(ctx_unet *u, const void *x, size_t g, size_t b, int64_t rows, int C, f16 *y)
@@ -497,33 +523,37 @@
     void *gn_stats;
 };
 
-static void *run_resnet(ctx_unet *u, const FwdCtx &f, const ResP &r, const void *x, int H, int W, void *out)
+static void *run_resnet(ctx_unet *u, const FwdCtx &f, const ResP &r, const void *x, int H, int W, void *out, const GnRec *xin = nullptr,
+                        GnRec *orq = nullptr)
 {
     const int B = f.B, HW = H * W, M = B * HW;
     size_t mark = u->top;
     f16 *t1 = u->allocH((size_t)M * r.cin);
-    op_gn(u, x, r.n1g, r.n1b, B, HW, r.cin, u->cfg.norm_eps, 1, t1, f.gn_stats);
+    op_gn(u, x, r.n1g, r.n1b, B, HW, r.cin, u->cfg.norm_eps, 1, t1, f.gn_stats, true, xin);
     f16 *h = u->allocH((size_t)M * r.cout);
-    op_conv(u, t1, r.c1w, r.c1b, f.tproj ? f.tproj + r.temb_row : nullptr, u->temb_rows, nullptr, B, H, W, r.cin, r.cout, 1, 0, h);
+    GnRec hr = {(float *)u->alloc(gn_rec_bytes(B, u->cfg.groups)), 0, HW};
+    op_conv(u, t1, r.c1w, r.c1b, f.tproj ? f.tproj + r.temb_row : nullptr, u->temb_rows, nullptr, B, H, W, r.cin, r.cout, 1, 0, h, false, false,
+            gn_want(u, &hr, HW, r.cout));
     f16 *t2 = u->allocH((size_t)M * r.cout);
-    op_gn(u, h, r.n2g, r.n2b, B, HW, r.cout, u->cfg.norm_eps, 1, t2, f.gn_stats, false);
+    op_gn(u, h, r.n2g, r.n2b, B, HW, r.cout, u->cfg.norm_eps, 1, t2, f.gn_stats, false, &hr);
     const void *sc = x;
     if (r.cin != r.cout) {
         void *s2 = u->allocS((size_t)M * r.cout);
         op_gemm(u, op_as16(u, x, (size_t)M * r.cin), r.scw, r.scb, true, nullptr, M, r.cout, r.cin, s2, 0, false, true);
         sc = s2;
     }
-    op_conv(u, t2, r.c2w, r.c2b, nullptr, 0, sc, B, H, W, r.cout, r.cout, 1, 0, out, true, true);
+    op_conv(u, t2, r.c2w, r.c2b, nullptr, 0, sc, B, H, W, r.cout, r.cout, 1, 0, out, true, true, gn_want(u, orq, HW, r.cout));
     u->top = mark;
     return out;
 }
 
-static void *run_transformer(ctx_unet *u, const FwdCtx &f, const TrP &t, const void *x, int H, int W, void *out)
+static void *run_transformer(ctx_unet *u, const FwdCtx &f, const TrP &t, const void *x, int H, int W, void *out, const GnRec *xin = nullptr,
+                             GnRec *orq = nullptr)
 {
     const int B = f.B, S = H * W, M = B * S, C = t.C, cd = u->cfg.cross_attention_dim;
     size_t mark = u->top;
     f16 *g = u->allocH((size_t)M * C);
-    op_gn(u, x, t.ng, t.nb, B, S, C, 1e-6f, 0, g, f.gn_stats);
+    op_gn(u, x, t.ng, t.nb, B, S, C, 1e-6f, 0, g, f.gn_stats, true, xin);
     void *h0 = u->allocS((size_t)M * C);
     op_gemm(u, g, t.piw, t.pib, true, nullptr, M, C, C, h0, 0, false, true);
     f16 *l = g;
@@ -579,7 +609,7 @@
     op_gemm(u, l, t.f1w, t.f1b, true, nullptr, M, 8 * C, C, ff, 1);
     void *h3 = h1;
     op_gemm(u, ff, t.f2w, t.f2b, true, h2, M, C, 4 * C, h3, 0, true, true);
-    op_gemm(u, op_as16(u, h3, (size_t)M * C), t.pow_, t.pob, true, x, M, C, C, out, 0, true, true);
+    op_gemm(u, op_as16(u, h3, (size_t)M * C), t.pow_, t.pob, true, x, M, C, C, out, 0, true, true, gn_want(u, orq, S, C));
     u->top = mark;
     return out;
 }
@@ -596,6 +626,14 @@
     for (int k = 0; k < 3; ++k) { u->launches[k] = 0; u->flops[k] = 0; }
     FwdCtx f; f.B = B; f.L = L;
     f.gn_stats = u->alloc((size_t)ctx_groupnorm_ws_bytes(B, c.groups));
+    {
+        const char *e = getenv("CTX_GN_EPI");
+        u->gn_epi = e ? atoi(e) : 1;
+    }
+    GnRec xr[2] = {{(float *)u->alloc(gn_rec_bytes(B, c.groups)), 0, 0}, {(float *)u->alloc(gn_rec_bytes(B, c.groups)), 0, 0}};
+    int xi = 0;
+    auto xnext = [&]() { xi ^= 1; return &xr[xi]; };
+    auto xnone = [&]() { xr[xi].ns = 0; };
     f16 *te0 = u->allocH((size_t)B * ch[0]);
     note(u, 2, 0); RUN(ctx_time_embed_f16(timestep, B, ch[0], te0, u->s));
     f16 *te1 = u->allocH((size_t)B * u->temb_dim);
@@ -668,14 +706,23 @@
         for (int j = 0; j < lpb; ++j) {
             int cout = Lv.res[j].cout;
             void *o = u->allocS((size_t)B * h * w * cout);
+            const bool o_gn = j + 1 < lpb || !Lv.has_sampler;
+            const GnRec *xin = &xr[xi];
             if (Lv.has_attn) {
                 size_t mark = u->top;
                 void *t = u->allocS((size_t)B * h * w * cout);
-                run_resnet(u, f, Lv.res[j], x, h, w, t);
+                GnRec *tr = xnext();
+                run_resnet(u, f, Lv.res[j], x, h, w, t, xin, tr);
                 u->tap(t, B * h * w, cout);
-                run_transformer(u, f, Lv.tr[j], t, h, w, o);
+                GnRec *orr = xnext();
+                run_transformer(u, f, Lv.tr[j], t, h, w, o, tr, o_gn ? orr : nullptr);
+                if (!o_gn) orr->ns = 0;
                 u->top = mark;
-            } else run_resnet(u, f, Lv.res[j], x, h, w, o);
+            } else {
+                GnRec *orr = xnext();
+                run_resnet(u, f, Lv.res[j], x, h, w, o, xin, o_gn ? orr : nullptr);
+                if (!o_gn) orr->ns = 0;
+            }
             u->tap(o, B * h * w, cout);
             x = o; cur = cout;
             skips.push_back({x, cur, h, w});
@@ -684,7 +731,9 @@
             int ho = (h - 1) / 2 + 1, wo = (w - 1) / 2 + 1;
             void *o = u->allocS((size_t)B * ho * wo * cur);
             size_t m0 = u->top;
-            op_conv(u, op_as16(u, x, (size_t)B * h * w * cur), Lv.sw, Lv.sb, nullptr, 0, nullptr, B, h, w, cur, cur, 2, 0, o, false, true);
+            GnRec *orr = xnext();
+            op_conv(u, op_as16(u, x, (size_t)B * h * w * cur), Lv.sw, Lv.sb, nullptr, 0, nullptr, B, h, w, cur, cur, 2, 0, o, false, true,
+                    gn_want(u, orr, ho * wo, cur));
             u->top = m0;
             x = o; h = ho; w = wo;
             u->tap(x, B * h * w, cur);
@@ -715,13 +764,17 @@
     }
     {
         void *o1 = u->allocS((size_t)B * h * w * cur);
-        run_resnet(u, f, u->mid.res[0], x, h, w, o1);
+        const GnRec *xin = &xr[xi];
+        GnRec *r1 = xnext();
+        run_resnet(u, f, u->mid.res[0], x, h, w, o1, xin, r1);
         u->tap(o1, B * h * w, cur);
         void *o2 = u->allocS((size_t)B * h * w * cur);
-        run_transformer(u, f, u->mid.tr[0], o1, h, w, o2);
+        GnRec *r2 = xnext();
+        run_transformer(u, f, u->mid.tr[0], o1, h, w, o2, r1, r2);
         u->tap(o2, B * h * w, cur);
         void *o3 = u->allocS((size_t)B * h * w * cur);
-        run_resnet(u, f, u->mid.res[1], o2, h, w, o3);
+        run_resnet(u, f, u->mid.res[1], o2, h, w, o3, r2);
+        xnext(); xnone();
         u->tap(o3, B * h * w, cur);
         x = o3;
     }
@@ -746,14 +799,26 @@
             size_t mark = u->top;
             void *cat = u->allocS((size_t)B * h * w * cin);
             note(u, 2, 0);
+            GnRec *cr = gn_want(u, xnext(), h * w, cin);
+            if (cr && !u->dry && u->rc == 0)
+                cr->ns = ctx_concat_rec_f16((const f16 *)x, (const f16 *)sk.p, B, h * w, cur, sk.C, c.groups, (f16 *)cat, cr->buf, u->s);
             if (u->res32) RUN(ctx_concat_f32((const float *)x, (const float *)sk.p, (int64_t)B * h * w, cur, sk.C, (float *)cat, u->s));
-            else RUN(ctx_concat_f16((const f16 *)x, (const f16 *)sk.p, (int64_t)B * h * w, cur, sk.C, (f16 *)cat, u->s));
+            else if (!cr || cr->ns == 0) RUN(ctx_concat_f16((const f16 *)x, (const f16 *)sk.p, (int64_t)B * h * w, cur, sk.C, (f16 *)cat, u->s));
+            const bool o_gn = i + 1 == n && j == lpb;
+            const GnRec *xin = &xr[xi];
             if (Lv.has_attn) {
                 void *t = u->allocS((size_t)B * h * w * cout);
-                run_resnet(u, f, Lv.res[j], cat, h, w, t);
+                GnRec *tr = xnext();
+                run_resnet(u, f, Lv.res[j], cat, h, w, t, xin, tr);
                 u->tap(t, B * h * w, cout);
-                run_transformer(u, f, Lv.tr[j], t, h, w, o);
-            } else run_resnet(u, f, Lv.res[j], cat, h, w, o);
+                GnRec *orr = xnext();
+                run_transformer(u, f, Lv.tr[j], t, h, w, o, tr, o_gn ? orr : nullptr);
+                if (!o_gn) orr->ns = 0;
+            } else {
+                GnRec *orr = xnext();
+                run_resnet(u, f, Lv.res[j], cat, h, w, o, xin, o_gn ? orr : nullptr);
+                if (!o_gn) orr->ns = 0;
+            }
             u->tap(o, B * h * w, cout);
             u->top = mark;
             x = o; cur = cout;
@@ -762,13 +827,14 @@
             void *o = u->allocS((size_t)B * (2 * h) * (2 * w) * cur);
             size_t m0 = u->top;
             op_conv(u, op_as16(u, x, (size_t)B * h * w * cur), Lv.sw, Lv.sb, nullptr, 0, nullptr, B, h, w, cur, cur, 1, 1, o, false, true);
+            xnone();
             u->top = m0;
             x = o; h *= 2; w *= 2;
             u->tap(x, B * h * w, cur);
         }
     }
     f16 *y = u->allocH((size_t)B * h * w * cur);
-    op_gn(u, x, u->cng, u->cnb, B, h * w, cur, c.norm_eps, 1, y, f.gn_stats);
+    op_gn(u, x, u->cng, u->cnb, B, h * w, cur, c.norm_eps, 1, y, f.gn_stats, true, &xr[xi]);
     note(u, 2, 2.0 * B * h * w * cur * c.out_channels * 9);
     RUN(ctx_conv_out_f16(y, u->W + u->cow, u->W + u->cob, B, h, w, cur, c.out_channels, out, u->s));
     if (!u->dry && u->rc == 0) {
```

Result: no change. 121.5 steps/s, median of 6 (+0.7%).
